# ath92/splat-renderer

Hardware: AMD Instinct MI355X
Metric: Msplats/sec (higher is better)
Workload: dtype f32

## Files before the change

include/splat.h:

```cpp
#ifndef SPLAT_H
#define SPLAT_H

#include <stddef.h>
#include <stdint.h>

#ifdef __cplusplus
extern "C" {
#endif

#define SPLAT_ABI_VERSION 3

#define SPLAT_OK 0
#define SPLAT_ERR_INVALID (-1)
#define SPLAT_ERR_HIP (-2)
#define SPLAT_ERR_OOM (-3)
#define SPLAT_ERR_CAPACITY (-4)
#define SPLAT_ERR_STATE (-5)
#define SPLAT_ERR_NO_DEVICE (-6)
#define SPLAT_ERR_COMM (-7)
#define SPLAT_ERR_RETRY (-8)

typedef struct splat_ctx splat_ctx;
typedef struct splat_sorter splat_sorter;
typedef struct splat_binner splat_binner;
typedef struct splat_comm splat_comm;

#define SPLAT_PROPS_BYTES 32
#define SPLAT_PROJECTED_BYTES 32
#define SPLAT_SORT_BLOCK 3840

enum {
    SPLAT_STAGE_PROJECT = 0,
    SPLAT_STAGE_SORT = 1,
    SPLAT_STAGE_BIN = 2,
    SPLAT_STAGE_COMPOSITE = 3,
    SPLAT_STAGE_EXCHANGE = 4,
    SPLAT_STAGE_BIN_SCATTER = 5,
    SPLAT_STAGE_BIN_PASS2 = 6,
    SPLAT_STAGE_BIN_TILE_SORT = 7,
    SPLAT_STAGE_COUNT = 8
};

int splat_ctx_create(int device_ordinal, splat_ctx **out);
int splat_ctx_create_on_stream(int device_ordinal, void *hip_stream, splat_ctx **out);
void splat_ctx_destroy(splat_ctx *ctx);
const char *splat_last_error(splat_ctx *ctx);
int splat_sync(splat_ctx *ctx);
int splat_abi_version(void);
int splat_set_timing(splat_ctx *ctx, int enabled);
#define SPLAT_TIMING_COUNT_ENTRIES 0x80000000u
int splat_set_timing_stages(splat_ctx *ctx, uint32_t stage_mask);
int splat_set_timing_sampling(splat_ctx *ctx, uint32_t every);
int splat_stage_time_ms(splat_ctx *ctx, int stage, float *ms);
// ... 24 lines not shown
void splat_sort_destroy(splat_sorter *s);
uint32_t splat_sort_capacity(const splat_sorter *s);
void *splat_sort_keys(splat_sorter *s);
void *splat_sort_payload(splat_sorter *s);
int splat_sort_run(splat_sorter *s, uint32_t n, uint32_t bit_begin, uint32_t bit_end);
void *splat_sort_sorted_payload(splat_sorter *s);
void *splat_sort_sorted_keys(splat_sorter *s);
int splat_probe_lds_atomic_order(splat_ctx *ctx, uint64_t *mismatches);
int splat_sort_set_mode(splat_sorter *s, int mode);
int splat_rank_status(splat_ctx *ctx, int *policy, int *atomics_ordered, uint32_t *order_faults);
#ifdef SPLAT_TEST_HOOKS
int splat_debug_inject_order_fault(splat_ctx *ctx, uint32_t tile, uint32_t position);
int splat_debug_set_tile_order(splat_ctx *ctx, const void *order_dptr);
int splat_debug_set_tile_sort_order(splat_ctx *ctx, const void *order_dptr);
int splat_debug_rerun_tile_sort(splat_ctx *ctx, splat_binner *binner);
int splat_debug_tile_sort_launches(splat_ctx *ctx, uint32_t *launches);
int splat_debug_lds_rate(splat_ctx *ctx, int kind, uint32_t workgroups_per_cu, uint32_t iters, float *ms);
#endif
int splat_composite_forget_history(splat_ctx *ctx);
int splat_composite_options(splat_ctx *ctx, int kernel, int ahead, int predict);

int splat_scan_u32(splat_ctx *ctx, const void *in, void *out, uint32_t n, void *total_dptr);

int splat_bin_create(splat_ctx *ctx, uint32_t tile_size, splat_binner **out);
void splat_bin_destroy(splat_binner *b);
int splat_bin_run(splat_binner *b, const void *projected, uint32_t n_splats, const void *sorted,
                  uint32_t n_sorted, uint32_t width, uint32_t height, uint32_t tile_row0,
                  uint32_t tile_row1);
uint32_t splat_bin_tile_size(const splat_binner *b);
int splat_bin_counts(splat_binner *b, void **dptr);
int splat_bin_offsets(splat_binner *b, void **dptr);
int splat_bin_indices(splat_binner *b, void **dptr);
int splat_bin_total(splat_binner *b, uint64_t *total_pairs);
#define SPLAT_FRAME_ORDER_DEFAULT (-1)
#define SPLAT_FRAME_SORT_FIRST 0
#define SPLAT_FRAME_TILE_FIRST 1
int splat_bin_set_frame_order(splat_binner *b, int order);
int splat_bin_dims(splat_binner *b, uint32_t *ntx, uint32_t *nty);

int splat_validate_tile_order(splat_ctx *ctx, const void *projected, const void *tile_offsets,
                              uint32_t num_tiles, const void *tile_indices, uint64_t total_pairs,
                              uint64_t *violations_host);

#define SPLAT_COMPOSITE_FRONT_TO_BACK 0
#define SPLAT_COMPOSITE_REFERENCE_LITERAL 1
#define SPLAT_RECORDS_PROJECTED 0
#define SPLAT_RECORDS_COMPACT 1
#define SPLAT_RECORDS_DISC48 2
#define SPLAT_RECORDS_LIT32 3
#define SPLAT_FOOTPRINT_ISOTROPIC 0
#define SPLAT_FOOTPRINT_DISC 1
#define SPLAT_FOOTPRINT_ELLIPSOID 2
typedef struct splat_composite_cfg {
    uint32_t mode;
    uint32_t early_out;
    uint32_t tile_size;
    uint32_t tile_row0;
    uint32_t tile_row1;
    uint32_t record_format;
    uint32_t prelit;
    uint32_t footprint;
} splat_composite_cfg;
int splat_lit_colors(splat_ctx *ctx, const void *color_opacity, uint32_t color_stride_vec4,
                     const void *normals, uint32_t normal_stride_vec4, uint32_t n, void *lit);
int splat_composite(splat_ctx *ctx, const splat_composite_cfg *cfg, const void *color_opacity,
                    uint32_t color_stride_vec4, const void *normals, uint32_t normal_stride_vec4,
// ... 191 lines not shown
```

splat_renderer_amd/_lib.py:

```python
import ctypes as C
import os

_HERE = os.path.dirname(os.path.abspath(__file__))
LIB_PATH = os.environ.get("SPLAT_LIB_PATH") or os.path.join(_HERE, "libsplat_hip.so")

OK = 0
ERR_NAMES = {-1: "INVALID", -2: "HIP", -3: "OOM", -4: "CAPACITY", -5: "STATE", -6: "NO_DEVICE", -7: "COMM", -8: "RETRY"}
ERR_CAPACITY, ERR_RETRY = -4, -8
RENDER_AGAIN = (ERR_CAPACITY, ERR_RETRY)

STAGE_PROJECT, STAGE_SORT, STAGE_BIN, STAGE_COMPOSITE, STAGE_EXCHANGE, STAGE_BIN_SCATTER, STAGE_BIN_PASS2, STAGE_BIN_TILE_SORT = range(8)
STAGE_NAMES = ("project", "sort", "bin", "composite", "exchange", "bin_scatter", "bin_second_pass", "bin_tile_sort")
TIMING_COUNT_ENTRIES = 0x80000000
MODE_FRONT_TO_BACK, MODE_REFERENCE_LITERAL = 0, 1
RECORDS_PROJECTED, RECORDS_COMPACT, RECORDS_DISC48, RECORDS_LIT32 = 0, 1, 2, 3
FOOTPRINT_ISOTROPIC, FOOTPRINT_DISC, FOOTPRINT_ELLIPSOID = 0, 1, 2
U32_MAX = 0xFFFFFFFF


class SplatError(RuntimeError):
    def __init__(self, code, msg):
        super().__init__(f"libsplat_hip error {ERR_NAMES.get(code, code)}: {msg}")
        self.code = code


SDF_SPHERE, SDF_BOX, SDF_TORUS, SDF_CAPSULE, SDF_UNION, SDF_INTERSECTION, SDF_SUBTRACTION, SDF_SMOOTH_UNION = 0, 1, 2, 3, 16, 17, 18, 19
SDF_MAX_INSTR = 32


class SdfInstr(C.Structure):
    _fields_ = [("op", C.c_uint32), ("a", C.c_float * 7)]


class Aov(C.Structure):
    _fields_ = [("depth_f32", C.c_void_p), ("alpha_f32", C.c_void_p), ("id_u32", C.c_void_p)]


class CompositeCfg(C.Structure):
    _fields_ = [("mode", C.c_uint32), ("early_out", C.c_uint32), ("tile_size", C.c_uint32),
                ("tile_row0", C.c_uint32), ("tile_row1", C.c_uint32), ("record_format", C.c_uint32),
                ("prelit", C.c_uint32), ("footprint", C.c_uint32)]

# ... 62 lines not shown
    "splat_densify_plan_workspace_bytes": (C.c_uint64, [_u32]),
    "splat_densify_plan": (_i, [_vp, _vp, _vp, _vp, _vp, _vp, _u32, C.POINTER(DensifyCfg), _vp, C.c_uint64, _vp, C.POINTER(_u32),
                                C.POINTER(_u32)]),
    "splat_densify_geometry": (_i, [_vp, _vp, _u32, _vp, _vp, _vp, C.POINTER(DensifyCfg), _vp, _vp]),
    "splat_densify_rows": (_i, [_vp, _vp, _u32, _vp, _vp, _u32, _u32]),
    "splat_mcmc_sample_workspace_bytes": (C.c_uint64, [_u32]),
    "splat_mcmc_sample": (_i, [_vp, _vp, _u32, _u32, _u32, _f64, C.c_uint64, _vp, C.c_uint64, _vp, _vp, _vp, C.POINTER(_u32)]),
    "splat_mcmc_apply": (_i, [_vp, _vp, _vp, _vp, _u32, _u32, _u32, _f64, C.POINTER(McmcPlanes)]),
    "splat_mcmc_noise": (_i, [_vp, _vp, _vp, _vp, _vp, _u32, _f64, _u32, C.c_uint64]),
    "splat_extract_keys":(_i, [_vp, _vp, _u32, _u32, _vp, _vp]),
    "splat_sort_create": (_i, [_vp, _u32, _pvp]),
    "splat_sort_destroy": (None, [_vp]),
    "splat_sort_capacity": (_u32, [_vp]),
    "splat_sort_keys": (_vp, [_vp]),
    "splat_sort_payload": (_vp, [_vp]),
    "splat_sort_run": (_i, [_vp, _u32, _u32, _u32]),
    "splat_sort_sorted_payload": (_vp, [_vp]),
    "splat_sort_sorted_keys": (_vp, [_vp]),
    "splat_probe_lds_atomic_order": (_i, [_vp, C.POINTER(C.c_uint64)]),
    "splat_sort_set_mode": (_i, [_vp, _i]),
    "splat_rank_status": (_i, [_vp, C.POINTER(_i), C.POINTER(_i), C.POINTER(_u32)]),
    "splat_composite_forget_history": (_i, [_vp]),
    "splat_composite_options": (_i, [_vp, _i, _i, _i]),
    "splat_scan_u32": (_i, [_vp, _vp, _vp, _u32, _vp]),
    "splat_bin_create": (_i, [_vp, _u32, _pvp]),
    "splat_bin_destroy": (None, [_vp]),
    "splat_bin_run": (_i, [_vp, _vp, _u32, _vp, _u32, _u32, _u32, _u32, _u32]),
    "splat_bin_tile_size": (_u32, [_vp]),
    "splat_bin_counts": (_i, [_vp, _pvp]),
    "splat_bin_offsets": (_i, [_vp, _pvp]),
    "splat_bin_indices": (_i, [_vp, _pvp]),
    "splat_bin_total": (_i, [_vp, C.POINTER(C.c_uint64)]),
    "splat_bin_set_frame_order": (_i, [_vp, _i]),
    "splat_bin_dims": (_i, [_vp, C.POINTER(_u32), C.POINTER(_u32)]),
    "splat_validate_tile_order": (_i, [_vp, _vp, _vp, _u32, _vp, C.c_uint64, C.POINTER(C.c_uint64)]),
    "splat_lit_colors": (_i, [_vp, _vp, _u32, _vp, _u32, _u32, _vp]),
    "splat_composite": (_i, [_vp, C.POINTER(CompositeCfg), _vp, _u32, _vp, _u32, _vp, _vp, _vp, _vp, _u32, _u32,
                             _vp, _vp, _vp]),
    "splat_render_frame": (_i, [_vp, _vp, _vp, C.POINTER(CompositeCfg), C.POINTER(C.c_float), _vp, _vp, _u32, _u32,
                                _u32, _vp, _vp, _vp]),
    "splat_render_frame_planes": (_i, [_vp, _vp, _vp, C.POINTER(CompositeCfg), C.POINTER(C.c_float), _vp, _vp, _vp, _u32,
                                       _u32, _u32, _vp, _vp, _vp]),
    "splat_composite_aov": (_i, [_vp, C.POINTER(CompositeCfg), _vp, _u32, _vp, _u32, _vp, _vp, _vp, _vp, _u32, _u32,
                                 _vp, _vp, _vp, C.POINTER(Aov)]),
    "splat_render_frame_aov": (_i, [_vp, _vp, _vp, C.POINTER(CompositeCfg), C.POINTER(C.c_float), _vp, _vp, _u32, _u32,
                                    _u32, _vp, _vp, _vp, C.POINTER(Aov)]),
    "splat_render_frame_planes_aov": (_i, [_vp, _vp, _vp, C.POINTER(CompositeCfg), C.POINTER(C.c_float), _vp, _vp, _vp,
                                           _u32, _u32, _u32, _vp, _vp, _vp, C.POINTER(Aov)]),
    "splat_project_slice": (_i, [_vp, C.POINTER(C.c_float), _vp, _u32, _u32, _u32, _vp]),
    "splat_project_slice_compact": (_i, [_vp, C.POINTER(C.c_float), _vp, _u32, _u32, _u32, _vp]),
    "splat_project_slice_disc": (_i, [_vp, C.POINTER(C.c_float), _vp, _u32, _vp, _u32, _u32, _u32, _vp]),
    "splat_expand_compact": (_i, [_vp, _vp, _u32, _u32, _vp]),
    "splat_band_frame": (_i, [_vp, _vp, _vp, C.POINTER(CompositeCfg), _vp, _vp, _vp, _u32, _u32, _u32, _vp, _vp, _vp]),
    "splat_band_settle": (_i, [_vp, _vp, _vp, C.POINTER(_u32), C.POINTER(C.c_uint64)]),
    "splat_band_kept": (_i, [_vp, _vp, C.POINTER(_u32)]),
    "splat_band_keys": (_i, [_vp, _vp, _vp, _u32, _u32, _u32, _u32, _u32, _u32, C.POINTER(_u32)]),
    "splat_sdf_gradients": (_i, [_vp, _vp, _u32, _vp, _u32, _vp]),
    "splat_sdf_update_positions": (_i, [_vp, _vp, _vp, _u32, _vp]),
    "splat_sdf_scale_factors": (_i, [_vp, _vp, _u32, _vp, _u32, _vp]),
    "splat_sdf_curvature": (_i, [_vp, _vp, _vp, _u32, _vp]),
    "splat_sdf_seed_positions": (_i, [_vp, C.POINTER(C.c_float), C.POINTER(C.c_float), _u32, C.c_uint64, _vp]),
    "splat_sdf_generate": (_i, [_vp, _vp, _u32, C.POINTER(C.c_float), C.POINTER(C.c_float), C.c_uint64, _vp, _u32, _u32, _vp, _vp, _vp, _vp]),
    "splat_point_frame": (_i, [_vp, _vp, C.POINTER(C.c_float), _vp, _u32, _vp, _u32, _vp, _u32, _u32, _u32, _u32, _vp, _vp, _vp, _vp]),
    "splat_comm_unique_id": (_i, [_vp]),
    "splat_comm_init": (_i, [_vp, _i, _i, _vp, _pvp]),
    "splat_comm_destroy": (None, [_vp]),
# ... 60 lines not shown
```

splat_renderer_amd/csrc/bin.hip:

```cpp
#include "common.h"
#include <cstring>
#include "tile_range.h"

#include <chrono>
#include <cstdio>
#include <cstdlib>
#include <sched.h>

constexpr uint32_t BIN_THREADS = 256;
constexpr uint32_t BIN_PER_THREAD = 4;
constexpr uint32_t BIN_BLOCK = BIN_THREADS * BIN_PER_THREAD;
constexpr uint32_t BIN_STAGE_PAIRS = 4096;

__device__ __forceinline__ uint32_t range_hits(uint2 r) {
    const uint32_t tx0 = r.x & 0xffffu, tx1 = r.x >> 16, ty0 = r.y & 0xffffu, ty1 = r.y >> 16;
    return (tx0 > tx1 || ty0 > ty1) ? 0u : (tx1 - tx0 + 1) * (ty1 - ty0 + 1);
}

__device__ __forceinline__ uint32_t block_sum(uint32_t v, uint32_t *wsum) {
#pragma unroll
    for (int d = 32; d >= 1; d >>= 1) v += __shfl_xor(v, d);
    if ((threadIdx.x & 63) == 0) wsum[threadIdx.x >> 6] = v;
    __syncthreads();
    return wsum[0] + wsum[1] + wsum[2] + wsum[3];
// ... 155 lines not shown
        hi = nhi;
    }
    const uint32_t pos = lo + lane;
    const bool less = pos < hi && sorted_tiles[pos] < t;
    const uint32_t first = lo + (uint32_t)__popcll(__ballot(less));
    if (lane == 0) offsets[t] = first;
}

__global__ __launch_bounds__(256) void k_tile_counts(const uint32_t *__restrict__ offsets, uint32_t tiles,
                                                     uint32_t *__restrict__ counts) {
    const uint32_t t = blockIdx.x * 256u + threadIdx.x;
    if (t < tiles) counts[t] = offsets[t + 1] - offsets[t];
}

__global__ __launch_bounds__(256) void k_validate_tile_order(const float4 *__restrict__ projected,
                                                             const uint32_t *__restrict__ offsets, uint32_t tiles,
                                                             const uint32_t *__restrict__ indices, uint32_t pairs,
                                                             unsigned long long *__restrict__ violations) {
    const uint32_t i = blockIdx.x * 256u + threadIdx.x;
    if (i + 1 >= pairs) return;
    uint32_t lo = 0, hi = tiles;
    while (hi - lo > 1) {
        const uint32_t mid = (lo + hi) >> 1;
        if (offsets[mid] <= i) lo = mid; else hi = mid;
    }
    if (i + 1 >= offsets[lo + 1]) return;
    const uint32_t a = indices[i], b = indices[i + 1];
    const uint32_t ka = __float_as_uint(reinterpret_cast<const float *>(projected)[(size_t)a * 8 + 4]);
    const uint32_t kb = __float_as_uint(reinterpret_cast<const float *>(projected)[(size_t)b * 8 + 4]);
    const uint32_t sa = ka ^ (((ka >> 31) == 1u) ? 0xffffffffu : 0x80000000u), sb = kb ^ (((kb >> 31) == 1u) ? 0xffffffffu : 0x80000000u);
    if (sa > sb || (sa == sb && a >= b)) atomicAdd(violations, 1ull);
}

static void binner_free(splat_binner *b) {
    if (b->counts) (void)hipFree(b->counts);
    if (b->offsets) (void)hipFree(b->offsets);
    if (b->blocksums) (void)hipFree(b->blocksums);
    if (b->ranges) (void)hipFree(b->ranges);
    if (b->tf_hist) (void)hipFree(b->tf_hist);
    b->tf_hist = nullptr;
    b->counts = b->offsets = b->blocksums = nullptr;
    b->ranges = nullptr;
    b->tiles_cap = b->splats_cap = 0;
}

static void sorter_free_members(splat_sorter *s) {
    if (s->keys) (void)hipFree(s->keys);
    if (s->keys_b) (void)hipFree(s->keys_b);
    if (s->hist) (void)hipFree(s->hist);
    if (s->d_count) (void)hipFree(s->d_count);
    s->keys = s->keys_b = s->payload = s->payload_b = s->hist = s->d_count = nullptr;
    s->capacity = 0;
}

int binner_reserve_range32(splat_binner *b, uint32_t n_splats) {
    splat_ctx *ctx = b->ctx;
    if (n_splats <= b->range32_cap) return SPLAT_OK;
    HIP_TRY(ctx, hipStreamSynchronize(ctx->stream));
    if (b->range32) (void)hipFree(b->range32);
    b->range32 = nullptr;
    b->range32_cap = 0;
    if (hipMalloc((void **)&b->range32, (size_t)n_splats * 4 + 16) != hipSuccess) return ctx_fail(ctx, SPLAT_ERR_OOM, "binner hipMalloc");
    b->range32_cap = n_splats;
    return SPLAT_OK;
}

// ... 34 lines not shown
    return SPLAT_OK;
}

int binner_reserve(splat_binner *b, uint32_t tiles, uint32_t n_sorted) {
    splat_ctx *ctx = b->ctx;
    if (tiles <= b->tiles_cap && n_sorted <= b->splats_cap) return SPLAT_OK;
    HIP_TRY(ctx, hipStreamSynchronize(ctx->stream));
    uint32_t tc = tiles > b->tiles_cap ? tiles : b->tiles_cap;
    uint32_t sc = n_sorted > b->splats_cap ? n_sorted : b->splats_cap;
    binner_free(b);
    if (hipMalloc((void **)&b->counts, (size_t)tc * 4 + 16) != hipSuccess ||
        hipMalloc((void **)&b->offsets, (size_t)tc * 4 + 16) != hipSuccess ||
        hipMalloc((void **)&b->blocksums, ((size_t)div_up(sc, BIN_BLOCK) + TF_SMALL_FRAME_SPLATS / TF_BLOCK_SMALL) * 4 + 16) != hipSuccess ||
        hipMalloc((void **)&b->ranges, (size_t)sc * 8 + 16) != hipSuccess ||
        hipMalloc((void **)&b->tf_hist, ((size_t)256 * (div_up(sc, BIN_BLOCK) + TF_SMALL_FRAME_SPLATS / TF_BLOCK_SMALL) + 256) * 4) != hipSuccess) {
        binner_free(b);
        return ctx_fail(ctx, SPLAT_ERR_OOM, "binner hipMalloc");
    }
    b->tiles_cap = tc;
    b->splats_cap = sc;
    return SPLAT_OK;
}

int binner_run(splat_binner *b, const void *projected, uint32_t n_splats, const void *sorted, uint32_t n_sorted, uint32_t width,
               uint32_t height, uint32_t tile_row0, uint32_t tile_row1, const uint32_t *range32, const uint32_t *n_sorted_dev,
               const uint32_t *depth_keys, const uint2 *range_wide) {
    splat_ctx *ctx = b->ctx;
    const bool tile_first = depth_keys != nullptr;
    const bool hist_ready = b->tf_hist_ready;
    const uint32_t *tf_cidx = b->tf_cidx, *tf_kept = b->tf_kept;
    b->tf_hist_ready = false;
    b->tf_cidx = nullptr;
    b->tf_kept = nullptr;
    ARG_CHECK(ctx, width >= 1 && height >= 1);
    ARG_CHECK(ctx, n_sorted == 0 || (projected && (sorted || tile_first)));
    ARG_CHECK(ctx, !tile_first || (range32 && n_sorted == n_splats && !n_sorted_dev));
    ARG_CHECK(ctx, !range_wide || (!range32 && !tile_first));
    const uint32_t ntx = div_up(width, b->tile), nty = div_up(height, b->tile);
    ARG_CHECK(ctx, ntx <= 65535 && nty <= 65535 && (uint64_t)ntx * nty <= (1u << 24));
    const uint32_t tiles = ntx * nty;
    if (tile_row1 > nty) tile_row1 = nty;
    if (tile_row0 > tile_row1) tile_row0 = tile_row1;
    const uint32_t blocks = div_up(n_sorted, BIN_BLOCK);

    int rc = binner_reserve(b, tiles, n_sorted);
    if (rc != SPLAT_OK) return rc;
    b->ntx = ntx;
    b->nty = nty;
    b->ran = false;
    const BinParams bp = {width, height, b->tile, ntx, nty, tile_row0, tile_row1};

    rc = binner_settle(b);
    if (rc != SPLAT_OK) return rc;

    const uint32_t tf_bits = tile_id_bits(tiles), tf_lo_bits = tile_id_low_bits(tiles);
    ARG_CHECK(ctx, !tile_first || hist_ready);

    stage_begin(ctx, SPLAT_STAGE_BIN);
    uint32_t total32 = 0;
    bool async = false;
    if (n_sorted > 0) {
        if (tile_first) {
            rc = radix_rowscan_launch(ctx, b->tf_hist, div_up(n_splats, b->tf_block), 1u << tf_lo_bits);
            if (rc != SPLAT_OK) return rc;
        } else if (range_wide)
            hipLaunchKernelGGL(k_bin_count_wide, dim3(blocks), dim3(BIN_THREADS), 0, ctx->stream, range_wide, n_splats,
// ... 8 lines not shown
        const uint64_t want_async = (uint64_t)b->last_total + b->last_total / 8 + 4096;
        async = b->allow_async && b->have_last && b->last_total > 0 && want_async <= b->pairs.capacity;
        if (!(tile_first && async)) {
            rc = scan_exclusive_u32(ctx, b->blocksums, b->blocksums, tile_first ? div_up(n_splats, b->tf_block) : blocks, b->d_total);
            if (rc != SPLAT_OK) return rc;
        }
        if (async) {
            b->pair_limit = (uint32_t)want_async;
            total32 = b->pair_limit;
        } else {
            HIP_TRY(ctx, hipMemcpyAsync(b->pinned, b->d_total, 4, hipMemcpyDeviceToHost, ctx->stream));
            HIP_TRY(ctx, hipStreamSynchronize(ctx->stream));
            total32 = *(volatile uint32_t *)b->pinned;
            b->last_total = total32;
            b->have_last = true;
            if (total32 > b->pairs.capacity) {
                uint64_t want = (uint64_t)total32 + total32 / 2 + 8192;
                if (want > 0x3ffff000ull) want = 0x3ffff000ull;
                if (total32 > want) return ctx_fail(ctx, SPLAT_ERR_CAPACITY, "binSplats: more than 2^30 tile-splat pairs");
                rc = sorter_reserve(&b->pairs, (uint32_t)want);
                if (rc != SPLAT_OK) return rc;
            }
            b->pair_limit = total32;
        }
    }
    b->total = async ? b->last_total : total32;
    if (total32 > 0 && tile_first) {
        rc = binner_reserve_wide(b);
        if (rc != SPLAT_OK) return rc;
        const uint32_t tf_hi_bits = tf_bits - tf_lo_bits;
        stage_begin(ctx, SPLAT_STAGE_BIN_SCATTER);
        rc = tf_scatter_launch(ctx, range32, depth_keys, n_splats, ntx, (1u << tf_lo_bits) - 1u, b->tf_hist, b->d_total, b->pair_limit,
                               b->d_total + 1, b->tf_hi, b->wide_a, b->tf_block, tf_lo_bits, tf_hi_bits > 0, &b->tf_runs, b->offsets, tiles,
                               nullptr, 0u, tf_cidx, tf_kept);
        stage_end(ctx, SPLAT_STAGE_BIN_SCATTER);
        if (rc != SPLAT_OK) return rc;
        const bool primary = tf_hi_bits == 0;
        stage_begin(ctx, SPLAT_STAGE_BIN_PASS2);
        rc = tf_second_pass_launch(ctx, b->tf_hi, b->wide_a, b->wide_b, &b->tf_runs, total32, tiles, tf_lo_bits, tf_hi_bits, b->tf2_hist,
                                   b->offsets, b->d_total);
        stage_end(ctx, SPLAT_STAGE_BIN_PASS2);
        if (rc != SPLAT_OK) return rc;
        const uint32_t band_tiles = tile_row1 > tile_row0 ? (tile_row1 - tile_row0) * ntx : 1u;
        const uint64_t band_key = ((uint64_t)tile_row0 << 48) ^ ((uint64_t)tile_row1 << 32) ^ tiles;
        stage_begin(ctx, SPLAT_STAGE_BIN_TILE_SORT);
        rc = tile_sort_launch(ctx, b->offsets, tiles, primary ? b->wide_a : b->wide_b, primary ? b->wide_b : b->wide_a, b->pairs.payload,
                              b->counts, b->d_total + 1, band_tiles >= 6144u ? (uint32_t)(b->total / band_tiles) : 0u, band_tiles,
                              (async && b->last_band_key == band_key) ? b->last_long_tiles : 0xffffffffu, &b->last_short_class);
        stage_end(ctx, SPLAT_STAGE_BIN_TILE_SORT);
        if (rc != SPLAT_OK) return rc;
        b->pairs.result_in_primary = true;
        b->pending_tile_first = true;
        b->last_band_key = band_key;
        b->report_for_composite = b->pinned_dev;
        b->report_seq = ++b->seq;
        b->pending = true;
    } else if (total32 > 0) {
        hipLaunchKernelGGL(k_bin_expand, dim3(blocks), dim3(BIN_THREADS), 0, ctx->stream, (const uint32_t *)sorted, n_sorted,
                           b->ranges, b->blocksums, ntx, b->pair_limit, b->d_total + 1, b->pairs.keys, b->pairs.payload);
        LAUNCH_CHECK(ctx, "k_bin_expand");
        const uint32_t bits = tile_id_bits(tiles);
        const uint32_t *p_dev = async ? b->d_total : nullptr;
        const uint32_t lo_bits = tile_id_low_bits(tiles);
        rc = radix_sort_pairs(ctx, b->pairs.keys, b->pairs.payload, b->pairs.keys_b, b->pairs.payload_b, b->pairs.hist, total32, 0,
                              bits, &b->pairs.result_in_primary, 0, p_dev, false, lo_bits);
        if (rc != SPLAT_OK) return rc;
        const uint32_t *sorted_tiles = b->pairs.result_in_primary ? b->pairs.keys : b->pairs.keys_b;
        hipLaunchKernelGGL(k_tile_offsets, dim3(div_up(tiles + 1, 4)), dim3(256), 0, ctx->stream, sorted_tiles, total32, p_dev,
                           tiles, b->offsets, b->d_total, async ? b->pinned_dev : nullptr, async ? ++b->seq : 0u);
        LAUNCH_CHECK(ctx, "k_tile_offsets");
        hipLaunchKernelGGL(k_tile_counts, dim3(div_up(tiles, 256)), dim3(256), 0, ctx->stream, b->offsets, tiles, b->counts);
        LAUNCH_CHECK(ctx, "k_tile_counts");
        if (async) b->pending = true;
    } else {
        HIP_TRY(ctx, hipMemsetAsync(b->counts, 0, (size_t)tiles * 4, ctx->stream));
        HIP_TRY(ctx, hipMemsetAsync(b->offsets, 0, (size_t)(tiles + 1) * 4, ctx->stream));
        if (b->pairs.capacity == 0) {
            rc = sorter_reserve(&b->pairs, 1);
            if (rc != SPLAT_OK) return rc;
        }
    }
    stage_end(ctx, SPLAT_STAGE_BIN);
    b->ran = true;
    return SPLAT_OK;
}

int binner_settle(splat_binner *b) {
    if (!b->pending) return SPLAT_OK;
    splat_ctx *ctx = b->ctx;
    b->pending = false;
    volatile uint32_t *rep = (volatile uint32_t *)b->pinned;
    auto next_query = std::chrono::steady_clock::now() + std::chrono::milliseconds(5);
    for (uint32_t spins = 0; rep[2] != b->seq; ++spins) {
        if ((spins & 63u) != 63u) continue;
        if (std::chrono::steady_clock::now() < next_query) {
            sched_yield();
            continue;
        }
        next_query = std::chrono::steady_clock::now() + std::chrono::milliseconds(1);
        const hipError_t q = hipStreamQuery(ctx->stream);
        if (q == hipSuccess) {
            if (rep[2] != b->seq) return ctx_fail(ctx, SPLAT_ERR_STATE, "binner: the pair-total report of the previous frame never arrived");
            break;
        }
        if (q != hipErrorNotReady) {
            b->have_last = false;
            return ctx_fail(ctx, SPLAT_ERR_HIP, "binner: waiting for the previous frame's pair total", q);
        }
    }
    __atomic_thread_fence(__ATOMIC_ACQUIRE);
    const uint32_t total = ((volatile uint32_t *)b->pinned)[0], flags = ((volatile uint32_t *)b->pinned)[1];
    b->last_long_tiles = b->pending_tile_first ? ((volatile uint32_t *)b->pinned)[3] : 0xffffffffu;
    b->pending_tile_first = false;
    b->last_total = total;
    b->have_last = true;
    b->total = total;
    if (flags & FRAME_FLAG_ORDER) {
        b->ran = false;
        ctx->order_faults++;
        if (ctx->rank_policy != RANK_BALLOT)
            fprintf(stderr, "[splat] a frame's tile lists failed the per-tile order check (tile lists are re-rendered): this context ranks with "
                            "ballots from now on (splat_rank_status: policy ballot, orderFaults %u)\n", ctx->order_faults);
        ctx->rank_policy = RANK_BALLOT;
        return ctx_fail(ctx, SPLAT_ERR_RETRY,
                        "the previous frame's tile lists failed the order check (ranking with returning LDS atomics was not in lane "
                        "order): the context now ranks with ballots; render that frame again");
    }
    if ((flags & FRAME_FLAG_OVERFLOW) || total > b->pair_limit) {
        uint64_t want = (uint64_t)total + total / 2 + 8192;
        if (want > 0x3ffff000ull) want = 0x3ffff000ull;
        b->ran = false;
        int rc = sorter_reserve(&b->pairs, (uint32_t)want);
        if (rc != SPLAT_OK) return rc;
        return ctx_fail(ctx, SPLAT_ERR_CAPACITY,
                        "the previous frame produced more tile-splat pairs than its sync-free limit (sized from the frame "
                        "before it): its tile lists are incomplete; capacity has been raised, render that frame again");
    }
    return SPLAT_OK;
}

extern "C" {

#ifdef SPLAT_TEST_HOOKS
int splat_debug_rerun_tile_sort(splat_ctx *ctx, splat_binner *b) {
    if (!ctx || !b) return ctx_fail(ctx, SPLAT_ERR_INVALID, "ctx/binner is NULL");
    ARG_CHECK(ctx, b->ran && b->wide_a && b->wide_b && b->ntx && b->nty);
    const uint32_t tiles = b->ntx * b->nty;
    const bool primary = tile_id_bits(tiles) - tile_id_low_bits(tiles) == 0;
    return tile_sort_launch(ctx, b->offsets, tiles, primary ? b->wide_a : b->wide_b, primary ? b->wide_b : b->wide_a, b->pairs.payload_b,
                            nullptr, b->d_total + 4, tiles >= 6144u ? (uint32_t)(b->total / tiles) : 0u);
}
#endif

int splat_bin_create(splat_ctx *ctx, uint32_t tile_size, splat_binner **out) {
    if (!ctx) return ctx_fail(nullptr, SPLAT_ERR_INVALID, "ctx is NULL");
    ARG_CHECK(ctx, out != nullptr);
    *out = nullptr;
    ARG_CHECK(ctx, tile_size >= 1 && tile_size <= 4096);
    splat_binner *b = new splat_binner();
    b->ctx = ctx;
    b->tile = tile_size;
    b->pairs.ctx = ctx;
    if (hipMalloc((void **)&b->d_total, 32) != hipSuccess || hipHostMalloc((void **)&b->pinned, 16, hipHostMallocMapped | hipHostMallocCoherent) != hipSuccess ||
        hipHostGetDevicePointer((void **)&b->pinned_dev, b->pinned, 0) != hipSuccess ||
        hipEventCreateWithFlags(&b->readback_done, hipEventDisableTiming) != hipSuccess) {
        if (b->d_total) (void)hipFree(b->d_total);
        if (b->pinned) (void)hipHostFree(b->pinned);
        delete b;
        return ctx_fail(ctx, SPLAT_ERR_OOM, "binner allocation");
    }
    memset(b->pinned, 0, 16);
    if (const char *e = getenv("SPLAT_BIN_SYNC")) b->allow_async = !(e[0] == '1');
    *out = b;
    return SPLAT_OK;
}

void splat_bin_destroy(splat_binner *b) {
    if (!b) return;
    (void)hipStreamSynchronize(b->ctx->stream);
    binner_free(b);
    sorter_free_members(&b->pairs);
    if (b->d_total) (void)hipFree(b->d_total);
    if (b->range32) (void)hipFree(b->range32);
    binner_free_wide(b);
    if (b->expanded) (void)hipFree(b->expanded);
    if (b->discs) (void)hipFree(b->discs);
    if (b->points) (void)hipFree(b->points);
    if (b->band_idx) (void)hipFree(b->band_idx);
    if (b->pinned) (void)hipHostFree(b->pinned);
    if (b->readback_done) (void)hipEventDestroy(b->readback_done);
    delete b;
}

int splat_bin_run(splat_binner *b, const void *projected, uint32_t n_splats, const void *sorted, uint32_t n_sorted,
                  uint32_t width, uint32_t height, uint32_t tile_row0, uint32_t tile_row1) {
    if (!b) return ctx_fail(nullptr, SPLAT_ERR_INVALID, "binner is NULL");
    return binner_run(b, projected, n_splats, sorted, n_sorted, width, height, tile_row0, tile_row1, nullptr);
}

uint32_t splat_bin_tile_size(const splat_binner *b) { return b ? b->tile : 0; }

int splat_bin_set_frame_order(splat_binner *b, int order) {
    if (!b) return ctx_fail(nullptr, SPLAT_ERR_INVALID, "binner is NULL");
    ARG_CHECK(b->ctx, order >= SPLAT_FRAME_ORDER_DEFAULT && order <= SPLAT_FRAME_TILE_FIRST);
    b->frame_order = order;
    return SPLAT_OK;
}

int splat_bin_counts(splat_binner *b, void **dptr) {
    if (!b || !dptr) return ctx_fail(nullptr, SPLAT_ERR_INVALID, "binner/dptr is NULL");
    if (int rc = binner_settle(b)) return rc;
    if (!b->ran) return ctx_fail(b->ctx, SPLAT_ERR_STATE, "Tile counts buffer not initialized");
    *dptr = b->counts;
    return SPLAT_OK;
}

int splat_bin_offsets(splat_binner *b, void **dptr) {
    if (!b || !dptr) return ctx_fail(nullptr, SPLAT_ERR_INVALID, "binner/dptr is NULL");
    if (int rc = binner_settle(b)) return rc;
    if (!b->ran) return ctx_fail(b->ctx, SPLAT_ERR_STATE, "Tile offsets buffer not initialized");
    *dptr = b->offsets;
    return SPLAT_OK;
}

int splat_bin_indices(splat_binner *b, void **dptr) {
    if (!b || !dptr) return ctx_fail(nullptr, SPLAT_ERR_INVALID, "binner/dptr is NULL");
    if (int rc = binner_settle(b)) return rc;
    if (!b->ran) return ctx_fail(b->ctx, SPLAT_ERR_STATE, "Tile indices buffer not initialized");
    *dptr = b->pairs.result_in_primary ? b->pairs.payload : b->pairs.payload_b;
    return SPLAT_OK;
}

int splat_bin_total(splat_binner *b, uint64_t *total_pairs) {
    if (!b || !total_pairs) return ctx_fail(nullptr, SPLAT_ERR_INVALID, "binner/total is NULL");
    if (int rc = binner_settle(b)) return rc;
    if (!b->ran) return ctx_fail(b->ctx, SPLAT_ERR_STATE, "binSplats has not run");
    *total_pairs = b->total;
    return SPLAT_OK;
}

int splat_validate_tile_order(splat_ctx *ctx, const void *projected, const void *tile_offsets, uint32_t num_tiles,
                              const void *tile_indices, uint64_t total_pairs, uint64_t *violations_host) {
    if (!ctx) return ctx_fail(nullptr, SPLAT_ERR_INVALID, "ctx is NULL");
    ARG_CHECK(ctx, violations_host && (total_pairs == 0 || (projected && tile_offsets && tile_indices)) && num_tiles >= 1);
    ARG_CHECK(ctx, total_pairs < (1ull << 32));
    *violations_host = 0;
    if (total_pairs < 2) return SPLAT_OK;
    int rc = ctx_ensure_scan_ws(ctx, 256);
    if (rc != SPLAT_OK) return rc;
    unsigned long long *d = (unsigned long long *)ctx->scan_ws;
    HIP_TRY(ctx, hipMemsetAsync(d, 0, 8, ctx->stream));
    hipLaunchKernelGGL(k_validate_tile_order, dim3(div_up((uint32_t)total_pairs, 256)), dim3(256), 0, ctx->stream,
                       (const float4 *)projected, (const uint32_t *)tile_offsets, num_tiles, (const uint32_t *)tile_indices,
                       (uint32_t)total_pairs, d);
    LAUNCH_CHECK(ctx, "k_validate_tile_order");
    unsigned long long v = 0;
    HIP_TRY(ctx, hipMemcpyAsync(&v, d, 8, hipMemcpyDeviceToHost, ctx->stream));
    HIP_TRY(ctx, hipStreamSynchronize(ctx->stream));
    *violations_host = v;
    return SPLAT_OK;
// ... 12 lines not shown
```

splat_renderer_amd/csrc/common.h:

```cpp
#pragma once

#include <hip/hip_runtime.h>
#include <stdint.h>
#include <string>

#include "../../include/splat.h"

constexpr int kWave = 64;

#include <vector>
struct StageTimer {
    std::vector<hipEvent_t> beg, end;
    size_t used = 0;
    uint32_t tick = 0;
};
struct PxHistory {
    uint64_t key = 0;
    uint32_t *mem = nullptr;
    uint32_t cap = 0, parity = 0, streak = 0;
    uint64_t last_use = 0;
};
constexpr int PX_HISTORIES = 4;

struct splat_ctx {
    int device = 0;
    hipStream_t stream = nullptr;
    bool own_stream = false;
    std::string err;
    bool timing = false;
    int lds_atomic_ordered = -1;
    int rank_policy = 0;
    uint32_t order_faults = 0;
#ifdef SPLAT_TEST_HOOKS
    const uint32_t *debug_tile_order = nullptr;
    const uint32_t *debug_sort_order = nullptr;
    uint32_t inject_order_fault = 0;
    uint32_t inject_order_position = 0;
    uint32_t tile_sort_launches = 0;
#endif
    int opt_composite_kernel = -1, opt_px_ahead = 0, opt_px_predict = -1;
    PxHistory px_hist[PX_HISTORIES];
    uint64_t px_clock = 0;
    uint32_t timing_mask = 0xffffffffu;
    uint32_t timing_every = 1;
    StageTimer timers[SPLAT_STAGE_COUNT];
    void *scan_ws = nullptr;
    size_t scan_ws_bytes = 0;
    unsigned long long *d_consumed = nullptr;
    uint32_t consumed_tiles = 0;
    uint2 *d_window_counts = nullptr;
    uint32_t window_counts_cap = 0;
    void *pinned = nullptr;
    size_t pinned_bytes = 0;
// ... 14 lines not shown
        hipError_t e__ = (expr);                                             \
        if (e__ != hipSuccess) return ctx_fail((ctx), SPLAT_ERR_HIP, #expr, e__); \
    } while (0)

#define LAUNCH_CHECK(ctx, name)                                                       \
    do {                                                                              \
        hipError_t e__ = hipGetLastError();                                           \
        if (e__ != hipSuccess) return ctx_fail((ctx), SPLAT_ERR_HIP, "launch " name, e__); \
    } while (0)

#define ARG_CHECK(ctx, cond)                                               \
    do {                                                                   \
        if (!(cond)) return ctx_fail((ctx), SPLAT_ERR_INVALID, "argument check failed: " #cond); \
    } while (0)

static inline uint32_t div_up(uint32_t a, uint32_t b) { return (a + b - 1) / b; }
static inline uint64_t div_up64(uint64_t a, uint64_t b) { return (a + b - 1) / b; }

int scan_exclusive_u32(splat_ctx *ctx, const uint32_t *in, uint32_t *out, uint32_t n, uint32_t *total);
constexpr uint32_t RADIX_PART = 4096;
int radix_sort_pairs(splat_ctx *ctx, uint32_t *k0, uint32_t *p0, uint32_t *k1, uint32_t *p1,
                     uint32_t *hist, uint32_t n, uint32_t bit_begin, uint32_t bit_end,
                     bool *result_in_primary, int mode = -1, const uint32_t *n_dev = nullptr,
                     bool iota_payload = false, uint32_t first_bits = 8);

int radix_probe_lds_atomic_order(splat_ctx *ctx, uint64_t *mismatches_host);
int ctx_resolve_rank_mode(splat_ctx *ctx);
constexpr int RANK_CHECKED = 0, RANK_ATOMIC = 1, RANK_BALLOT = 2;
static inline bool rank_atomic_ok(const splat_ctx *ctx, bool checked) {
    if (ctx->lds_atomic_ordered != 1 || ctx->rank_policy == RANK_BALLOT) return false;
    return ctx->rank_policy == RANK_ATOMIC || checked;
}
constexpr uint32_t FRAME_FLAG_OVERFLOW = 1u, FRAME_FLAG_ORDER = 2u;

struct splat_sorter {
    splat_ctx *ctx = nullptr;
    uint32_t capacity = 0;
    uint32_t *keys = nullptr, *keys_b = nullptr, *payload = nullptr, *payload_b = nullptr;
    uint32_t *hist = nullptr;
    uint32_t *d_count = nullptr;
    bool count_pending = false, have_last_count = false;
    uint32_t last_count = 0, count_bound = 0;
    uint32_t *pinned_count = nullptr;
    hipEvent_t count_event = nullptr;
    uint32_t kept_blocks = 0;
    bool result_in_primary = true;
    bool ran = false;
    int mode = -1;
};

int sorter_reserve(splat_sorter *s, uint32_t capacity);

struct TfRuns {
    uint32_t *start, *total;
    uint8_t *part_digit;
    uint32_t *parts;
};
constexpr uint32_t TF_RUN_ALIGN = 4096;
constexpr uint32_t TF_RUN_SLACK = 256 * TF_RUN_ALIGN;
static inline uint32_t tf2_parts_bound(uint32_t pairs, uint32_t lo_bits) { return div_up(pairs, TF_RUN_ALIGN) + (1u << lo_bits); }

struct splat_binner {
    splat_ctx *ctx = nullptr;
    uint32_t tile = 16;
    uint32_t ntx = 0, nty = 0;
    uint32_t tiles_cap = 0, splats_cap = 0, range32_cap = 0;
// ... 9 lines not shown
    uint32_t *tf2_hist = nullptr;
    uint32_t *tf_runs_mem = nullptr;
    TfRuns tf_runs = {};
    uint32_t *tf_hist = nullptr;
    int frame_order = -1;
    void *expanded = nullptr;
    uint32_t expanded_cap = 0;
    void *discs = nullptr;
    uint32_t discs_cap = 0;
    void *points = nullptr;
    uint32_t points_cap = 0;
    bool tf_hist_ready = false;
    uint32_t tf_block = 1024;
    const uint32_t *tf_cidx = nullptr, *tf_kept = nullptr;
    uint32_t *band_idx = nullptr;
    uint32_t band_idx_cap = 0;
    uint64_t total = 0;
    bool ran = false;
    bool allow_async = true;
    bool pending = false;
    bool have_last = false;
    uint32_t last_total = 0;
    uint32_t last_long_tiles = 0xffffffffu;
    uint64_t last_band_key = ~0ull;
    uint32_t last_short_class = 0;
    bool pending_tile_first = false;
    uint32_t pair_limit = 0;
    uint32_t *pinned = nullptr;
    uint32_t *pinned_dev = nullptr;
    uint32_t seq = 0;
    uint32_t *report_for_composite = nullptr;
    uint32_t report_seq = 0;
    hipEvent_t readback_done = nullptr;
};

struct BinParams {
    uint32_t width, height, tile, ntx, nty, row0, row1;
    uint32_t skip_outside;
};

constexpr uint32_t TF_BLOCK_LARGE = 1024, TF_BLOCK_SMALL = 256, TF_SMALL_FRAME_SPLATS = 1u << 20;
struct TfHistOut {
    uint32_t *hist, *blocksums, *overflow_flag;
    uint32_t mask, num_parts;
    uint32_t block = TF_BLOCK_LARGE;
    uint32_t xcd_per = 0;
    uint32_t *cidx = nullptr, *kept_groups = nullptr;
};
__device__ __forceinline__ uint32_t xcd_block_of(uint32_t i, uint32_t xcd_per) {
    return xcd_per ? (i & 7u) * xcd_per + (i >> 3) : i;
}
static inline uint32_t tile_id_bits(uint32_t tiles) {
    uint32_t bits = 1;
    while ((1u << bits) < tiles) ++bits;
    return bits;
}
static inline uint32_t tile_id_low_bits(uint32_t tiles) {
    const uint32_t bits = tile_id_bits(tiles);
    return bits <= 8 ? bits : bits / 2 < 8 ? bits / 2 : 8;
}

__device__ __forceinline__ void tile_report(const uint32_t *d_total, uint32_t *report, uint32_t seq) {
    report[0] = d_total[0];
    report[1] = d_total[1];
    report[3] = d_total[3];
    __threadfence_system();
    __hip_atomic_store(&report[2], seq, __ATOMIC_RELEASE, __HIP_MEMORY_SCOPE_SYSTEM);
}

int binner_reserve_range32(splat_binner *b, uint32_t n_splats);
int binner_run(splat_binner *b, const void *projected, uint32_t n_splats, const void *sorted, uint32_t n_sorted, uint32_t width,
               uint32_t height, uint32_t tile_row0, uint32_t tile_row1, const uint32_t *range32,
               const uint32_t *n_sorted_dev = nullptr, const uint32_t *depth_keys = nullptr,
               const uint2 *range_wide = nullptr);
int binner_reserve(splat_binner *b, uint32_t tiles, uint32_t n_sorted);
int tf_scatter_launch(splat_ctx *ctx, const uint32_t *range32, const uint32_t *depth_keys, uint32_t n, uint32_t ntx, uint32_t mask,
                      const uint32_t *hist, uint32_t *d_total, uint32_t pair_limit, uint32_t *overflow, uint8_t *out_hi,
                      uint2 *out_val, uint32_t block_splats, uint32_t lo_bits, bool second_pass, const TfRuns *runs,
                      uint32_t *offsets_if_final, uint32_t tiles, uint32_t *report, uint32_t seq, const uint32_t *cidx = nullptr,
                      const uint32_t *kept = nullptr);
int tf_second_pass_launch(splat_ctx *ctx, const uint8_t *hi, const uint2 *val_in, uint2 *val_out, const TfRuns *runs, uint32_t pairs_bound,
                          uint32_t tiles, uint32_t lo_bits, uint32_t hi_bits, uint32_t *hist, uint32_t *offsets, const uint32_t *d_total);
int radix_rowscan_launch(splat_ctx *ctx, uint32_t *hist, uint32_t parts, uint32_t rows);
int tile_sort_launch(splat_ctx *ctx, const uint32_t *offsets, uint32_t tiles, uint2 *vals, uint2 *scratch, uint32_t *out_idx,
                     uint32_t *counts, uint32_t *frame_flags, uint32_t mean_list, uint32_t band_tiles = 0,
                     uint32_t long_tiles_hint = 0xffffffffu, uint32_t *short_class_io = nullptr);
int binner_settle(splat_binner *b);
struct CompositeArgs {
    const void *color_opacity = nullptr, *normals = nullptr;
    uint32_t color_stride_vec4 = 1, normal_stride_vec4 = 1;
    const void *projected = nullptr, *tile_indices = nullptr, *tile_counts = nullptr, *tile_offsets = nullptr;
    uint32_t width = 0, height = 0;
    void *out_rgba8 = nullptr, *out_rgba32f = nullptr;
    void *consumed = nullptr;
    const uint32_t *frame_total = nullptr;
    uint32_t *report = nullptr;
    uint32_t report_seq = 0;
    const splat_aov *aov = nullptr;
    const float *ext_z = nullptr;
    uint32_t ext_zstride = 0;
};
int composite_launch(splat_ctx *ctx, const splat_composite_cfg *cfg, const CompositeArgs &a);
int aov_check(splat_ctx *ctx, const splat_composite_cfg *cfg, const splat_aov *aov, bool has_depth);
int project_launch(splat_ctx *ctx, const float *uniforms, const void *pos_radius, uint32_t pr_stride_vec4, uint32_t n,
                   uint32_t index_base, void *projected, void *keys, void *payload, uint32_t n_padded, uint32_t *range32,
                   const BinParams *bp, const TfHistOut *hist_out = nullptr, const void *normals = nullptr,
                   uint32_t normal_stride_vec4 = 1, void *discs = nullptr,
                   const struct LitIO *lit = nullptr,
                   uint2 *range_wide = nullptr,
                   const struct EllIO *ell = nullptr);
int binner_reserve_range_wide(splat_binner *b, uint32_t n_splats);
```

splat_renderer_amd/csrc/composite.h:

```cpp
#pragma once
#include "common.h"
#include "disc.h"
#include "shade.h"
#include "variant.h"

typedef float v2f __attribute__((ext_vector_type(2)));

constexpr int CT = 16;
constexpr int CBATCH = 256;

struct CompositeParams {
    const float4 *color;  uint32_t color_stride;
    const float4 *normals; uint32_t normal_stride;
    const float4 *projected;
    uint32_t compact;
    uint32_t lit32;
    uint32_t disc;
    uint32_t disc_stride;
    uint32_t disc_lit;
    uint32_t prelit;
    const uint32_t *indices, *counts, *offsets;
    uint32_t width, height, ntx, tile_row0;
    uint32_t *out_rgba8;
    float4 *out_rgba32f;
    unsigned long long *consumed;
    const uint32_t *frame_total;
    uint32_t *report;
    uint32_t report_seq;
    const uint32_t *tile_order;
    uint32_t *tile_cost;
    const uint32_t *order_src;
    uint32_t *order_dst;
    const uint32_t *cost_prev;
#ifdef PX_PROFILE
    uint32_t debug_cap;
#endif
    float *aov_depth;
    float *aov_alpha;
    uint32_t *aov_id;
    const float *aov_z;
    uint32_t aov_zstride;
};

struct AovPixel {
    float zw = 0.0f, ws = 0.0f, wmax = 0.0f;
    uint32_t id = 0xffffffffu;
    __device__ __forceinline__ void add(float w, float2 zi) {
        zw += zi.x * w;
        ws += w;
        const bool top = w > wmax;
        wmax = top ? w : wmax;
        id = top ? __float_as_uint(zi.y) : id;
    }
    __device__ __forceinline__ void store(const CompositeParams &p, size_t o, float T_end) const {
        if (p.aov_alpha) p.aov_alpha[o] = 1.0f - T_end;
        if (p.aov_depth) p.aov_depth[o] = ws > 0.0f ? zw / ws : __builtin_inff();
        if (p.aov_id) p.aov_id[o] = id;
    }
};

__device__ __forceinline__ float2 aov_entry(const CompositeParams &p, uint32_t idx) {
    if (idx == 0xffffffffu) return make_float2(0.0f, __uint_as_float(0xffffffffu));
    const float z = p.aov_z ? p.aov_z[(size_t)idx * p.aov_zstride] : 0.0f;
    return make_float2(z, __uint_as_float(idx));
}

__device__ __forceinline__ uint32_t unorm8(float v) {
    v = fminf(fmaxf(v, 0.0f), 1.0f);
    return (uint32_t)(v * 255.0f + 0.5f);
}

__device__ __forceinline__ uint2 quadrant_mask(uint32_t xb, uint32_t yb) {
    const uint32_t lo = (((yb & 15u) * 0x00204081u) & 0x01010101u) * xb;
    const uint32_t hi = (((yb >> 4) * 0x00204081u) & 0x01010101u) * xb;
// ... 64 lines not shown
```

splat_renderer_amd/csrc/composite.hip:

```cpp
#include "composite.h"


#include <cstdlib>

__global__ __launch_bounds__(256) void k_lit_colors(const float4 *__restrict__ color, uint32_t color_stride,
                                                    const float4 *__restrict__ normals, uint32_t normal_stride, uint32_t n,
                                                    float4 *__restrict__ lit) {
    const uint32_t i = blockIdx.x * 256u + threadIdx.x;
    if (i < n) lit[i] = lit_color(color[(size_t)i * color_stride], normals[(size_t)i * normal_stride]);
}

template <int MODE, bool EARLY_OUT, bool DISC, bool LIT32, bool AOV = false, bool ELL = false>
__global__ __launch_bounds__(256) void k_composite(CompositeParams p) {
    constexpr int PAR = DISC ? 3 : 2;
    __shared__ float4 s_par[CBATCH][PAR];
    __shared__ uint2 s_mask[4][CBATCH];
    __shared__ uint32_t s_wave_done[4];
    __shared__ uint32_t s_wave_consumed[4];
    __shared__ float2 s_aov[AOV ? CBATCH : 1];
    static_assert(!AOV || MODE == SPLAT_COMPOSITE_FRONT_TO_BACK, "the auxiliary outputs are nearest-on-top only");
    AovPixel aov;

    const uint32_t tid = threadIdx.x, lane = tid & 63, w = tid >> 6;
    if (p.report && blockIdx.x == 0 && blockIdx.y == 0 && tid == 0) tile_report(p.frame_total, p.report, p.report_seq);
// ... 349 lines not shown
}

#ifndef PX_WAVES
#define PX_WAVES 5
#endif
#define PX_PRIORITY(N)                                         \
    do {                                                       \
        if ((N) == 3u) __builtin_amdgcn_s_setprio(1);          \
        else if ((N) == 6u) __builtin_amdgcn_s_setprio(2);     \
        else if ((N) == 10u) __builtin_amdgcn_s_setprio(3);    \
    } while (0)
__device__ __forceinline__ v2f fma_clamp01(v2f a, v2f b, v2f c) {
    v2f r;
    asm("v_pk_fma_f32 %0, %1, %2, %3 clamp" : "=v"(r) : "v"(a), "v"(b), "v"(c));
    return r;
}

__device__ __forceinline__ bool px_any_live(const v2f *T) {
    const uint32_t m = max(max(__float_as_uint(T[0].x), __float_as_uint(T[0].y)), max(__float_as_uint(T[1].x), __float_as_uint(T[1].y)));
    return m > __float_as_uint(T_STOP);
}

__device__ __forceinline__ void px_top(v2f w, uint32_t id, v2f &wmax, v2u &idmax) {
    const bool t0 = w.x > wmax.x, t1 = w.y > wmax.y;
    wmax = (v2f){t0 ? w.x : wmax.x, t1 ? w.y : wmax.y};
    idmax = (v2u){t0 ? id : idmax.x, t1 ? id : idmax.y};
}
__device__ __forceinline__ void px_aov_store(const CompositeParams &p, size_t o, float T_end, float zw, float ws, uint32_t id) {
    if (p.aov_alpha) p.aov_alpha[o] = 1.0f - T_end;
    if (p.aov_depth) p.aov_depth[o] = ws > 0.0f ? zw / ws : __builtin_inff();
    if (p.aov_id) p.aov_id[o] = id;
}

template <bool EARLY_OUT, bool LIT32, bool COUNT, int AH, bool DISC, bool AOV = false, bool ELL = false>
__global__ __launch_bounds__(128, AOV ? 4 : PX_WAVES) void k_composite_px(CompositeParams p, uint32_t band_tiles) {
    constexpr uint32_t NB = AH + 1;
    typedef typename PxBufOf<DISC>::type Buf;
    constexpr uint32_t BUF_BYTES = NB * sizeof(Buf) > PX_ORDER_SCRATCH ? NB * sizeof(Buf) : PX_ORDER_SCRATCH;
    __shared__ __attribute__((aligned(16))) char s_raw[BUF_BYTES];
    Buf *const s_buf = reinterpret_cast<Buf *>(s_raw);
    __shared__ uint32_t s_done[2];
    __shared__ float2 s_aov[AOV ? NB : 1][PXC + 1];
    const uint32_t tid = threadIdx.x, lane = tid & 63;
    const uint32_t role = (uint32_t)__builtin_amdgcn_readfirstlane((int)(tid >> 6));
    if (blockIdx.x == 0) {
        if (p.report && tid == 0) tile_report(p.frame_total, p.report, p.report_seq);
        if (p.order_dst) px_make_order(p.order_src, band_tiles, p.order_dst, reinterpret_cast<uint32_t *>(s_buf));
        return;
    }
    const uint32_t t_local = p.tile_order ? p.tile_order[blockIdx.x - 1u] : blockIdx.x - 1u;
    const uint32_t tx = t_local % p.ntx, ty = t_local / p.ntx + p.tile_row0;
    const uint32_t tile_idx = ty * p.ntx + tx;
#ifdef PX_PROFILE
    const uint32_t count = min(p.counts[tile_idx], p.debug_cap), off = p.offsets[tile_idx];
#else
    const uint32_t count = p.counts[tile_idx], off = p.offsets[tile_idx];
#endif
    const uint32_t nchunks = (count + PXC - 1) / PXC;
    const float tile_x0 = (float)(tx * CT), tile_y0 = (float)(ty * CT);
    uint32_t lim = nchunks;
    if (p.cost_prev) lim = min(max(p.cost_prev[t_local], 1u), nchunks);
    lim = (uint32_t)__builtin_amdgcn_readfirstlane((int)lim);

    if (role == 1) {
        if (count == 0) return;
        const uint32_t e = lane & 31, h = lane >> 5;
        const float tile_c = (h ? tile_y0 : tile_x0) + 0.5f, tile_0 = h ? tile_y0 : tile_x0;
        if constexpr (DISC) {
            if (lane < 3 * NB) s_buf[lane / 3].par[0][lane % 3] = make_float4(0.0f, 0.0f, 0.0f, 0.0f);
        } else if (lane <= PX_TROWS) {
#pragma unroll
            for (uint32_t b = 0; b < NB; ++b) {
                if (lane < PX_TROWS) s_buf[b].t[lane][0] = make_float2(0.0f, 0.0f);
                else s_buf[b].col[0] = make_float4(0.0f, 0.0f, 0.0f, 0.0f);
            }
        }
        if constexpr (AOV) {
            if (lane < NB) s_aov[lane][0] = make_float2(0.0f, __uint_as_float(0xffffffffu));
        }
// ... 107 lines not shown
#endif
            if (EARLY_OUT && __builtin_amdgcn_readfirstlane((int)s_done[k & 1])) break;
            if (k >= nchunks) break;
            if (k >= lim) {
                lim = nchunks;
                fetch_lim = count - 1u;
                idx_c = p.indices[off + min((k + 2u) * PXC + e, fetch_lim)];
                PX_FETCH(p.indices[off + min((k + 1u) * PXC + e, fetch_lim)], rb);
                if (COUNT) staged = max(staged, min((k + 2u) * PXC, count));
                built = k;
                continue;
            }
            ++k;
        }
#ifdef PX_PROFILE
        if (p.consumed && lane == 0)
            p.consumed[(size_t)tile_idx * 2] = (((__builtin_amdgcn_s_memtime() - pb0) >> 4) & 0xffffull) | (((pb_wait >> 4) & 0xffffull) << 16) |
                                               ((pb_chunks & 0xffffull) << 48);
        return;
#endif
        if (COUNT && p.consumed && lane == 0) p.consumed[(size_t)tile_idx * 2] += (unsigned long long)staged;
        return;
    }

    const uint32_t bx = lane & 7, by = lane >> 3;
    const uint32_t px0 = tx * CT + 2 * bx, py0 = ty * CT + 2 * by;
    const bool okx0 = px0 < p.width, okx1 = px0 + 1 < p.width, oky0 = py0 < p.height, oky1 = py0 + 1 < p.height;
    v2f cr[2] = {{0.0f, 0.0f}, {0.0f, 0.0f}}, cg[2] = {{0.0f, 0.0f}, {0.0f, 0.0f}}, cb[2] = {{0.0f, 0.0f}, {0.0f, 0.0f}};
    v2f T[2] = {{(okx0 && oky0) ? 1.0f : 0.0f, (okx1 && oky0) ? 1.0f : 0.0f}, {(okx0 && oky1) ? 1.0f : 0.0f, (okx1 && oky1) ? 1.0f : 0.0f}};
    v2f zw[2] = {{0.0f, 0.0f}, {0.0f, 0.0f}}, ws[2] = {{0.0f, 0.0f}, {0.0f, 0.0f}}, wm[2] = {{0.0f, 0.0f}, {0.0f, 0.0f}};
    v2u idm[2] = {{0xffffffffu, 0xffffffffu}, {0xffffffffu, 0xffffffffu}};
    uint32_t stop_pos = 0;
    uint32_t walked = 0;
    constexpr uint32_t NONE = 0xffffffffu;
    const uint32_t lane_x = DISC ? 48u : (bx * PX_ROW + 1u) * 8u;
    const uint32_t d_xy = ((8u + by - bx) * PX_ROW) * 8u;
    const uint32_t d_col = DISC ? 0u : (uint32_t)offsetof(PxBuf, col) + 16u - lane_x;
    const v2f pxc = {(float)px0 + 0.5f, (float)px0 + 1.5f}, pyc = {(float)py0 + 0.5f, (float)py0 + 1.5f};
    const char *const lds = reinterpret_cast<const char *>(s_buf);
    v2f k_huge = {0x1p40f, 0x1p40f}, k_stop = {-T_STOP * 0x1p40f, -T_STOP * 0x1p40f};
    asm volatile("" : "+v"(k_huge), "+v"(k_stop));
    v2f k_in_a = {-0x1p23f, -0x1p23f}, k_in_b = {0x1p23f + 1.0f, 0x1p23f + 1.0f};
    static_assert(0x1p23f + 1.0f == 8388609.0f, "2^23 + 1 is a binary32 number");
    if (DISC) asm volatile("" : "+v"(k_in_a), "+v"(k_in_b));
#ifdef PX_PROFILE
    const unsigned long long pc0 = __builtin_amdgcn_s_memtime();
    unsigned long long pc_wait = 0, pc_trips = 0, pc_ntrips = 0;
#endif
    if (count) {
        if (lane < 2) s_done[lane] = 0;
        bool finished = false;
        bool carried_ok = false;
        uint32_t carried = 0;
        for (uint32_t k = 0;; ++k) {
#ifdef PX_PROFILE
            { const unsigned long long w0_ = __builtin_amdgcn_s_memtime(); __syncthreads(); pc_wait += __builtin_amdgcn_s_memtime() - w0_; }
#else
            __syncthreads();
#endif
            if (EARLY_OUT && finished) break;
            if (k >= nchunks) break;
            if (k >= lim) {
                lim = nchunks;
                __syncthreads();
            }
            const uint32_t o0 = (k % NB) * (uint32_t)sizeof(Buf), o1 = ((k + 1u) % NB) * (uint32_t)sizeof(Buf);
// ... 141 lines not shown
            for (;;) {
                if (ra_ == 0) break;
#ifdef PX_PROFILE
                pc_ntrips++;
#endif
                PX_POP(jb, rb_, ab, sb);
                PX_LOAD(jb, ab, eb);
                __builtin_amdgcn_sched_barrier(0);
                PX_BLEND(ja, ra_, sa, ea, true);
                if (EARLY_OUT && all_stopped) break;
                if (rb_ == 0) break;
#ifdef PX_PROFILE
                pc_ntrips++;
#endif
                PX_POP(ja, ra_, aa, sa);
                PX_LOAD(ja, aa, ea);
                __builtin_amdgcn_sched_barrier(0);
                PX_BLEND(jb, rb_, sb, eb, COUNT);
                if (EARLY_OUT && all_stopped) break;
            }
#undef PX_POP
#undef PX_LOAD
#undef PX_BLEND
#undef PX_DISC_ROW
#ifdef PX_PROFILE
            if (__ballot(T[0].x > 1e30f) == 0) pc_trips += __builtin_amdgcn_s_memtime() - pt0;
#endif
            carried = nxt;
            if (AH >= 2) walked += __ballot(nxt != nxt0) != 0 ? 1u : 0u;
            if (COUNT && EARLY_OUT && jlast != NONE) stop_pos = cb0 + jlast + 1;
            if (EARLY_OUT) {
                const bool live = px_any_live(T);
                finished = __ballot(live) == 0;
                if (finished && lane == 0) s_done[(k + 1u) & 1u] = 1;
            }
        }
    }

    if (p.tile_cost && lane == 0) p.tile_cost[t_local] = walked;
#ifdef PX_PROFILE
    if (p.consumed && lane == 0)
        p.consumed[(size_t)tile_idx * 2 + 1] = (((__builtin_amdgcn_s_memtime() - pc0) >> 4) & 0xffffull) | (((pc_wait >> 4) & 0xffffull) << 16) |
                                               (((pc_trips >> 4) & 0xffffull) << 32) | ((pc_ntrips & 0xffffull) << 48);
#else
    if (COUNT && p.consumed && count) {
        uint32_t used = stop_pos;
#pragma unroll
        for (int d = 32; d >= 1; d >>= 1) used = max(used, (uint32_t)__shfl_xor((int)used, d));
        const bool px_live = px_any_live(T);
        if (!EARLY_OUT || __ballot(px_live) != 0) used = count;
        if (lane == 0) p.consumed[(size_t)tile_idx * 2 + 1] += (unsigned long long)used;
    }
#endif

#pragma unroll
    for (int r = 0; r < 2; ++r) {
        const uint32_t py = py0 + r;
        if (py >= p.height || !okx0) continue;
        if (EARLY_OUT && !DISC) {
            T[r].x = (T[r].x >= 0.0f) ? T[r].x : __builtin_nanf("");
            T[r].y = (T[r].y >= 0.0f) ? T[r].y : __builtin_nanf("");
        }
        const float r0 = cr[r].x + 0.05f * T[r].x, g0 = cg[r].x + 0.05f * T[r].x, b0 = cb[r].x + 0.1f * T[r].x;
        const float r1 = cr[r].y + 0.05f * T[r].y, g1 = cg[r].y + 0.05f * T[r].y, b1 = cb[r].y + 0.1f * T[r].y;
        const size_t o = (size_t)py * p.width + px0;
        const uint32_t q0 = unorm8(r0) | (unorm8(g0) << 8) | (unorm8(b0) << 16) | (255u << 24);
        const uint32_t q1 = unorm8(r1) | (unorm8(g1) << 8) | (unorm8(b1) << 16) | (255u << 24);
        if (p.out_rgba8) {
            if (okx1 && (o & 1) == 0) *reinterpret_cast<uint2 *>(p.out_rgba8 + o) = make_uint2(q0, q1);
            else {
                p.out_rgba8[o] = q0;
                if (okx1) p.out_rgba8[o + 1] = q1;
            }
        }
        if (p.out_rgba32f) {
            p.out_rgba32f[o] = make_float4(r0, g0, b0, 1.0f);
            if (okx1) p.out_rgba32f[o + 1] = make_float4(r1, g1, b1, 1.0f);
        }
        if constexpr (AOV) {
            px_aov_store(p, o, T[r].x, zw[r].x, ws[r].x, idm[r].x);
            if (okx1) px_aov_store(p, o + 1, T[r].y, zw[r].y, ws[r].y, idm[r].y);
        }
    }
}

static bool g_px_order_on = true;
static bool g_px_predict_on = true;
static int g_px_ahead = 0;

bool composite_uses_px(const splat_ctx *ctx, uint32_t ntx, uint32_t nty) {
    constexpr uint32_t PX_MIN_TILES = 2048;
    static int s_px = -2;
    if (s_px == -2) {
        const char *e = getenv("SPLAT_COMPOSITE");
        s_px = !e ? -1 : (e[0] == 'p' || e[0] == 'P') ? 1 : (e[0] == 'q' || e[0] == 'Q') ? 0 : -1;
    }
    const int kernel = ctx->opt_composite_kernel >= 0 ? ctx->opt_composite_kernel : s_px;
    return kernel == 1 || (kernel == -1 && ntx * nty >= PX_MIN_TILES);
}

static int px_order_prepare(splat_ctx *ctx, uint32_t band_tiles, uint64_t key, CompositeParams &p) {
    const bool predict_on = ctx->opt_px_predict >= 0 ? ctx->opt_px_predict != 0 : g_px_predict_on;
    if (!g_px_order_on && !predict_on) return SPLAT_OK;
    PxHistory *h = nullptr, *lru = &ctx->px_hist[0];
    for (auto &e : ctx->px_hist) {
        if (e.key == key) h = &e;
        if (e.last_use < lru->last_use) lru = &e;
    }
    if (!h) {
        h = lru;
        h->key = key;
        h->streak = 0;
    }
    h->last_use = ++ctx->px_clock;
    if (band_tiles > h->cap) {
        HIP_TRY(ctx, hipStreamSynchronize(ctx->stream));
        if (h->mem) (void)hipFree(h->mem);
        h->mem = nullptr;
        h->cap = 0;
        h->streak = 0;
        const uint32_t cap = (band_tiles + 128u * 16u + 1023u) & ~1023u;
        if (hipMalloc((void **)&h->mem, (size_t)cap * 16) != hipSuccess) {
            h->key = 0;
            return ctx_fail(ctx, SPLAT_ERR_OOM, "composite tile order hipMalloc");
        }
        (void)hipMemsetAsync(h->mem, 0, (size_t)cap * 16, ctx->stream);
        h->cap = cap;
    }
    uint32_t *cost[2] = {h->mem, h->mem + h->cap}, *order[2] = {h->mem + 2 * (size_t)h->cap, h->mem + 3 * (size_t)h->cap};
    const uint32_t q = h->parity & 1u;
    p.tile_cost = cost[q];
    if (g_px_order_on && h->streak >= 2) p.tile_order = order[q];
    if (h->streak >= 1) {
        if (predict_on) p.cost_prev = cost[q ^ 1u];
        if (g_px_order_on) {
            p.order_src = cost[q ^ 1u];
            p.order_dst = order[q ^ 1u];
        }
    }
    h->parity ^= 1u;
    if (h->streak < 2) h->streak++;
#ifdef PX_PROFILE
    {
        static int freeze = -1;
        static uint32_t *frozen = nullptr;
        if (freeze < 0) freeze = getenv("SPLAT_PX_FREEZE") ? 1 : 0;
        if (freeze) {
// ... 144 lines not shown
    const uint32_t ntx = div_up(width, T), nty = div_up(height, T);
    uint32_t r0 = cfg->tile_row0, r1 = cfg->tile_row1 > nty ? nty : cfg->tile_row1;
    if (r0 >= r1) return SPLAT_OK;
    CompositeParams p;
    p.color = (const float4 *)a.color_opacity;
    p.color_stride = a.color_stride_vec4;
    p.normals = (const float4 *)a.normals;
    p.normal_stride = a.normal_stride_vec4;
    p.projected = (const float4 *)a.projected;
    p.compact = cfg->record_format == SPLAT_RECORDS_COMPACT;
    p.lit32 = lit32;
    p.prelit = cfg->prelit != 0;
    p.disc = is_disc;
    p.disc_stride = (cfg->record_format == SPLAT_RECORDS_DISC48 || (p.disc && lit32)) ? 3u : 2u;
    p.disc_lit = p.disc && lit32;
    p.indices = (const uint32_t *)a.tile_indices;
    p.counts = (const uint32_t *)a.tile_counts;
    p.offsets = (const uint32_t *)a.tile_offsets;
    p.width = width;
    p.height = height;
    p.ntx = ntx;
    p.tile_row0 = r0;
    p.out_rgba8 = (uint32_t *)a.out_rgba8;
    p.out_rgba32f = (float4 *)a.out_rgba32f;
    p.consumed = (unsigned long long *)a.consumed;
    p.frame_total = a.frame_total;
    p.report = a.report;
    p.report_seq = a.report_seq;
    p.tile_order = nullptr;
    p.tile_cost = nullptr;
    p.order_src = nullptr;
    p.order_dst = nullptr;
    p.cost_prev = nullptr;
#ifdef PX_PROFILE
    p.debug_cap = getenv("SPLAT_PX_CAP") ? (uint32_t)strtoul(getenv("SPLAT_PX_CAP"), nullptr, 10) : 0xffffffffu;
#endif
    p.aov_depth = aov ? (float *)aov->depth_f32 : nullptr;
    p.aov_alpha = aov ? (float *)aov->alpha_f32 : nullptr;
    p.aov_id = aov ? (uint32_t *)aov->id_u32 : nullptr;
    p.aov_z = (aov && aov->depth_f32) ? zsrc + zoff : (const float *)a.tile_counts;
    p.aov_zstride = (aov && aov->depth_f32) ? zstride : 0u;
    if (T != CT) return composite_tile_launch(ctx, cfg, p, nty, r0, r1, &report.launched);
    static bool s_env = false;
    if (!s_env) {
        s_env = true;
        const char *o = getenv("SPLAT_TILE_ORDER");
        g_px_order_on = !(o && o[0] == '0');
        const char *pr = getenv("SPLAT_PX_PREDICT");
        g_px_predict_on = !(pr && pr[0] == '0');
        const char *ah = getenv("SPLAT_PX_AHEAD");
        g_px_ahead = !ah ? 0 : ah[0] == '1' ? 1 : 2;
    }
    const bool eo = cfg->early_out != 0, want_aov = aov != nullptr, ell = cfg->footprint == SPLAT_FOOTPRINT_ELLIPSOID;
    if (cfg->mode == SPLAT_COMPOSITE_FRONT_TO_BACK && composite_uses_px(ctx, ntx, nty)) {
        const int ahead = ctx->opt_px_ahead > 0 ? ctx->opt_px_ahead : g_px_ahead > 0 ? g_px_ahead : ((eo && !p.disc) ? 1 : 2);
        const uint32_t band_tiles = ntx * (r1 - r0);
        const uint64_t key = (((uint64_t)ntx << 40) ^ ((uint64_t)r0 << 20) ^ (uint64_t)r1 ^ ((uint64_t)width << 50) ^
                              ((uint64_t)(uintptr_t)a.tile_counts * 0x9E3779B97F4A7C15ull)) | 1u;
        const int orc = px_order_prepare(ctx, band_tiles, key, p);
        if (orc != SPLAT_OK) return orc;
#ifdef SPLAT_TEST_HOOKS
        if (ctx->debug_tile_order) p.tile_order = ctx->debug_tile_order;
#endif
        const bool ok = variant_dispatch(
            [&](auto eo_, auto lit, auto cnt, auto ah, auto disc, auto aov_, auto ell_) {
                if constexpr (!(disc.value && lit.value)) {
                    launch_kernel(ctx, SPLAT_STAGE_COMPOSITE, k_composite_px<eo_.value, lit.value, cnt.value, ah.value, disc.value, aov_.value, ell_.value>,
                                  dim3(band_tiles + 1u), dim3(128), p, band_tiles);
                    return true;
                } else return false;
            },
            eo, lit32 && !p.disc, p.consumed != nullptr, OneOf<1, 2>{ahead == 2 ? 2 : 1}, p.disc != 0, want_aov, ell);
        if (!ok) return ctx_fail(ctx, SPLAT_ERR_INVALID, "k_composite_px: no kernel for this footprint and record format");
        report.launched = hipPeekAtLastError() == hipSuccess;
        LAUNCH_CHECK(ctx, "k_composite_px");
        return SPLAT_OK;
    }
    const bool ok = variant_dispatch(
        [&](auto mode, auto eo_, auto disc, auto lit, auto aov_, auto ell_) {
            if constexpr (composite_variant_exists(mode.value, disc.value, lit.value, aov_.value, ell_.value)) {
                launch_kernel(ctx, SPLAT_STAGE_COMPOSITE, k_composite<mode.value, eo_.value, disc.value, lit.value, aov_.value, ell_.value>,
                              dim3(ntx, r1 - r0), dim3(256), p);
                return true;
            } else return false;
        },
        OneOf<SPLAT_COMPOSITE_FRONT_TO_BACK, SPLAT_COMPOSITE_REFERENCE_LITERAL>{(int)cfg->mode}, eo, p.disc != 0, lit32 && !p.disc, want_aov, ell);
    if (!ok) return ctx_fail(ctx, SPLAT_ERR_INVALID, "k_composite: no kernel for this footprint, record format, blend and outputs");
    report.launched = hipPeekAtLastError() == hipSuccess;
    LAUNCH_CHECK(ctx, "k_composite");
    return SPLAT_OK;
}
```

splat_renderer_amd/csrc/frame.hip:

```cpp
#include "common.h"
#include "tile_range.h"
#include "disc.h"
#include "ellipsoid.h"
#include "shade.h"

#include <cstdlib>

__device__ __forceinline__ uint32_t depth_key_of(float depth) {
    uint32_t bits = __float_as_uint(depth);
    uint32_t mask = ((bits >> 31) == 1u) ? 0xffffffffu : 0x80000000u;
    return bits ^ mask;
}

__global__ __launch_bounds__(256) void k_band_flag(const float4 *__restrict__ projected, uint32_t n, uint32_t width,
                                                   uint32_t height, uint32_t tile, uint32_t ntx, uint32_t nty, uint32_t row0,
                                                   uint32_t row1, uint32_t *__restrict__ flags) {
    uint32_t i = blockIdx.x * 256u + threadIdx.x;
    if (i >= n) return;
    uint32_t a, b, c, d;
    flags[i] = tile_range(projected[(size_t)i * 2], width, height, tile, ntx, nty, row0, row1, a, b, c, d) ? 1u : 0u;
}

__global__ __launch_bounds__(256) void k_band_scatter(const float4 *__restrict__ projected, uint32_t n,
                                                      const uint32_t *__restrict__ slot, const uint32_t *__restrict__ total,
// ... 657 lines not shown
        rc = binner_reserve_range_wide(binner, n);
        if (rc != SPLAT_OK) return rc;
        range_wide = reinterpret_cast<uint2 *>(binner->range32);
    }
    ARG_CHECK(ctx, (((uintptr_t)props | (uintptr_t)projected) & 15) == 0);
    const bool tile_first = fast && frame_order(binner) == SPLAT_FRAME_TILE_FIRST;
    TfHistOut ho = {};
    const bool band_compact = tile_first && bp.skip_outside && band_compacting(row0, row1, nty);
    if (tile_first) {
        rc = binner_reserve(binner, ntx * nty, n);
        if (rc != SPLAT_OK) return rc;
        const uint32_t block = band_compact ? BTC_GROUP : (n <= TF_SMALL_FRAME_SPLATS && !bp.skip_outside) ? TF_BLOCK_SMALL : TF_BLOCK_LARGE;
        ho = {binner->tf_hist, binner->blocksums, binner->d_total + 1, (1u << tile_id_low_bits(ntx * nty)) - 1u, div_up(n, block), block};
        binner->tf_block = block;
        if (band_compact) {
            rc = binner_reserve_band_idx(ctx, binner, n);
            if (rc != SPLAT_OK) return rc;
            ho.cidx = binner->band_idx;
            ho.kept_groups = sorter->hist;
        }
    }
    if (disc && n > binner->discs_cap) {
        HIP_TRY(ctx, hipStreamSynchronize(ctx->stream));
        if (binner->discs) (void)hipFree(binner->discs);
        binner->discs = nullptr;
        binner->discs_cap = 0;
        if (hipMalloc(&binner->discs, (size_t)n * 48 + 256) != hipSuccess) return ctx_fail(ctx, SPLAT_ERR_OOM, "disc records hipMalloc");
        binner->discs_cap = n;
    }
    if (ctx->timing) {
        rc = ctx_ensure_consumed(ctx, ntx * nty);
        if (rc != SPLAT_OK) return rc;
    }
    const LitIO lio = {(const float4 *)color, (const float4 *)normals, color_stride, 1u, cfg->prelit,
                       lit ? (float4 *)projected : disc_lit ? (float4 *)binner->discs : nullptr};
    rc = project_launch(ctx, uniforms, props, pos_stride, n, 0, lit ? nullptr : projected, splat_sort_keys(sorter), nullptr, n, range32, &bp,
                        tile_first ? &ho : nullptr, normals, 1, disc ? binner->discs : nullptr, &lio, range_wide, ell);
    if (rc != SPLAT_OK) return rc;
    binner->tf_hist_ready = tile_first;
    binner->tf_cidx = band_compact ? binner->band_idx : nullptr;
    binner->tf_kept = band_compact ? sorter->hist : nullptr;
    const void *bin_records = projected ? projected : (const void *)binner->discs;
    if (tile_first) {
        sorter->ran = false;
        rc = binner_run(binner, bin_records, n, nullptr, n, width, height, row0, row1, range32, nullptr, sorter->keys);
        if (rc != SPLAT_OK) return rc;
    } else {
        stage_begin(ctx, SPLAT_STAGE_SORT);
        rc = radix_sort_pairs(ctx, sorter->keys, sorter->payload, sorter->keys_b, sorter->payload_b, sorter->hist, n, 0, 32,
                              &sorter->result_in_primary, 0, nullptr, true);
        stage_end(ctx, SPLAT_STAGE_SORT);
        if (rc != SPLAT_OK) return rc;
        sorter->ran = true;
        rc = binner_run(binner, bin_records, n, splat_sort_sorted_payload(sorter), n, width, height, row0, row1, range32, nullptr, nullptr,
                        range_wide);
        if (rc != SPLAT_OK) return rc;
    }
    void *counts = binner->counts, *offsets = binner->offsets;
    void *indices = binner->pairs.result_in_primary ? binner->pairs.payload : binner->pairs.payload_b;
    const void *records = disc ? (n ? (const void *)binner->discs : (projected ? projected : (const void *)counts)) : projected;
    uint32_t *report = binner->report_for_composite;
    binner->report_for_composite = nullptr;
    CompositeArgs a;
    a.color_opacity = color, a.color_stride_vec4 = color_stride;
    a.normals = normals;
    a.projected = records;
    a.tile_indices = indices, a.tile_counts = counts, a.tile_offsets = offsets;
    a.width = width, a.height = height;
    a.out_rgba8 = out_rgba8, a.out_rgba32f = out_rgba32f;
    a.consumed = (ctx->timing && (ctx->timing_mask & SPLAT_TIMING_COUNT_ENTRIES)) ? (void *)ctx->d_consumed : nullptr;
    a.frame_total = binner->d_total, a.report = report, a.report_seq = binner->report_seq;
    a.aov = aov;
    a.ext_z = (disc && !disc_lit && projected) ? (const float *)projected + 4 : nullptr, a.ext_zstride = 8u;
    return composite_launch(ctx, cfg, a);
}

extern "C" {

int splat_render_frame(splat_ctx *ctx, splat_sorter *sorter, splat_binner *binner, const splat_composite_cfg *cfg,
                       const float *uniforms, const void *props, const void *normals, uint32_t n, uint32_t width,
                       uint32_t height, void *projected, void *out_rgba8, void *out_rgba32f) {
    return splat_render_frame_aov(ctx, sorter, binner, cfg, uniforms, props, normals, n, width, height, projected, out_rgba8, out_rgba32f,
                                  nullptr);
}

int splat_render_frame_aov(splat_ctx *ctx, splat_sorter *sorter, splat_binner *binner, const splat_composite_cfg *cfg,
                           const float *uniforms, const void *props, const void *normals, uint32_t n, uint32_t width,
                           uint32_t height, void *projected, void *out_rgba8, void *out_rgba32f, const splat_aov *aov) {
    return render_frame_impl(ctx, sorter, binner, cfg, uniforms, props, 2, props ? (const char *)props + 16 : nullptr, 2, normals, n,
                             width, height, projected, out_rgba8, out_rgba32f, aov);
}

int splat_render_frame_planes(splat_ctx *ctx, splat_sorter *sorter, splat_binner *binner, const splat_composite_cfg *cfg,
                              const float *uniforms, const void *pos_radius, const void *color_opacity, const void *normals,
                              uint32_t n, uint32_t width, uint32_t height, void *projected, void *out_rgba8, void *out_rgba32f) {
    return splat_render_frame_planes_aov(ctx, sorter, binner, cfg, uniforms, pos_radius, color_opacity, normals, n, width, height, projected,
                                         out_rgba8, out_rgba32f, nullptr);
}

int splat_render_frame_planes_aov(splat_ctx *ctx, splat_sorter *sorter, splat_binner *binner, const splat_composite_cfg *cfg,
                                  const float *uniforms, const void *pos_radius, const void *color_opacity, const void *normals,
                                  uint32_t n, uint32_t width, uint32_t height, void *projected, void *out_rgba8, void *out_rgba32f,
                                  const splat_aov *aov) {
    return render_frame_impl(ctx, sorter, binner, cfg, uniforms, pos_radius, 1, color_opacity, 1, normals, n, width, height, projected,
                             out_rgba8, out_rgba32f, aov);
// ... 17 lines not shown
```

splat_renderer_amd/csrc/project.hip:

```cpp
#include "common.h"
#include "variant.h"
#include "tile_range.h"
#include "disc.h"
#include "ellipsoid.h"
#include "shade.h"

struct FrameUniforms {
    float m[16];
    float eye[3];
    float time;
    float w, h;
};

__device__ __forceinline__ void to_screen(const FrameUniforms &u, float x, float y, float z, float &sx, float &sy) {
    float cx = ((u.m[0] * x + u.m[4] * y) + u.m[8] * z) + u.m[12];
    float cy = ((u.m[1] * x + u.m[5] * y) + u.m[9] * z) + u.m[13];
    float cw = ((u.m[3] * x + u.m[7] * y) + u.m[11] * z) + u.m[15];
    float nx = cx / cw, ny = cy / cw;
    sx = ((nx + 1.0f) * 0.5f) * u.w;
    sy = ((1.0f - ny) * 0.5f) * u.h;
}

__device__ __forceinline__ uint32_t depth_key(float depth) {
    uint32_t bits = __float_as_uint(depth);
// ... 47 lines not shown
    const float icw = __builtin_amdgcn_rcpf(cw), iden = __builtin_amdgcn_rcpf(den);
    const float ndx = cx * icw, ndy = cy * icw;
    const float bx = (0.5f * u.w) * (ax + fabsf(ndx) * aw) * iden, by = (0.5f * u.h) * (ay + fabsf(ndy) * aw) * iden;
    const float reach = __builtin_amdgcn_sqrtf(bx * bx + by * by) * (1.5f * 1.001f) + 1.0f;
    const float scy = ((1.0f - ndy) * 0.5f) * u.h;
    const float ts = (float)bp.tile;
    return (scy + reach < (float)bp.row0 * ts - 2.0f) || (scy - reach > (float)bp.row1 * ts + 2.0f);
}

struct SplatIn {
    float4 pr, col, nrm, scl, rot;
};
template <bool DISC, bool LIT, bool ELL = false>
__device__ __forceinline__ SplatIn load_splat(const float4 *__restrict__ pos_radius, uint32_t stride_vec4, uint32_t i, const DiscIO &dio,
                                              const LitIO &lio) {
    SplatIn s;
    s.pr = pos_radius[(size_t)i * stride_vec4];
    s.col = s.nrm = s.scl = s.rot = make_float4(0.0f, 0.0f, 0.0f, 0.0f);
    if (ELL) {
        s.scl = dio.ell.scales[(size_t)i * dio.ell.scale_stride];
        s.rot = dio.ell.rotations[(size_t)i * dio.ell.rot_stride];
    } else if (DISC) s.nrm = dio.normals[(size_t)i * dio.normal_stride];
    if (LIT) {
        s.col = lio.color[(size_t)i * lio.color_stride];
        if (!lio.prelit) s.nrm = lio.normals[(size_t)i * lio.normal_stride];
    }
    return s;
}

template <bool WITH_KEYS, bool WITH_RANGE, bool DISC, bool LIT = false, bool WIDE = false, bool ELL = false>
__device__ __forceinline__ uint32_t project_one(const FrameUniforms &u, const SplatIn &in, uint32_t i, uint32_t index_base,
                                                float4 *__restrict__ projected, uint32_t *__restrict__ keys,
                                                uint32_t *__restrict__ payload, uint32_t *__restrict__ range32, const BinParams &bp,
                                                const DiscIO &dio, const LitIO &lio = LitIO{}, uint32_t kslot = 0xffffffffu) {
    const uint32_t ks = kslot == 0xffffffffu ? i : kslot;
    float4 a, b;
    float depth;
    if (DISC) {
        const float4 pr = in.pr;
        const DiscRecord d = ELL ? ellipsoid_record(u.m, u.w, u.h, pr, in.scl, in.rot) : disc_record(u.m, u.w, u.h, pr, in.nrm);
        dio.discs[(size_t)i * dio.disc_stride] = d.a;
        dio.discs[(size_t)i * dio.disc_stride + 1] = d.b;
        const float dx = pr.x - u.eye[0], dy = pr.y - u.eye[1], dz = pr.z - u.eye[2];
        depth = sqrtf((dx * dx + dy * dy) + dz * dz);
        if (LIT) {
            const float4 lc = (ELL || lio.prelit) ? in.col : lit_color(in.col, in.nrm);
            dio.discs[(size_t)i * dio.disc_stride + 2] = make_float4(lc.x, lc.y, lc.z, depth);
        }
        disc_bounds(d, a);
        b = make_float4(depth, 0.5f * fmaxf(a.z - a.x, a.w - a.y), __uint_as_float(index_base + i), 0.0f);
    } else {
        const float4 c = project_centre(u, in.pr);
        const float scx = c.x, scy = c.y, max_r = c.z;
        depth = c.w;
        float padded = max_r * 1.5f;
        a = make_float4(scx - padded, scy - padded, scx + padded, scy + padded);
        b = make_float4(depth, max_r, __uint_as_float(index_base + i), 0.0f);
        if (LIT) {
            lio.records[(size_t)i * 2] = c;
            lio.records[(size_t)i * 2 + 1] = lio.prelit ? in.col : lit_color(in.col, in.nrm);
        }
    }
    if ((!DISC && !LIT) || projected) {
        projected[(size_t)i * 2] = a;
        projected[(size_t)i * 2 + 1] = b;
    }
    if (WITH_KEYS) {
        keys[ks] = depth_key(depth);
        if (payload) payload[ks] = index_base + i;
    }
    uint32_t packed = 1u;
    if (WITH_RANGE) {
        uint32_t tx0, tx1, ty0, ty1;
        const bool ok = tile_range(a, bp.width, bp.height, bp.tile, bp.ntx, bp.nty, bp.row0, bp.row1, tx0, tx1, ty0, ty1);
        if (WIDE) {
            reinterpret_cast<uint2 *>(range32)[ks] = pack_range_wide(ok, tx0, tx1, ty0, ty1);
        } else {
            packed = pack_range32(ok, tx0, tx1, ty0, ty1);
            range32[ks] = packed;
        }
    }
    return packed;
}

__global__ __launch_bounds__(256) void k_project_compact(FrameUniforms u, const float4 *__restrict__ pos_radius, uint32_t stride_vec4,
                                                         uint32_t n, float4 *__restrict__ records16) {
    const uint32_t i = blockIdx.x * 256u + threadIdx.x;
    if (i < n) records16[i] = project_centre(u, pos_radius[(size_t)i * stride_vec4]);
}

__global__ __launch_bounds__(256) void k_project_disc48(FrameUniforms u, const float4 *__restrict__ pos_radius, uint32_t stride_vec4,
                                                        const float4 *__restrict__ normals, uint32_t normal_stride, uint32_t n,
                                                        float4 *__restrict__ records48) {
    const uint32_t i = blockIdx.x * 256u + threadIdx.x;
    if (i >= n) return;
    const float4 pr = pos_radius[(size_t)i * stride_vec4];
    const DiscRecord d = disc_record(u.m, u.w, u.h, pr, normals[(size_t)i * normal_stride]);
    const float dx = pr.x - u.eye[0], dy = pr.y - u.eye[1], dz = pr.z - u.eye[2];
    records48[(size_t)i * 3] = d.a;
    records48[(size_t)i * 3 + 1] = d.b;
    records48[(size_t)i * 3 + 2] = make_float4(sqrtf((dx * dx + dy * dy) + dz * dz), 0.0f, 0.0f, 0.0f);
// ... 12 lines not shown
template <bool WITH_KEYS, bool WITH_RANGE, bool DISC, bool LIT = false, bool ELL = false>
__global__ __launch_bounds__(256) void k_project(FrameUniforms u, const float4 *__restrict__ pos_radius,
                                                 uint32_t stride_vec4, uint32_t n, uint32_t n_padded, uint32_t index_base,
                                                 float4 *__restrict__ projected, uint32_t *__restrict__ keys,
                                                 uint32_t *__restrict__ payload, uint32_t *__restrict__ range32, BinParams bp,
                                                 DiscIO dio, LitIO lio) {
    uint32_t i = blockIdx.x * 256u + threadIdx.x;
    if (i >= n) {
        if (WITH_KEYS && i < n_padded) {
            keys[i] = 0xffffffffu;
            if (payload) payload[i] = 0xffffffffu;
        }
        return;
    }
    const SplatIn in = load_splat<DISC, LIT, ELL>(pos_radius, stride_vec4, i, dio, lio);
    project_one<WITH_KEYS, WITH_RANGE, DISC, LIT, false, ELL>(u, in, i, index_base, projected, keys, payload, range32, bp, dio, lio);
}

template <bool DISC, bool LIT, bool ELL = false>
__global__ __launch_bounds__(256) void k_project_wide(FrameUniforms u, const float4 *__restrict__ pos_radius, uint32_t stride_vec4,
                                                      uint32_t n, uint32_t n_padded, float4 *__restrict__ projected,
                                                      uint32_t *__restrict__ keys, uint2 *__restrict__ range_wide, BinParams bp,
                                                      DiscIO dio, LitIO lio) {
    const uint32_t i = blockIdx.x * 256u + threadIdx.x;
    if (i >= n) {
        if (i < n_padded) keys[i] = 0xffffffffu;
        return;
    }
    const SplatIn in = load_splat<DISC, LIT, ELL>(pos_radius, stride_vec4, i, dio, lio);
    project_one<true, true, DISC, LIT, true, ELL>(u, in, i, 0, projected, keys, nullptr, reinterpret_cast<uint32_t *>(range_wide), bp, dio,
                                                  lio);
}

template <bool DISC, bool LIT, uint32_t PER, uint32_t AHEAD = 1, bool ELL = false>
__global__ __launch_bounds__(256) void k_project_hist(FrameUniforms u, const float4 *__restrict__ pos_radius, uint32_t stride_vec4,
                                                      uint32_t n, uint32_t n_padded, float4 *__restrict__ projected,
                                                      uint32_t *__restrict__ keys, uint32_t *__restrict__ range32, BinParams bp,
                                                      TfHistOut ho, DiscIO dio, LitIO lio) {
    __shared__ uint32_t lh[4][256];
    __shared__ uint32_t wsum[4];
    const uint32_t tid = threadIdx.x, w = tid >> 6;
    const uint32_t blk = xcd_block_of(blockIdx.x, ho.xcd_per);
    if (blk * (PER * 256u) >= n_padded) return;
    SplatIn in[PER];
#pragma unroll
    for (uint32_t k = 0; k < AHEAD; ++k) {
        const uint32_t i = blk * (PER * 256u) + k * 256u + tid;
        if (i < n) in[k] = load_splat<DISC, LIT, ELL>(pos_radius, stride_vec4, i, dio, lio);
    }
    if (blk == 0 && tid == 0) *ho.overflow_flag = 0;
    for (uint32_t j = tid; j < 4 * 256; j += 256) (&lh[0][0])[j] = 0;
    __syncthreads();
    uint32_t local = 0;
#pragma unroll
    for (uint32_t k = 0; k < PER; ++k) {
        if (k + AHEAD < PER) {
            const uint32_t i = blk * (PER * 256u) + (k + AHEAD) * 256u + tid;
            if (i < n) in[k + AHEAD] = load_splat<DISC, LIT, ELL>(pos_radius, stride_vec4, i, dio, lio);
        }
        const uint32_t i = blk * (PER * 256u) + k * 256u + tid;
        if (i >= n) {
            if (i < n_padded) keys[i] = 0xffffffffu;
            continue;
        }
        const uint32_t r = project_one<true, true, DISC, LIT, false, ELL>(u, in[k], i, 0, projected, keys, nullptr, range32, bp, dio, lio);
        const uint32_t tx0 = r & 0xffu, tx1 = (r >> 8) & 0xffu, ty0 = (r >> 16) & 0xffu, ty1 = r >> 24;
        if (tx0 > tx1 || ty0 > ty1) continue;
        local += hist_add_rect(lh[w], tx0, tx1, ty0, ty1, bp.ntx, ho.mask);
    }
#pragma unroll
    for (int d = 32; d >= 1; d >>= 1) local += __shfl_xor(local, d);
    if ((tid & 63) == 0) wsum[w] = local;
    __syncthreads();
    if (blk < ho.num_parts) {
        if (tid <= ho.mask) ho.hist[(size_t)tid * ho.num_parts + blk] = lh[0][tid] + lh[1][tid] + lh[2][tid] + lh[3][tid];
        if (tid == 0) ho.blocksums[blk] = wsum[0] + wsum[1] + wsum[2] + wsum[3];
    }
}

template <bool DISC, bool LIT>
__global__ __launch_bounds__(256) void k_project_hist_band(FrameUniforms u, const float4 *__restrict__ pos_radius, uint32_t stride_vec4,
                                                           uint32_t n, uint32_t n_padded, float4 *__restrict__ projected,
                                                           uint32_t *__restrict__ keys, uint32_t *__restrict__ range32, BinParams bp,
                                                           TfHistOut ho, DiscIO dio, LitIO lio) {
    __shared__ uint32_t lh[4][256];
    __shared__ uint32_t wsum[4];
    __shared__ uint32_t s_list[1024];
    __shared__ uint32_t s_count;
    const uint32_t tid = threadIdx.x, w = tid >> 6, lane = tid & 63;
    if (blockIdx.x == 0 && tid == 0) *ho.overflow_flag = 0;
    if (tid == 0) s_count = 0;
    for (uint32_t j = tid; j < 4 * 256; j += 256) (&lh[0][0])[j] = 0;
    __syncthreads();
#pragma unroll
    for (uint32_t k = 0; k < 4; ++k) {
        const uint32_t i = blockIdx.x * 1024u + k * 256u + tid;
        bool keep = false;
        if (i < n) {
            const float4 pr = pos_radius[(size_t)i * stride_vec4];
            float r = fabsf(pr.w);
            if (DISC) {
                const float4 nr = dio.normals[(size_t)i * dio.normal_stride];
                r *= fmaxf(1.0f, 1.001f * __builtin_amdgcn_sqrtf((nr.x * nr.x + nr.y * nr.y) + nr.z * nr.z));
            }
            keep = !cannot_reach_band<DISC>(u, pr, r, bp);
            if (!keep) {
                keys[i] = 0xffffffffu;
                range32[i] = 1u;
            }
// ... 143 lines not shown
    if (i >= n) return;
    float4 p = positions[i], c = curvature[i];
    props[(size_t)i * 2] = make_float4(p.x, p.y, p.z, 0.04f);
    props[(size_t)i * 2 + 1] = make_float4(fabsf(c.x) * 0.8f + 0.2f, fabsf(c.y) * 0.8f + 0.2f, fabsf(c.z) * 0.8f + 0.2f, 1.0f);
}

__global__ __launch_bounds__(256) void k_update_props_planes(const float4 *__restrict__ positions,
                                                             const float4 *__restrict__ curvature, uint32_t n,
                                                             float4 *__restrict__ pos_radius, float4 *__restrict__ color_opacity) {
    uint32_t i = blockIdx.x * 256u + threadIdx.x;
    if (i >= n) return;
    float4 p = positions[i], c = curvature[i];
    pos_radius[i] = make_float4(p.x, p.y, p.z, 0.04f);
    color_opacity[i] = make_float4(fabsf(c.x) * 0.8f + 0.2f, fabsf(c.y) * 0.8f + 0.2f, fabsf(c.z) * 0.8f + 0.2f, 1.0f);
}

__global__ __launch_bounds__(256) void k_props_to_planes(const float4 *__restrict__ props, uint32_t n,
                                                         float4 *__restrict__ pos_radius, float4 *__restrict__ color_opacity) {
    uint32_t i = blockIdx.x * 256u + threadIdx.x;
    if (i >= n) return;
    pos_radius[i] = props[(size_t)i * 2];
    color_opacity[i] = props[(size_t)i * 2 + 1];
}

static void load_uniforms(FrameUniforms &u, const float *uniforms) {
    for (int i = 0; i < 16; ++i) u.m[i] = uniforms[i];
    u.eye[0] = uniforms[16]; u.eye[1] = uniforms[17]; u.eye[2] = uniforms[18];
    u.time = uniforms[19]; u.w = uniforms[20]; u.h = uniforms[21];
}

int project_launch(splat_ctx *ctx, const float *uniforms, const void *pos_radius, uint32_t pr_stride_vec4, uint32_t n,
                   uint32_t index_base, void *projected, void *keys, void *payload, uint32_t n_padded, uint32_t *range32,
                   const BinParams *bp, const TfHistOut *hist_out, const void *normals, uint32_t normal_stride_vec4, void *discs,
                   const LitIO *lit, uint2 *range_wide, const EllIO *ell) {
    FrameUniforms u;
    load_uniforms(u, uniforms);
    const uint32_t work = keys ? n_padded : n;
    if (work == 0) return SPLAT_OK;
    BinParams none = {0, 0, 1, 0, 0, 0, 0};
    const float4 *src = (const float4 *)pos_radius + (size_t)index_base * pr_stride_vec4;
    const bool disc = discs != nullptr;
    const bool el = disc && ell != nullptr;
    if (el && hist_out && bp && bp->skip_outside)
        return ctx_fail(ctx, SPLAT_ERR_INVALID, "project_launch: the ellipsoid footprint has no band projector");
    const bool with_lit = lit && lit->records && !disc, disc_lit = lit && lit->records && disc;
    if ((with_lit || disc_lit) && !(keys && (range32 || range_wide) && !payload && index_base == 0))
        return ctx_fail(ctx, SPLAT_ERR_INVALID, "project_launch: lit records are written by the frame's projector only");
    DiscIO dio = {(disc && !el) ? (const float4 *)normals + (size_t)index_base * normal_stride_vec4 : nullptr, normal_stride_vec4,
                  (float4 *)discs, disc_lit ? 3u : 2u, EllIO{}};
    if (el) {
        dio.ell = *ell;
        dio.ell.scales += (size_t)index_base * ell->scale_stride;
        dio.ell.rotations += (size_t)index_base * ell->rot_stride;
    }
    const LitIO lio = (with_lit || disc_lit) ? *lit : LitIO{};
    stage_begin(ctx, SPLAT_STAGE_PROJECT);
    const dim3 block(256);
    const bool lit_out = with_lit || disc_lit;
    const bool frame_keys = keys && !payload && index_base == 0;
    bool ok = false;
    if (hist_out && frame_keys && range32 && bp->skip_outside) {
        TfHistOut ho = *hist_out;
        if (hist_out->cidx) {
            ho.xcd_per = ho.num_parts >= 64u ? div_up(ho.num_parts, 8u) : 0u;
            const dim3 grid(ho.xcd_per ? 8u * ho.xcd_per : ho.num_parts);
            ok = variant_dispatch(
                [&](auto d, auto l) {
                    launch_kernel(ctx, NO_STAGE, k_project_hist_bandc<d.value, l.value>, grid, dim3(PBC_THREADS), u, src, pr_stride_vec4, n,
                                  (float4 *)projected, (uint32_t *)keys, range32, *bp, ho, dio, lio);
                    return true;
                },
                disc, lit_out);
        } else {
            ok = variant_dispatch(
                [&](auto d, auto l) {
                    launch_kernel(ctx, NO_STAGE, k_project_hist_band<d.value, l.value>, dim3(div_up(work, 1024)), block, u, src, pr_stride_vec4, n,
                                  n_padded, (float4 *)projected, (uint32_t *)keys, range32, *bp, ho, dio, lio);
                    return true;
                },
                disc, lit_out);
        }
    } else if (hist_out && frame_keys && range32) {
        TfHistOut ho = *hist_out;
        const bool small = hist_out->block == TF_BLOCK_SMALL;
        const uint32_t blocks = div_up(work, small ? 256u : 1024u);
        ho.xcd_per = blocks >= 64u ? div_up(blocks, 8u) : 0u;
        const dim3 grid(ho.xcd_per ? 8u * ho.xcd_per : blocks);
        ok = variant_dispatch(
            [&](auto d, auto l, auto per, auto e) {
                if constexpr (d.value || !e.value) {
                    launch_kernel(ctx, NO_STAGE, k_project_hist<d.value, l.value, per.value, 1, e.value>, grid, block, u, src, pr_stride_vec4, n,
                                  n_padded, (float4 *)projected, (uint32_t *)keys, range32, *bp, ho, dio, lio);
                    return true;
                } else return false;
            },
            disc, lit_out, OneOf<1, 4>{small ? 1 : 4}, el);
    } else if (frame_keys && range_wide) {
        ok = variant_dispatch(
            [&](auto d, auto l, auto e) {
                if constexpr (d.value || !e.value) {
                    launch_kernel(ctx, NO_STAGE, k_project_wide<d.value, l.value, e.value>, dim3(div_up(work, 256)), block, u, src, pr_stride_vec4, n,
                                  n_padded, (float4 *)projected, (uint32_t *)keys, range_wide, *bp, dio, lio);
                    return true;
                } else return false;
            },
            disc, lit_out, el);
    } else {
        const bool with_keys = keys != nullptr, with_range = keys && range32;
        ok = variant_dispatch(
            [&](auto k, auto r, auto d, auto l, auto e) {
                if constexpr ((k.value || !r.value) && (r.value || !l.value) && (d.value || !e.value)) {
                    launch_kernel(ctx, NO_STAGE, k_project<k.value, r.value, d.value, l.value, e.value>, dim3(div_up(work, 256)), block, u, src,
                                  pr_stride_vec4, n, with_keys ? n_padded : n, index_base, (float4 *)projected, (uint32_t *)keys,
                                  (uint32_t *)payload, with_range ? range32 : nullptr, with_range ? *bp : none, dio, lio);
                    return true;
                } else return false;
            },
            with_keys, with_range, disc, with_range && lit_out, el);
    }
    if (!ok) return ctx_fail(ctx, SPLAT_ERR_INVALID, "project_launch: no kernel for this footprint and these outputs");
    LAUNCH_CHECK(ctx, "k_project");
    stage_end(ctx, SPLAT_STAGE_PROJECT);
    return SPLAT_OK;
}

extern "C" {

int splat_project(splat_ctx *ctx, const float *uniforms, const void *pos_radius, uint32_t pr_stride_vec4, uint32_t n,
                  void *projected, void *keys, void *payload, uint32_t n_padded) {
// ... 134 lines not shown
```

splat_renderer_amd/csrc/tile_first.hip:

```cpp
#include "common.h"
#include "tile_range.h"

constexpr uint32_t TF_THREADS = 256;
constexpr uint32_t TF_STAGE = 4096;
static_assert(TF_BLOCK_LARGE == 1024 && TF_BLOCK_SMALL == 256, "the stage word packs the block-local slot in 10 bits; blocks are 256 x {4, 1}");

__device__ __forceinline__ uint32_t range32_hits(uint32_t r) {
    const uint32_t tx0 = r & 0xffu, tx1 = (r >> 8) & 0xffu, ty0 = (r >> 16) & 0xffu, ty1 = r >> 24;
    return (tx0 > tx1 || ty0 > ty1) ? 0u : (tx1 - tx0 + 1) * (ty1 - ty0 + 1);
}

constexpr uint32_t TS_THREADS = 256, TS_WAVES = 4;
constexpr uint32_t TS_LONG_ITEMS = 24;
constexpr uint32_t TS_LDS_ELEMS = 5888;
constexpr uint32_t TS_CHUNK_ITEMS = 16;

struct TileSortShared {
    uint32_t wave_hist[TS_WAVES][256];
    uint32_t digit_base[256];
    uint32_t wave_sums[TS_WAVES];
    uint32_t kmin, kmax;
};

template <bool RANK_ATOMIC>
// ... 22 lines not shown
    wave_hist[2][tid] = c0 + c1;
    wave_hist[3][tid] = c0 + c1 + c2;
    return c0 + c1 + c2 + c3;
}

__device__ __forceinline__ uint32_t ts_scan256(uint32_t *wave_sums, uint32_t v, uint32_t tid) {
    const uint32_t lane = tid & 63, w = tid >> 6;
    uint32_t incl = v;
#pragma unroll
    for (int s = 1; s < 64; s <<= 1) {
        const uint32_t t = __shfl_up(incl, s);
        if ((int)lane >= s) incl += t;
    }
    if (lane == 63) wave_sums[w] = incl;
    __syncthreads();
    const uint32_t wprefix = (w > 0 ? wave_sums[0] : 0u) + (w > 1 ? wave_sums[1] : 0u) + (w > 2 ? wave_sums[2] : 0u);
    __syncthreads();
    return wprefix + incl - v;
}

constexpr uint32_t TFS_ITEMS = TF_STAGE / TF_THREADS;

struct TfScatterShared {
    uint32_t wave_hist[TS_WAVES][256];
    uint32_t digit_base[256];
    uint32_t global_base[256];
    uint32_t wave_sums[TS_WAVES];
};

#ifndef TF_SCATTER_WAVES
#define TF_SCATTER_WAVES 5
#endif
constexpr uint32_t TF_GROUP = 4096;
template <bool RANK_ATOMIC, uint32_t TF_PER_THREAD, bool COMPACTED = false>
__global__ __launch_bounds__(TF_THREADS, TF_SCATTER_WAVES) void k_tf_scatter(const uint32_t *__restrict__ range32,
                                                           const uint32_t *__restrict__ depth_keys, uint32_t n, uint32_t ntx,
                                                           uint32_t mask, uint32_t num_parts,
                                                           const uint32_t *__restrict__ scanned_hist,
                                                           const uint32_t *__restrict__ totals, uint32_t *__restrict__ d_total,
                                                           uint32_t pair_limit, uint32_t *__restrict__ overflow,
                                                           uint8_t *__restrict__ out_hi, uint2 *__restrict__ out_val,
                                                           uint32_t lo_bits, uint32_t align_m1, TfRuns runs,
                                                           uint32_t *__restrict__ offsets_out, uint32_t tiles, uint32_t *report,
                                                           uint32_t seq, const uint32_t *__restrict__ cidx,
                                                           const uint32_t *__restrict__ kept, uint32_t xcd_per) {
    static_assert(!COMPACTED || TF_PER_THREAD == 4, "compacted groups are read four splats per thread");
    const uint32_t blk = xcd_block_of(blockIdx.x, xcd_per);
    if (blk >= num_parts) return;
    __shared__ TfScatterShared sh;
    __shared__ uint32_t wsum[4];
    __shared__ uint32_t stage[TF_STAGE];
    __shared__ uint32_t s_key[TF_THREADS * TF_PER_THREAD];
    __shared__ uint32_t s_idx[COMPACTED ? TF_THREADS * TF_PER_THREAD : 1];
    const uint32_t tid = threadIdx.x, lane = tid & 63, w = tid >> 6;
    uint32_t first = blk * (COMPACTED ? TF_GROUP : TF_THREADS * TF_PER_THREAD);
    if (COMPACTED) n = first + min(kept[blk], TF_GROUP);
    static_assert(TF_PER_THREAD == 4 || TF_PER_THREAD == 1, "uint4 or scalar loads");
    uint32_t i0 = first + tid * TF_PER_THREAD;
    uint4 rr = make_uint4(1u, 1u, 1u, 1u), kk = make_uint4(0, 0, 0, 0);
    if (TF_PER_THREAD == 1) {
        if (i0 < n) { rr.x = range32[i0]; kk.x = depth_keys[i0]; }
    } else if (i0 + 3 < n) {
        rr = reinterpret_cast<const uint4 *>(range32)[i0 >> 2];
        kk = reinterpret_cast<const uint4 *>(depth_keys)[i0 >> 2];
    } else {
        if (i0 < n) { rr.x = range32[i0]; kk.x = depth_keys[i0]; }
        if (i0 + 1 < n) { rr.y = range32[i0 + 1]; kk.y = depth_keys[i0 + 1]; }
        if (i0 + 2 < n) { rr.z = range32[i0 + 2]; kk.z = depth_keys[i0 + 2]; }
    }
    const uint32_t digit_total = totals[tid];
    const uint32_t row_prefix = tid <= mask ? scanned_hist[(size_t)tid * num_parts + blk] : 0u;

    const uint32_t digit_room = (digit_total + align_m1) & ~align_m1;
    uint32_t gincl = digit_total, aincl = digit_room;
    unsigned long long g64 = digit_total;
#pragma unroll
    for (int s = 1; s < 64; s <<= 1) {
        const uint32_t t = __shfl_up(gincl, s), a = __shfl_up(aincl, s);
        const unsigned long long t64 = __shfl_up(g64, s);
        if ((int)lane >= s) {
            gincl += t;
            aincl += a;
            g64 += t64;
        }
    }
    __shared__ unsigned long long wsum64[4];
    if (lane == 63) {
        sh.wave_sums[w] = gincl;
        wsum[w] = aincl;
        wsum64[w] = g64;
    }
    __syncthreads();
    const uint32_t aprefix = (w > 0 ? wsum[0] : 0u) + (w > 1 ? wsum[1] : 0u) + (w > 2 ? wsum[2] : 0u);
    const unsigned long long all_pairs64 = wsum64[0] + wsum64[1] + wsum64[2] + wsum64[3];
    const uint32_t all_pairs = all_pairs64 > 0xffffffffull ? 0xffffffffu : (uint32_t)all_pairs64;
    const uint32_t run_start = aprefix + aincl - digit_room;
    if (blk == 0) {
        const bool fits = all_pairs <= pair_limit;
        if (tid == 0) {
            d_total[0] = all_pairs;
            d_total[2] = fits ? all_pairs : 0u;
            d_total[3] = 0u;
            if (!fits) atomicOr(overflow, 1u);
        }
        runs.start[tid] = fits ? run_start : 0u;
        runs.total[tid] = fits ? digit_total : 0u;
        if (align_m1 && fits)
            for (uint32_t j = 0, first_part = run_start / (align_m1 + 1u); j < digit_room / (align_m1 + 1u); ++j)
                runs.part_digit[first_part + j] = (uint8_t)tid;
        if (tid == 255) *runs.parts = (align_m1 && fits) ? (run_start + digit_room) / (align_m1 + 1u) : 0u;
        if (offsets_out) {
            if (tid < tiles) offsets_out[tid] = fits ? run_start : 0u;
            if (tid == 0) {
                offsets_out[tiles] = fits ? all_pairs : 0u;
                if (report) tile_report(d_total, report, seq);
            }
        }
    }
    if (all_pairs > pair_limit) return;
    sh.global_base[tid] = run_start + row_prefix;
    for (;;) {
    __syncthreads();

    uint32_t r[TF_PER_THREAD], h[TF_PER_THREAD];
    if constexpr (TF_PER_THREAD == 4) {
        reinterpret_cast<uint4 *>(s_key)[tid] = kk;
        r[0] = rr.x; r[1] = rr.y; r[2] = rr.z; r[3] = rr.w;
        if constexpr (COMPACTED) {
            uint4 ii = make_uint4(0, 0, 0, 0);
            if (i0 + 3 < n) ii = reinterpret_cast<const uint4 *>(cidx)[i0 >> 2];
            else {
                if (i0 < n) ii.x = cidx[i0];
                if (i0 + 1 < n) ii.y = cidx[i0 + 1];
                if (i0 + 2 < n) ii.z = cidx[i0 + 2];
            }
            reinterpret_cast<uint4 *>(s_idx)[tid] = ii;
        }
    } else {
        s_key[tid] = kk.x;
        r[0] = rr.x;
    }
#pragma unroll
    for (uint32_t k = 0; k < TF_PER_THREAD; ++k) h[k] = range32_hits(r[k]);
    uint32_t off[TF_PER_THREAD];
    uint32_t carry;
    {
        uint32_t mine = 0;
#pragma unroll
        for (uint32_t k = 0; k < TF_PER_THREAD; ++k) mine += h[k];
        uint32_t incl = mine;
#pragma unroll
        for (int d = 1; d < 64; d <<= 1) {
// ... 569 lines not shown
}

int tf_second_pass_launch(splat_ctx *ctx, const uint8_t *hi, const uint2 *val_in, uint2 *val_out, const TfRuns *runs, uint32_t pairs_bound,
                          uint32_t tiles, uint32_t lo_bits, uint32_t hi_bits, uint32_t *hist, uint32_t *offsets, const uint32_t *d_total) {
    const uint32_t num_parts = tf2_parts_bound(pairs_bound, lo_bits);
    uint32_t *totals = hist + (size_t)256 * num_parts;
    if (hi_bits > 0) {
        const uint32_t hmask = (1u << hi_bits) - 1u;
        const uint32_t xcd_per = num_parts >= 64u ? div_up(num_parts, 8u) : 0u;
        const uint32_t part_blocks = xcd_per ? 8u * xcd_per : num_parts;
        hipLaunchKernelGGL(k_tf_upsweep2, dim3(part_blocks), dim3(TF_THREADS), 0, ctx->stream, hi, *runs, hmask, num_parts, hist, xcd_per);
        LAUNCH_CHECK(ctx, "k_tf_upsweep2");
        int rc = radix_rowscan_launch(ctx, hist, num_parts, hmask + 1u);
        if (rc != SPLAT_OK) return rc;
        const TfOffsetsArgs off = {tiles, lo_bits, offsets, d_total};
        const dim3 grid(part_blocks + div_up(tiles + 1, 256));
        const bool ra = rank_atomic_ok(ctx, true);
        const uint32_t pad = hi_bits >= 8u ? 4096u : 0u;
        if (ra)
            hipLaunchKernelGGL((k_tf_downsweep2<true, 4>), grid, dim3(TF_THREADS), pad, ctx->stream, hi, val_in, val_out, *runs, hmask, num_parts, hist,
                               totals, off, part_blocks, xcd_per);
        else
            hipLaunchKernelGGL((k_tf_downsweep2<false, 4>), grid, dim3(TF_THREADS), pad, ctx->stream, hi, val_in, val_out, *runs, hmask, num_parts, hist,
                               totals, off, part_blocks, xcd_per);
        LAUNCH_CHECK(ctx, "k_tf_downsweep2");
    }
    return SPLAT_OK;
}

int tf_scatter_launch(splat_ctx *ctx, const uint32_t *range32, const uint32_t *depth_keys, uint32_t n, uint32_t ntx, uint32_t mask,
                      const uint32_t *hist, uint32_t *d_total, uint32_t pair_limit, uint32_t *overflow, uint8_t *out_hi,
                      uint2 *out_val, uint32_t block_splats, uint32_t lo_bits, bool second_pass, const TfRuns *runs,
                      uint32_t *offsets_if_final, uint32_t tiles, uint32_t *report, uint32_t seq, const uint32_t *cidx,
                      const uint32_t *kept) {
    const uint32_t parts = div_up(n, block_splats);
    const uint32_t xcd_per = parts >= 64u ? div_up(parts, 8u) : 0u;
    const uint32_t grid_blocks = xcd_per ? 8u * xcd_per : parts;
    if (cidx && block_splats != TF_GROUP) return ctx_fail(ctx, SPLAT_ERR_INVALID, "tf_scatter_launch: compacted input comes in groups of 4096 records");
    const uint32_t *totals = hist + (size_t)256 * parts;
    {
        int prc = ctx_resolve_rank_mode(ctx);
        if (prc != SPLAT_OK) return prc;
    }
    const bool ra = rank_atomic_ok(ctx, true);
#define SPLAT_TF_SCATTER_(RA, PER, COMPACTED)                                                                                     \
    hipLaunchKernelGGL((k_tf_scatter<RA, PER, COMPACTED>), dim3(grid_blocks), dim3(TF_THREADS), 0, ctx->stream, range32, depth_keys, n, ntx, mask, parts, \
                       hist, totals, d_total, pair_limit, overflow, out_hi, out_val, lo_bits, second_pass ? TF_RUN_ALIGN - 1u : 0u, *runs,         \
                       second_pass ? nullptr : offsets_if_final, tiles, report, seq, cidx, kept, xcd_per)
#define SPLAT_TF_SCATTER(RA, PER) SPLAT_TF_SCATTER_(RA, PER, false)
    if (cidx) {
        if (ra) SPLAT_TF_SCATTER_(true, 4, true);
        else SPLAT_TF_SCATTER_(false, 4, true);
    } else if (block_splats == TF_BLOCK_SMALL) {
        if (ra) SPLAT_TF_SCATTER(true, 1);
        else SPLAT_TF_SCATTER(false, 1);
    } else {
        if (ra) SPLAT_TF_SCATTER(true, 4);
        else SPLAT_TF_SCATTER(false, 4);
    }
#undef SPLAT_TF_SCATTER
#undef SPLAT_TF_SCATTER_
    LAUNCH_CHECK(ctx, "k_tf_scatter");
    return SPLAT_OK;
}
```

splat_renderer_amd/dist.py:

```python
import ctypes as C

import numpy as np

from . import _lib
from ._lib import CompositeCfg, check

TILE = 16
REC_FLOATS = 4
DISC_REC_FLOATS = 12


def shard_size(n, world):
    return -(-n // world)


def slice_range(n, rank, world):
    per = shard_size(n, world)
    first = min(rank * per, n)
    return first, min(per, n - first)


def band_rows(nty, rank, world):
    return nty * rank // world, nty * (rank + 1) // world

# ... 24 lines not shown
        if normals_ptr is None:
            raise ValueError("the oriented-disc projector needs the normals")
        check(lib.splat_project_slice_disc(ctx, up, props_ptr, 2, normals_ptr, 1, first, count, out_records.data_ptr()), ctx)
    else:
        check(lib.splat_project_slice_compact(ctx, up, props_ptr, 2, first, count, out_records.data_ptr()), ctx)


class HipStages:

    def __init__(self, torch, device_ordinal, n_total_padded, width, height, tile=TILE, mode=_lib.MODE_FRONT_TO_BACK,
                 early_out=True, footprint="isotropic"):
        self.torch = torch
        if footprint not in ("isotropic", "disc"):
            raise ValueError(f"footprint must be 'isotropic' or 'disc', not {footprint!r}")
        self.disc = footprint == "disc"
        self.rec_floats = DISC_REC_FLOATS if self.disc else REC_FLOATS
        self.lib = _lib.load()
        self.ordinal = device_ordinal
        p = C.c_void_p()
        stream = torch.cuda.current_stream().cuda_stream
        check(self.lib.splat_ctx_create_on_stream(device_ordinal, C.c_void_p(stream), C.byref(p)))
        self.ctx = p
        s = C.c_void_p()
        check(self.lib.splat_sort_create(self.ctx, n_total_padded, C.byref(s)), self.ctx)
        self.sorter = s
        b = C.c_void_p()
        check(self.lib.splat_bin_create(self.ctx, tile, C.byref(b)), self.ctx)
        self.binner = b
        self.width, self.height, self.tile = width, height, tile
        self.mode, self.early_out = mode, early_out
        self.pairs = 0
        self.overflows = 0
        self.misranked = 0
        self.consumed = None
        self.lit = None
        self.pos_plane = None
        self.local_projected = None

    def _again(self, rc):
        if rc == _lib.ERR_RETRY:
            self.misranked += 1
        else:
            self.overflows += 1

    def rank_status(self):
        pol, ordered, faults = C.c_int(), C.c_int(), C.c_uint32()
        check(self.lib.splat_rank_status(self.ctx, C.byref(pol), C.byref(ordered), C.byref(faults)), self.ctx)
        return {"policy": ("checked", "atomic", "ballot")[pol.value], "atomicsOrdered": bool(ordered.value == 1),
                "orderFaults": int(faults.value)}

    def set_lit(self, props_ptr, normals_ptr, n):
        if self.lit is None or self.lit.shape[0] != n:
            self.lit = self.torch.empty((n, 4), dtype=self.torch.float32, device=f"cuda:{self.ordinal}")
        check(self.lib.splat_lit_colors(self.ctx, props_ptr + 16, 2, normals_ptr, 1, n, self.lit.data_ptr()), self.ctx)
        if self.pos_plane is None or self.pos_plane.shape[0] != n:
            self.pos_plane = self.torch.empty((n, 4), dtype=self.torch.float32, device=f"cuda:{self.ordinal}")
        scratch = self.torch.empty((n, 4), dtype=self.torch.float32, device=f"cuda:{self.ordinal}")
        check(self.lib.splat_props_to_planes(self.ctx, props_ptr, n, self.pos_plane.data_ptr(), scratch.data_ptr()), self.ctx)
        check(self.lib.splat_sync(self.ctx), self.ctx)

    def set_timing(self, enabled, stage_mask=0xFFFFFFFF):
        check(self.lib.splat_set_timing_stages(self.ctx, stage_mask), self.ctx)
        check(self.lib.splat_set_timing(self.ctx, int(enabled)), self.ctx)

    def stage_avg_ms(self, stage):
        cnt, tot = C.c_uint32(), C.c_double()
        check(self.lib.splat_stage_time_stats(self.ctx, stage, C.byref(cnt), C.byref(tot)), self.ctx)
        return tot.value / max(cnt.value, 1)

    def row_pairs(self):
        ntx, nty = -(-self.width // self.tile), -(-self.height // self.tile)
        counts = C.c_void_p()
        check(self.lib.splat_bin_counts(self.binner, C.byref(counts)), self.ctx)
        host = np.empty(ntx * nty, np.uint32)
# ... 255 lines not shown
```

splat_renderer_amd/host.py:

```python
import ctypes as C

import numpy as np

from . import _lib
from ._lib import CompositeCfg, SplatError, check

U32_MAX = 0xFFFFFFFF


class Buffer:

    def __init__(self, device, ptr, size, owned=True):
        self.device, self.ptr, self.size, self._owned = device, ptr, int(size), owned
        self._host_shadow = None

    def destroy(self):
        if self._owned and self.ptr:
            check(self.device.lib.splat_buf_free(self.device.ctx, self.ptr), self.device.ctx)
        self.ptr = None

    def write(self, array, offset=0):
        a = np.ascontiguousarray(array)
        if offset + a.nbytes > self.size:
            raise ValueError("write past the end of the buffer")
# ... 477 lines not shown
        n_sorted = numSplats if numSorted is None else numSorted
        check(d.lib.splat_bin_run(self._b, projectedBuffer.ptr, numSplats, sortedIndicesBuffer.ptr, n_sorted, screenWidth,
                                  screenHeight, tileRow0, tileRow1), d.ctx)
        self._tiles = -(-screenWidth // self.tileSize) * -(-screenHeight // self.tileSize)
        d.lastBinner = self

    def _get(self, fn, size):
        p = C.c_void_p()
        rc = fn(self._b, C.byref(p))
        if rc != 0:
            raise SplatError(rc, self.device.lib.splat_last_error(self.device.ctx).decode())
        return Buffer(self.device, p.value, size, owned=False)

    def getTileOffsetsBuffer(self):
        return self._get(self.device.lib.splat_bin_offsets, self._tiles * 4)

    def getTileIndicesBuffer(self):
        buf = self._get(self.device.lib.splat_bin_indices, 4)
        buf.size = max(self.getTotalIndices(), 1) * 4
        return buf

    def getTileCountsBuffer(self):
        return self._get(self.device.lib.splat_bin_counts, self._tiles * 4)

    def getTotalIndices(self):
        t = C.c_uint64()
        check(self.device.lib.splat_bin_total(self._b, C.byref(t)), self.device.ctx)
        return int(t.value)

    def setFrameOrder(self, order):
        code = {"default": -1, "sortFirst": 0, "tileFirst": 1}[order] if isinstance(order, str) else int(order)
        check(self.device.lib.splat_bin_set_frame_order(self._b, code), self.device.ctx)

    def getTileSize(self):
        return self.tileSize

    def cleanupTempBuffers(self):
        self.prefixSumScanner.cleanupTempBuffers()

    def destroy(self):
        if self.device.lastBinner is self:
            self.device.lastBinner = None
        if self._b:
            self.device.lib.splat_bin_destroy(self._b)
            self._b = None


class PerTileSorter:

    def __init__(self, device, validate=False):
        self.device, self.validate = device, validate
        self.violations = 0

    def sort(self, commandEncoder, projectedBuffer, tileListsBuffer, tileOffsetsBuffer, splatIndicesBuffer, numTiles,
             maxSplatsPerTile, totalPairs=None):
        if not self.validate:
            return None
        d = self.device
        if totalPairs is None:
            totalPairs = splatIndicesBuffer.size // 4
        v = C.c_uint64()
        check(d.lib.splat_validate_tile_order(d.ctx, projectedBuffer.ptr, tileOffsetsBuffer.ptr, numTiles,
                                              splatIndicesBuffer.ptr, totalPairs, C.byref(v)), d.ctx)
        self.violations = int(v.value)
        return self.violations

# ... 188 lines not shown
        return self.compositor.readPixelsFloat()

    def destroy(self):
        self.projector.destroy()
        self.binner.destroy()
        self.compositor.destroy()


class Renderer:

    def __init__(self, device, context=None, presentationFormat="rgba8unorm", numPoints=0, tileSize=16,
                 mode=_lib.MODE_FRONT_TO_BACK, earlyOut=True, frameOrder=None, footprint="isotropic", writeProjected=True,
                 records="lit"):
        self.footprint = _footprint(footprint)
        if not writeProjected and self.footprint == _lib.FOOTPRINT_ISOTROPIC:
            raise SplatError(-1, "writeProjected=False: the isotropic composite reads the records the projector writes")
        if records not in ("lit", "lit-always", "projected"):
            raise SplatError(-1, f"records must be 'lit', 'lit-always' or 'projected', not {records!r}")
        self.records = records
        self.writeProjected = writeProjected
        self.device, self.numPoints, self.tileSize = device, numPoints, tileSize
        self.projector = SplatProjector(device, numPoints)
        self.sorter = RadixSorter(device, numPoints)
        self.binner = GPUTileBinner(device, tileSize)
        if frameOrder is not None:
            self.binner.setFrameOrder(frameOrder)
        self.mode, self.earlyOut = mode, earlyOut
        self.output = None
        self.outputFloat = None
        self._wh = (0, 0)
        self._last = None
        self.previousFrameOverflowed = False
        self.framesMisranked = 0
        self.aov = _AovBuffers(device)

    def _again(self, rc):
        if rc == _lib.ERR_RETRY:
            self.framesMisranked += 1
        else:
            self.previousFrameOverflowed = True

    def render(self, uniformData, propertyBuffer, normalsBuffer, scaleFactorsBuffer, width, height, tileRows=(0, U32_MAX),
               wantFloat=False, wantAov=False):
        d = self.device
        u = _uniform_floats(uniformData).copy()
        if u.shape[0] < 22:
            u = np.concatenate([u[:20], np.array([width, height], np.float32)])
        if self._wh != (width, height):
            if self.output:
                self.output.destroy()
            if self.outputFloat:
                self.outputFloat.destroy()
                self.outputFloat = None
            self.output = d.createBuffer(width * height * 4)
            self._wh = (width, height)
        if wantFloat and self.outputFloat is None:
            self.outputFloat = d.createBuffer(width * height * 16)
        ell = self.footprint == _lib.FOOTPRINT_ELLIPSOID
        if ell != isinstance(propertyBuffer, GaussianCloud):
            raise SplatError(-1, "Renderer(footprint='ellipsoid') renders a GaussianCloud, and only it renders one")
        if ell and (normalsBuffer is not None or propertyBuffer.n > self.numPoints):
            raise SplatError(-1, "an ellipsoid frame takes no normals, and at most numPoints splats")
        prelit = ell or (isinstance(propertyBuffer, PropertyPlanes) and propertyBuffer.prelit)
        ts = self.tileSize
        lit = self.records == "lit-always" or (self.records == "lit" and -(-width // ts) <= 256 and -(-height // ts) <= 256)
        frame_format = self.frameRecordFormat = _lib.RECORDS_LIT32 if lit else _lib.RECORDS_PROJECTED
        iso_lit = lit and self.footprint == _lib.FOOTPRINT_ISOTROPIC
        self.recordFormat = _lib.RECORDS_LIT32 if iso_lit else _lib.RECORDS_PROJECTED
        self.projector.contents = "lit" if iso_lit else "projected"
        cfg = CompositeCfg(self.mode, int(self.earlyOut), self.tileSize, tileRows[0], tileRows[1], frame_format, int(prelit),
                           self.footprint)
# ... 167 lines not shown
```

splat_renderer_amd/napi/splat_napi.c:

```c
#define NAPI_VERSION 6
#include <node_api.h>
#include <stdint.h>
#include <stdlib.h>
#include <string.h>

#include "../../include/splat.h"

#define MAX_ARGS 18

typedef struct {
    napi_env env;
    size_t argc;
    napi_value argv[MAX_ARGS];
    int failed;
} call_t;

static int get_args(napi_env env, napi_callback_info info, call_t *c, size_t want) {
    c->env = env;
    c->argc = MAX_ARGS;
    c->failed = 0;
    if (napi_get_cb_info(env, info, &c->argc, c->argv, NULL, NULL) != napi_ok || c->argc < want) {
        napi_throw_type_error(env, NULL, "wrong number of arguments");
        return 0;
    }
// ... 57 lines not shown
    napi_value r;
    napi_create_double(env, v, &r);
    return r;
}

static napi_value mk_undefined(napi_env env) {
    napi_value r;
    napi_get_undefined(env, &r);
    return r;
}

static napi_value mk_external(napi_env env, void *p) {
    napi_value r;
    napi_create_external(env, p, NULL, NULL, &r);
    return r;
}

static napi_value check(napi_env env, splat_ctx *ctx, int rc, napi_value ok) {
    if (rc == SPLAT_OK) return ok;
    char msg[600];
    const char *m = splat_last_error(ctx);
    strcpy(msg, "libsplat_hip ");
    char num[16];
    int n = rc, k = 0;
    if (n < 0) { msg[strlen(msg) + 1] = 0; msg[strlen(msg)] = '-'; n = -n; }
    do { num[k++] = (char)('0' + n % 10); n /= 10; } while (n);
    while (k) { size_t l = strlen(msg); msg[l] = num[--k]; msg[l + 1] = 0; }
    strcat(msg, ": ");
    strncat(msg, m ? m : "", sizeof msg - strlen(msg) - 1);
    napi_throw_error(env, NULL, msg);
    return NULL;
}

#define AGAIN(rc) ((rc) == SPLAT_ERR_CAPACITY || (rc) == SPLAT_ERR_RETRY)

#define FN(name) static napi_value name(napi_env env, napi_callback_info info)
#define ARGS(n) call_t c; if (!get_args(env, info, &c, n)) return NULL
#define BAIL if (c.failed) return NULL

FN(abi_version) { (void)info; return mk_number(env, splat_abi_version()); }

FN(ctx_create) {
    ARGS(1);
    int dev = (int)arg_number(&c, 0); BAIL;
    splat_ctx *ctx = NULL;
    int rc = splat_ctx_create(dev, &ctx);
    return check(env, NULL, rc, rc == SPLAT_OK ? mk_external(env, ctx) : NULL);
}
FN(ctx_destroy) { ARGS(1); splat_ctx_destroy((splat_ctx *)arg_external(&c, 0)); return mk_undefined(env); }
FN(sync) { ARGS(1); splat_ctx *x = arg_external(&c, 0); BAIL; return check(env, x, splat_sync(x), mk_undefined(env)); }
FN(rank_status) {
    ARGS(1); splat_ctx *x = arg_external(&c, 0); BAIL;
    int pol = 0, ordered = 0; uint32_t faults = 0;
    int rc = splat_rank_status(x, &pol, &ordered, &faults);
    if (rc != SPLAT_OK) return check(env, x, rc, NULL);
    napi_value arr;
    if (napi_create_array_with_length(env, 3, &arr) != napi_ok) return NULL;
    napi_set_element(env, arr, 0, mk_number(env, pol));
    napi_set_element(env, arr, 1, mk_number(env, ordered));
    napi_set_element(env, arr, 2, mk_number(env, (double)faults));
    return arr;
}
FN(set_timing) { ARGS(2); splat_ctx *x = arg_external(&c, 0); int e = (int)arg_number(&c, 1); BAIL; return check(env, x, splat_set_timing(x, e), mk_undefined(env)); }
FN(stage_time_ms) {
    ARGS(2); splat_ctx *x = arg_external(&c, 0); int st = (int)arg_number(&c, 1); BAIL;
    float ms = 0; int rc = splat_stage_time_ms(x, st, &ms);
    return check(env, x, rc, mk_number(env, ms));
// ... 41 lines not shown
    return check(env, x, splat_project(x, u, pr, st, n, proj, keys, pay, np), mk_undefined(env));
}
FN(project_disc) {
    ARGS(12); splat_ctx *x = arg_external(&c, 0); size_t ub = 0; float *u = arg_hostbuf(&c, 1, &ub);
    void *pr = arg_dptr(&c, 2); uint32_t st = (uint32_t)arg_number(&c, 3); void *nrm = arg_dptr(&c, 4);
    uint32_t ns = (uint32_t)arg_number(&c, 5), n = (uint32_t)arg_number(&c, 6);
    void *proj = arg_dptr(&c, 7), *discs = arg_dptr(&c, 8), *keys = arg_dptr(&c, 9), *pay = arg_dptr(&c, 10); uint32_t np = (uint32_t)arg_number(&c, 11); BAIL;
    if (ub < 22 * sizeof(float)) { napi_throw_range_error(env, NULL, "uniform block needs 22 floats"); return NULL; }
    return check(env, x, splat_project_disc(x, u, pr, st, nrm, ns, n, proj, discs, keys, pay, np), mk_undefined(env));
}
FN(extract_keys) {
    ARGS(6); splat_ctx *x = arg_external(&c, 0); void *proj = arg_dptr(&c, 1); uint32_t n = (uint32_t)arg_number(&c, 2), np = (uint32_t)arg_number(&c, 3);
    void *k = arg_dptr(&c, 4), *p = arg_dptr(&c, 5); BAIL;
    return check(env, x, splat_extract_keys(x, proj, n, np, k, p), mk_undefined(env));
}
FN(sort_create) {
    ARGS(2); splat_ctx *x = arg_external(&c, 0); uint32_t cap = (uint32_t)arg_number(&c, 1); BAIL;
    splat_sorter *s = NULL; int rc = splat_sort_create(x, cap, &s);
    return check(env, x, rc, rc == SPLAT_OK ? mk_external(env, s) : NULL);
}
FN(sort_destroy) { ARGS(1); splat_sort_destroy(arg_external(&c, 0)); return mk_undefined(env); }
FN(sort_capacity) { ARGS(1); return mk_number(env, splat_sort_capacity(arg_external(&c, 0))); }
FN(sort_keys) { ARGS(1); return mk_number(env, (double)(uintptr_t)splat_sort_keys(arg_external(&c, 0))); }
FN(sort_payload) { ARGS(1); return mk_number(env, (double)(uintptr_t)splat_sort_payload(arg_external(&c, 0))); }
FN(sort_sorted_payload) { ARGS(1); return mk_number(env, (double)(uintptr_t)splat_sort_sorted_payload(arg_external(&c, 0))); }
FN(sort_sorted_keys) { ARGS(1); return mk_number(env, (double)(uintptr_t)splat_sort_sorted_keys(arg_external(&c, 0))); }
FN(sort_run) {
    ARGS(5); splat_ctx *x = arg_external(&c, 0); splat_sorter *s = arg_external(&c, 1);
    uint32_t n = (uint32_t)arg_number(&c, 2), b0 = (uint32_t)arg_number(&c, 3), b1 = (uint32_t)arg_number(&c, 4); BAIL;
    return check(env, x, splat_sort_run(s, n, b0, b1), mk_undefined(env));
}
FN(sort_set_mode) { ARGS(3); splat_ctx *x = arg_external(&c, 0); splat_sorter *s = arg_external(&c, 1); int m = (int)arg_number(&c, 2); BAIL; return check(env, x, splat_sort_set_mode(s, m), mk_undefined(env)); }
FN(bin_set_frame_order) { ARGS(3); splat_ctx *x = arg_external(&c, 0); splat_binner *b = arg_external(&c, 1); int o = (int)arg_number(&c, 2); BAIL; return check(env, x, splat_bin_set_frame_order(b, o), mk_undefined(env)); }
FN(scan_u32) {
    ARGS(5); splat_ctx *x = arg_external(&c, 0); void *in = arg_dptr(&c, 1), *out = arg_dptr(&c, 2); uint32_t n = (uint32_t)arg_number(&c, 3);
    void *tot = arg_dptr(&c, 4); BAIL;
    return check(env, x, splat_scan_u32(x, in, out, n, tot), mk_undefined(env));
}
FN(bin_create) {
    ARGS(2); splat_ctx *x = arg_external(&c, 0); uint32_t t = (uint32_t)arg_number(&c, 1); BAIL;
    splat_binner *b = NULL; int rc = splat_bin_create(x, t, &b);
    return check(env, x, rc, rc == SPLAT_OK ? mk_external(env, b) : NULL);
}
FN(bin_destroy) { ARGS(1); splat_bin_destroy(arg_external(&c, 0)); return mk_undefined(env); }
FN(bin_run) {
    ARGS(10); splat_ctx *x = arg_external(&c, 0); splat_binner *b = arg_external(&c, 1); void *proj = arg_dptr(&c, 2);
    uint32_t ns = (uint32_t)arg_number(&c, 3); void *sorted = arg_dptr(&c, 4); uint32_t nso = (uint32_t)arg_number(&c, 5);
    uint32_t w = (uint32_t)arg_number(&c, 6), h = (uint32_t)arg_number(&c, 7), r0 = (uint32_t)arg_number(&c, 8), r1 = (uint32_t)arg_number(&c, 9); BAIL;
    return check(env, x, splat_bin_run(b, proj, ns, sorted, nso, w, h, r0, r1), mk_undefined(env));
}
#define BIN_GETTER(jsname, cfn)                                                                        \
    FN(jsname) {                                                                                       \
        ARGS(2); splat_ctx *x = arg_external(&c, 0); splat_binner *b = arg_external(&c, 1); BAIL;      \
        void *p = NULL; int rc = cfn(b, &p);                                                           \
        return check(env, x, rc, mk_number(env, (double)(uintptr_t)p));                                \
    }
BIN_GETTER(bin_counts, splat_bin_counts)
BIN_GETTER(bin_offsets, splat_bin_offsets)
BIN_GETTER(bin_indices, splat_bin_indices)
FN(bin_total) {
    ARGS(2); splat_ctx *x = arg_external(&c, 0); splat_binner *b = arg_external(&c, 1); BAIL;
    uint64_t t = 0; int rc = splat_bin_total(b, &t);
    return check(env, x, rc, mk_number(env, (double)t));
}
FN(validate_tile_order) {
    ARGS(6); splat_ctx *x = arg_external(&c, 0); void *proj = arg_dptr(&c, 1), *off = arg_dptr(&c, 2); uint32_t nt = (uint32_t)arg_number(&c, 3);
// ... 490 lines not shown
    uint32_t n = (uint32_t)arg_number(&c, 3), w = (uint32_t)arg_number(&c, 4), h = (uint32_t)arg_number(&c, 5), t = (uint32_t)arg_number(&c, 6);
    uint32_t r0 = (uint32_t)arg_number(&c, 7), r1 = (uint32_t)arg_number(&c, 8); BAIL;
    uint32_t kept = 0;
    int rc = splat_band_keys(x, s, proj, n, w, h, t, r0, r1, &kept);
    return check(env, x, rc, rc == SPLAT_OK ? mk_number(env, kept) : NULL);
}
FN(band_kept) {
    ARGS(2); splat_ctx *x = arg_external(&c, 0); splat_sorter *s = arg_external(&c, 1); BAIL;
    uint32_t kept = 0;
    int rc = splat_band_kept(x, s, &kept);
    return check(env, x, rc, rc == SPLAT_OK ? mk_number(env, kept) : NULL);
}
FN(comm_rank) {
    ARGS(1); splat_comm *cm = arg_external(&c, 0); BAIL;
    int r = 0, w = 0;
    int rc = splat_comm_rank(cm, &r, &w);
    return rc == SPLAT_OK ? mk_pair(env, r, w) : check(env, NULL, rc, NULL);
}
FN(comm_count) {
    ARGS(1); splat_comm *cm = arg_external(&c, 0); BAIL;
    int n = 0, r = 0;
    int rc = splat_comm_count(cm, &n, &r);
    return rc == SPLAT_OK ? mk_pair(env, n, r) : check(env, NULL, rc, NULL);
}

static napi_value init(napi_env env, napi_value exports) {
#define EXPORT(name) { #name, NULL, name, NULL, NULL, NULL, napi_enumerable, NULL }
    napi_property_descriptor d[] = {
        EXPORT(abi_version), EXPORT(ctx_create), EXPORT(ctx_destroy), EXPORT(sync), EXPORT(rank_status), EXPORT(set_timing), EXPORT(stage_time_ms),
        EXPORT(buf_alloc), EXPORT(buf_free), EXPORT(buf_zero), EXPORT(buf_upload), EXPORT(buf_download), EXPORT(update_props), EXPORT(update_props_planes), EXPORT(props_to_planes), EXPORT(lit_colors),
        EXPORT(project), EXPORT(project_disc), EXPORT(extract_keys), EXPORT(sort_create), EXPORT(sort_destroy), EXPORT(sort_capacity), EXPORT(sort_keys),
        EXPORT(sort_payload), EXPORT(sort_sorted_payload), EXPORT(sort_sorted_keys), EXPORT(sort_run), EXPORT(sort_set_mode),
        EXPORT(scan_u32), EXPORT(bin_create), EXPORT(bin_destroy), EXPORT(bin_run), EXPORT(bin_counts), EXPORT(bin_offsets),
        EXPORT(bin_indices), EXPORT(bin_total), EXPORT(bin_set_frame_order), EXPORT(validate_tile_order), EXPORT(composite), EXPORT(render_frame), EXPORT(render_frame_planes),
        EXPORT(composite_aov), EXPORT(render_frame_aov), EXPORT(render_frame_planes_aov),
        EXPORT(project_slice_compact), EXPORT(band_frame), EXPORT(band_settle), EXPORT(comm_unique_id), EXPORT(comm_init), EXPORT(comm_destroy),
        EXPORT(ctx_create_on_stream), EXPORT(last_error), EXPORT(set_timing_stages), EXPORT(set_timing_sampling), EXPORT(stage_time_stats), EXPORT(timing_consumed),
        EXPORT(buf_copy), EXPORT(probe_lds_atomic_order),
        EXPORT(composite_forget_history), EXPORT(composite_options), EXPORT(bin_dims), EXPORT(bin_tile_size), EXPORT(project_slice),
        EXPORT(project_slice_disc), EXPORT(expand_compact), EXPORT(band_keys), EXPORT(band_kept), EXPORT(comm_rank), EXPORT(comm_count),
        EXPORT(allgather_records), EXPORT(sdf_gradients), EXPORT(sdf_update_positions), EXPORT(sdf_scale_factors), EXPORT(sdf_curvature), EXPORT(sdf_seed_positions), EXPORT(sdf_generate),
        EXPORT(point_frame), EXPORT(project_ellipsoid), EXPORT(sh_colors), EXPORT(render_frame_ellipsoids),
        EXPORT(composite_backward), EXPORT(project_ellipsoid_backward), EXPORT(sh_colors_backward),
        EXPORT(composite_aov_depth), EXPORT(composite_backward_depth), EXPORT(project_ellipsoid_backward_depth),
        EXPORT(project_ellipsoid_backward_camera), EXPORT(sh_colors_backward_camera),
        EXPORT(image_loss_workspace_bytes), EXPORT(image_loss), EXPORT(image_loss_backward),
        EXPORT(adam_step), EXPORT(density_accumulate), EXPORT(densify_plan_workspace_bytes), EXPORT(densify_plan),
        EXPORT(densify_geometry), EXPORT(densify_rows),
        EXPORT(mcmc_sample_workspace_bytes), EXPORT(mcmc_sample), EXPORT(mcmc_apply), EXPORT(mcmc_noise),
    };
    napi_define_properties(env, exports, sizeof d / sizeof d[0], d);
    return exports;
}

NAPI_MODULE(NODE_GYP_MODULE_NAME, init)
```

Baseline: 15600.

## Bin only pairs in front of previous frame's per-tile depth cuts

Adds a temporal depth-cut mode. Per-tile depth cuts from the previous frame are dilated into neighbourhood max tables, and the scatter kernel drops splats masked as lying behind them, so fewer tile pairs are binned and sorted. If a tile's composite walk goes past its cut, the frame returns CUT_SHORT and is re-rendered with full binning. Full lists can also be rebuilt on demand when callers ask for bin buffers. This adds cut-table kernels, a mask buffer and a possible re-render, and it is enabled through an env var or setter.

```diff
diff --git a/include/splat.h b/include/splat.h
--- a/include/splat.h
+++ b/include/splat.h
@@ -19,6 +19,7 @@
 #define SPLAT_ERR_NO_DEVICE (-6)
 #define SPLAT_ERR_COMM (-7)
 #define SPLAT_ERR_RETRY (-8)
+#define SPLAT_ERR_CUT_SHORT (-9)
 
 typedef struct splat_ctx splat_ctx;
 typedef struct splat_sorter splat_sorter;
@@ -109,6 +110,8 @@
 int splat_bin_offsets(splat_binner *b, void **dptr);
 int splat_bin_indices(splat_binner *b, void **dptr);
 int splat_bin_total(splat_binner *b, uint64_t *total_pairs);
+int splat_bin_set_depth_cut(splat_binner *b, int on);
+int splat_bin_cut_stats(splat_binner *b, uint64_t *pairs_binned, uint64_t *pairs_full, uint32_t *frames_short);
 #define SPLAT_FRAME_ORDER_DEFAULT (-1)
 #define SPLAT_FRAME_SORT_FIRST 0
 #define SPLAT_FRAME_TILE_FIRST 1
diff --git a/splat_renderer_amd/_lib.py b/splat_renderer_amd/_lib.py
--- a/splat_renderer_amd/_lib.py
+++ b/splat_renderer_amd/_lib.py
@@ -5,9 +5,9 @@
 LIB_PATH = os.environ.get("SPLAT_LIB_PATH") or os.path.join(_HERE, "libsplat_hip.so")
 
 OK = 0
-ERR_NAMES = {-1: "INVALID", -2: "HIP", -3: "OOM", -4: "CAPACITY", -5: "STATE", -6: "NO_DEVICE", -7: "COMM", -8: "RETRY"}
-ERR_CAPACITY, ERR_RETRY = -4, -8
-RENDER_AGAIN = (ERR_CAPACITY, ERR_RETRY)
+ERR_NAMES = {-1: "INVALID", -2: "HIP", -3: "OOM", -4: "CAPACITY", -5: "STATE", -6: "NO_DEVICE", -7: "COMM", -8: "RETRY", -9: "CUT_SHORT"}
+ERR_CAPACITY, ERR_RETRY, ERR_CUT_SHORT = -4, -8, -9
+RENDER_AGAIN = (ERR_CAPACITY, ERR_RETRY, ERR_CUT_SHORT)
 
 STAGE_PROJECT, STAGE_SORT, STAGE_BIN, STAGE_COMPOSITE, STAGE_EXCHANGE, STAGE_BIN_SCATTER, STAGE_BIN_PASS2, STAGE_BIN_TILE_SORT = range(8)
 STAGE_NAMES = ("project", "sort", "bin", "composite", "exchange", "bin_scatter", "bin_second_pass", "bin_tile_sort")
@@ -136,6 +136,8 @@
     "splat_bin_indices": (_i, [_vp, _pvp]),
     "splat_bin_total": (_i, [_vp, C.POINTER(C.c_uint64)]),
     "splat_bin_set_frame_order": (_i, [_vp, _i]),
+    "splat_bin_set_depth_cut": (_i, [_vp, _i]),
+    "splat_bin_cut_stats": (_i, [_vp, C.POINTER(C.c_uint64), C.POINTER(C.c_uint64), C.POINTER(_u32)]),
     "splat_bin_dims": (_i, [_vp, C.POINTER(_u32), C.POINTER(_u32)]),
     "splat_validate_tile_order": (_i, [_vp, _vp, _vp, _u32, _vp, C.c_uint64, C.POINTER(C.c_uint64)]),
     "splat_lit_colors": (_i, [_vp, _vp, _u32, _vp, _u32, _u32, _vp]),
diff --git a/splat_renderer_amd/csrc/bin.hip b/splat_renderer_amd/csrc/bin.hip
--- a/splat_renderer_amd/csrc/bin.hip
+++ b/splat_renderer_amd/csrc/bin.hip
@@ -211,6 +211,93 @@
     if (sa > sb || (sa == sb && a >= b)) atomicAdd(violations, 1ull);
 }
 
+__global__ __launch_bounds__(256) void k_cut_tables(const uint32_t *__restrict__ cuts, uint32_t ntx, uint32_t nty, uint32_t *__restrict__ dil,
+                                                    uint32_t *__restrict__ m2, uint32_t *__restrict__ m4, uint32_t *__restrict__ state) {
+    const uint32_t t = blockIdx.x * 256u + threadIdx.x;
+    if (t == 0) state[0] = state[1] = state[2] = 0u;
+    if (t >= ntx * nty) return;
+    const uint32_t tx = t % ntx, ty = t / ntx;
+    const uint32_t x0 = tx ? tx - 1u : 0u, y0 = ty ? ty - 1u : 0u;
+    uint32_t d = 0, a2 = 0, a4 = 0;
+    for (uint32_t y = y0; y <= min(ty + 4u, nty - 1u); ++y)
+        for (uint32_t x = x0; x <= min(tx + 4u, ntx - 1u); ++x) {
+            const uint32_t c = cuts[y * ntx + x];
+            a4 = max(a4, c);
+            if (x <= tx + 2u && y <= ty + 2u) a2 = max(a2, c);
+            if (x <= tx + 1u && y <= ty + 1u) d = max(d, c);
+        }
+    dil[t] = d;
+    m2[t] = a2;
+    m4[t] = a4;
+}
+
+template <uint32_t PER>
+__global__ __launch_bounds__(256) void k_range_hist(const uint32_t *__restrict__ range32, uint32_t n, uint32_t ntx, uint32_t mask,
+                                                    uint32_t num_parts, uint32_t *__restrict__ hist, uint32_t *__restrict__ blocksums,
+                                                    uint32_t *__restrict__ overflow_flag) {
+    __shared__ uint32_t lh[4][256];
+    __shared__ uint32_t wsum[4];
+    const uint32_t tid = threadIdx.x, w = tid >> 6, blk = blockIdx.x;
+    if (blk == 0 && tid == 0) *overflow_flag = 0;
+    for (uint32_t j = tid; j < 4 * 256; j += 256) (&lh[0][0])[j] = 0;
+    __syncthreads();
+    uint32_t local = 0;
+#pragma unroll
+    for (uint32_t k = 0; k < PER; ++k) {
+        const uint32_t i = blk * (PER * 256u) + k * 256u + tid;
+        if (i >= n) continue;
+        const uint32_t r = range32[i];
+        const uint32_t tx0 = r & 0xffu, tx1 = (r >> 8) & 0xffu, ty0 = (r >> 16) & 0xffu, ty1 = r >> 24;
+        if (tx0 > tx1 || ty0 > ty1) continue;
+        local += hist_add_rect(lh[w], tx0, tx1, ty0, ty1, ntx, mask);
+    }
+#pragma unroll
+    for (int d = 32; d >= 1; d >>= 1) local += __shfl_xor(local, d);
+    if ((tid & 63) == 0) wsum[w] = local;
+    __syncthreads();
+    if (blk < num_parts) {
+        if (tid <= mask) hist[(size_t)tid * num_parts + blk] = lh[0][tid] + lh[1][tid] + lh[2][tid] + lh[3][tid];
+        if (tid == 0) blocksums[blk] = wsum[0] + wsum[1] + wsum[2] + wsum[3];
+    }
+}
+
+__global__ void k_bin_report(const uint32_t *d_total, uint32_t *report, uint32_t seq) { tile_report(d_total, report, seq); }
+
+static void binner_free_cut(splat_binner *b) {
+    if (b->cut_tables) (void)hipFree(b->cut_tables);
+    if (b->cut_mask) (void)hipFree(b->cut_mask);
+    if (b->cut_state) (void)hipFree(b->cut_state);
+    b->cut_tables = b->cut_state = nullptr;
+    b->cut_mask = nullptr;
+    b->cut_tiles_cap = b->cut_mask_cap = 0;
+}
+
+int binner_cut_begin(splat_binner *b, const uint32_t *prev_cuts, uint32_t ntx, uint32_t nty, uint32_t n_splats) {
+    splat_ctx *ctx = b->ctx;
+    const uint32_t tiles = ntx * nty;
+    b->cut = CutFrame{};
+    if (tiles > b->cut_tiles_cap || n_splats > b->cut_mask_cap || !b->cut_state) {
+        HIP_TRY(ctx, hipStreamSynchronize(ctx->stream));
+        const uint32_t tc = tiles > b->cut_tiles_cap ? tiles : b->cut_tiles_cap, sc = n_splats > b->cut_mask_cap ? n_splats : b->cut_mask_cap;
+        binner_free_cut(b);
+        if (hipMalloc((void **)&b->cut_tables, (size_t)tc * 12 + 16) != hipSuccess ||
+            hipMalloc((void **)&b->cut_mask, ((size_t)div_up(sc, 64) + 1) * 8) != hipSuccess ||
+            hipMalloc((void **)&b->cut_state, 32) != hipSuccess) {
+            binner_free_cut(b);
+            return ctx_fail(ctx, SPLAT_ERR_OOM, "binner hipMalloc (depth cut)");
+        }
+        b->cut_tiles_cap = tc;
+        b->cut_mask_cap = sc;
+    }
+    uint32_t *dil = b->cut_tables, *m2 = dil + b->cut_tiles_cap, *m4 = m2 + b->cut_tiles_cap;
+    hipLaunchKernelGGL(k_cut_tables, dim3(div_up(tiles, 256)), dim3(256), 0, ctx->stream, prev_cuts, ntx, nty, dil, m2, m4, b->cut_state);
+    LAUNCH_CHECK(ctx, "k_cut_tables");
+    b->cut.dil = dil, b->cut.m2 = m2, b->cut.m4 = m4;
+    b->cut.mask = b->cut_mask;
+    b->cut.state = b->cut_state;
+    return SPLAT_OK;
+}
+
 static void binner_free(splat_binner *b) {
     if (b->counts) (void)hipFree(b->counts);
     if (b->offsets) (void)hipFree(b->offsets);
@@ -311,6 +398,10 @@
     b->tf_hist_ready = false;
     b->tf_cidx = nullptr;
     b->tf_kept = nullptr;
+    const CutFrame cutf = b->cut;
+    b->cut = CutFrame{};
+    b->lists_cut = false;
+    const bool cut_frame = cutf.mask != nullptr && tile_first;
     ARG_CHECK(ctx, width >= 1 && height >= 1);
     ARG_CHECK(ctx, n_sorted == 0 || (projected && (sorted || tile_first)));
     ARG_CHECK(ctx, !tile_first || (range32 && n_sorted == n_splats && !n_sorted_dev));
@@ -385,7 +476,7 @@
         stage_begin(ctx, SPLAT_STAGE_BIN_SCATTER);
         rc = tf_scatter_launch(ctx, range32, depth_keys, n_splats, ntx, (1u << tf_lo_bits) - 1u, b->tf_hist, b->d_total, b->pair_limit,
                                b->d_total + 1, b->tf_hi, b->wide_a, b->tf_block, tf_lo_bits, tf_hi_bits > 0, &b->tf_runs, b->offsets, tiles,
-                               nullptr, 0u, tf_cidx, tf_kept);
+                               nullptr, 0u, tf_cidx, tf_kept, cut_frame ? cutf.mask : nullptr);
         stage_end(ctx, SPLAT_STAGE_BIN_SCATTER);
         if (rc != SPLAT_OK) return rc;
         const bool primary = tf_hi_bits == 0;
@@ -397,8 +488,9 @@
         const uint32_t band_tiles = tile_row1 > tile_row0 ? (tile_row1 - tile_row0) * ntx : 1u;
         const uint64_t band_key = ((uint64_t)tile_row0 << 48) ^ ((uint64_t)tile_row1 << 32) ^ tiles;
         stage_begin(ctx, SPLAT_STAGE_BIN_TILE_SORT);
+        const uint64_t mean_pairs = (cut_frame && b->cut_last_binned) ? b->cut_last_binned : b->total;
         rc = tile_sort_launch(ctx, b->offsets, tiles, primary ? b->wide_a : b->wide_b, primary ? b->wide_b : b->wide_a, b->pairs.payload,
-                              b->counts, b->d_total + 1, band_tiles >= 6144u ? (uint32_t)(b->total / band_tiles) : 0u, band_tiles,
+                              b->counts, b->d_total + 1, band_tiles >= 6144u ? (uint32_t)(mean_pairs / band_tiles) : 0u, band_tiles,
                               (async && b->last_band_key == band_key) ? b->last_long_tiles : 0xffffffffu, &b->last_short_class);
         stage_end(ctx, SPLAT_STAGE_BIN_TILE_SORT);
         if (rc != SPLAT_OK) return rc;
@@ -408,6 +500,8 @@
         b->report_for_composite = b->pinned_dev;
         b->report_seq = ++b->seq;
         b->pending = true;
+        b->pending_cut = cut_frame;
+        b->lists_cut = cut_frame;
     } else if (total32 > 0) {
         hipLaunchKernelGGL(k_bin_expand, dim3(blocks), dim3(BIN_THREADS), 0, ctx->stream, (const uint32_t *)sorted, n_sorted,
                            b->ranges, b->blocksums, ntx, b->pair_limit, b->d_total + 1, b->pairs.keys, b->pairs.payload);
@@ -425,6 +519,12 @@
         hipLaunchKernelGGL(k_tile_counts, dim3(div_up(tiles, 256)), dim3(256), 0, ctx->stream, b->offsets, tiles, b->counts);
         LAUNCH_CHECK(ctx, "k_tile_counts");
         if (async) b->pending = true;
+    } else if (cut_frame) {
+        stage_end(ctx, SPLAT_STAGE_BIN);
+        b->have_last = false;
+        b->cut_skip_next = true;
+        b->cut_frames_short++;
+        return ctx_fail(ctx, SPLAT_ERR_CUT_SHORT, "every pair of this frame lies behind the previous frame's depth cuts: render it again");
     } else {
         HIP_TRY(ctx, hipMemsetAsync(b->counts, 0, (size_t)tiles * 4, ctx->stream));
         HIP_TRY(ctx, hipMemsetAsync(b->offsets, 0, (size_t)(tiles + 1) * 4, ctx->stream));
@@ -434,6 +534,10 @@
         }
     }
     stage_end(ctx, SPLAT_STAGE_BIN);
+    if (tile_first) {
+        b->cut_n = n_splats, b->cut_w = width, b->cut_h = height;
+        b->cut_keys = depth_keys;
+    }
     b->ran = true;
     return SPLAT_OK;
 }
@@ -465,9 +569,16 @@
     const uint32_t total = ((volatile uint32_t *)b->pinned)[0], flags = ((volatile uint32_t *)b->pinned)[1];
     b->last_long_tiles = b->pending_tile_first ? ((volatile uint32_t *)b->pinned)[3] : 0xffffffffu;
     b->pending_tile_first = false;
-    b->last_total = total;
+    const bool was_cut = b->pending_cut;
+    b->pending_cut = false;
+    uint32_t full = total;
+    if (was_cut && ((volatile uint32_t *)b->pinned)[4] > total) full = ((volatile uint32_t *)b->pinned)[4];
+    b->cut_pairs_binned = total;
+    b->cut_pairs_full = full;
+    b->cut_last_binned = was_cut ? (total ? total : 1u) : 0u;
+    b->last_total = full;
     b->have_last = true;
-    b->total = total;
+    b->total = full;
     if (flags & FRAME_FLAG_ORDER) {
         b->ran = false;
         ctx->order_faults++;
@@ -479,8 +590,18 @@
                         "the previous frame's tile lists failed the order check (ranking with returning LDS atomics was not in lane "
                         "order): the context now ranks with ballots; render that frame again");
     }
+    if (was_cut && (flags & FRAME_FLAG_CUT_SHORT)) {
+        b->ran = false;
+        b->lists_cut = false;
+        b->have_last = false;
+        b->cut_skip_next = true;
+        b->cut_frames_short++;
+        return ctx_fail(ctx, SPLAT_ERR_CUT_SHORT,
+                        "the previous frame was binned in front of per-tile depth cuts and a tile's walk went past its cut: render "
+                        "that frame again (it will be binned in full)");
+    }
     if ((flags & FRAME_FLAG_OVERFLOW) || total > b->pair_limit) {
-        uint64_t want = (uint64_t)total + total / 2 + 8192;
+        uint64_t want = (uint64_t)full + full / 2 + 8192;
         if (want > 0x3ffff000ull) want = 0x3ffff000ull;
         b->ran = false;
         int rc = sorter_reserve(&b->pairs, (uint32_t)want);
@@ -492,7 +613,49 @@
     return SPLAT_OK;
 }
 
+static int binner_complete(splat_binner *b) {
+    int rc = binner_settle(b);
+    if (rc != SPLAT_OK || !b->lists_cut || !b->ran) return rc;
+    splat_ctx *ctx = b->ctx;
+    b->lists_cut = false;
+    const uint32_t n = b->cut_n, parts = div_up(n, b->tf_block), lo_mask = (1u << tile_id_low_bits(b->ntx * b->nty)) - 1u;
+    if (b->tf_block == TF_BLOCK_SMALL)
+        hipLaunchKernelGGL(k_range_hist<1>, dim3(parts), dim3(256), 0, ctx->stream, b->range32, n, b->ntx, lo_mask, parts, b->tf_hist, b->blocksums,
+                           b->d_total + 1);
+    else
+        hipLaunchKernelGGL(k_range_hist<4>, dim3(parts), dim3(256), 0, ctx->stream, b->range32, n, b->ntx, lo_mask, parts, b->tf_hist, b->blocksums,
+                           b->d_total + 1);
+    LAUNCH_CHECK(ctx, "k_range_hist");
+    b->tf_hist_ready = true;
+    const bool allow_async = b->allow_async;
+    b->allow_async = false;
+    rc = binner_run(b, b->range32, n, nullptr, n, b->cut_w, b->cut_h, 0, b->nty, b->range32, nullptr, b->cut_keys);
+    b->allow_async = allow_async;
+    if (b->report_for_composite) {
+        hipLaunchKernelGGL(k_bin_report, dim3(1), dim3(1), 0, ctx->stream, b->d_total, b->report_for_composite, b->report_seq);
+        b->report_for_composite = nullptr;
+        (void)hipGetLastError();
+    }
+    if (rc != SPLAT_OK) return rc;
+    return binner_settle(b);
+}
+
 extern "C" {
+
+int splat_bin_set_depth_cut(splat_binner *b, int on) {
+    if (!b) return ctx_fail(nullptr, SPLAT_ERR_INVALID, "binner is NULL");
+    b->cut_on = on != 0;
+    return SPLAT_OK;
+}
+
+int splat_bin_cut_stats(splat_binner *b, uint64_t *pairs_binned, uint64_t *pairs_full, uint32_t *frames_short) {
+    if (!b) return ctx_fail(nullptr, SPLAT_ERR_INVALID, "binner is NULL");
+    if (int rc = binner_settle(b)) return rc;
+    if (pairs_binned) *pairs_binned = b->cut_pairs_binned;
+    if (pairs_full) *pairs_full = b->cut_pairs_full;
+    if (frames_short) *frames_short = b->cut_frames_short;
+    return SPLAT_OK;
+}
 
 #ifdef SPLAT_TEST_HOOKS
 int splat_debug_rerun_tile_sort(splat_ctx *ctx, splat_binner *b) {
@@ -514,7 +677,7 @@
     b->ctx = ctx;
     b->tile = tile_size;
     b->pairs.ctx = ctx;
-    if (hipMalloc((void **)&b->d_total, 32) != hipSuccess || hipHostMalloc((void **)&b->pinned, 16, hipHostMallocMapped | hipHostMallocCoherent) != hipSuccess ||
+    if (hipMalloc((void **)&b->d_total, 32) != hipSuccess || hipHostMalloc((void **)&b->pinned, 32, hipHostMallocMapped | hipHostMallocCoherent) != hipSuccess ||
         hipHostGetDevicePointer((void **)&b->pinned_dev, b->pinned, 0) != hipSuccess ||
         hipEventCreateWithFlags(&b->readback_done, hipEventDisableTiming) != hipSuccess) {
         if (b->d_total) (void)hipFree(b->d_total);
@@ -522,8 +685,9 @@
         delete b;
         return ctx_fail(ctx, SPLAT_ERR_OOM, "binner allocation");
     }
-    memset(b->pinned, 0, 16);
+    memset(b->pinned, 0, 32);
     if (const char *e = getenv("SPLAT_BIN_SYNC")) b->allow_async = !(e[0] == '1');
+    if (const char *e = getenv("SPLAT_DEPTH_CUT")) b->cut_on = !(e[0] == '0');
     *out = b;
     return SPLAT_OK;
 }
@@ -536,6 +700,7 @@
     if (b->d_total) (void)hipFree(b->d_total);
     if (b->range32) (void)hipFree(b->range32);
     binner_free_wide(b);
+    binner_free_cut(b);
     if (b->expanded) (void)hipFree(b->expanded);
     if (b->discs) (void)hipFree(b->discs);
     if (b->points) (void)hipFree(b->points);
@@ -562,7 +727,7 @@
 
 int splat_bin_counts(splat_binner *b, void **dptr) {
     if (!b || !dptr) return ctx_fail(nullptr, SPLAT_ERR_INVALID, "binner/dptr is NULL");
-    if (int rc = binner_settle(b)) return rc;
+    if (int rc = binner_complete(b)) return rc;
     if (!b->ran) return ctx_fail(b->ctx, SPLAT_ERR_STATE, "Tile counts buffer not initialized");
     *dptr = b->counts;
     return SPLAT_OK;
@@ -570,7 +735,7 @@
 
 int splat_bin_offsets(splat_binner *b, void **dptr) {
     if (!b || !dptr) return ctx_fail(nullptr, SPLAT_ERR_INVALID, "binner/dptr is NULL");
-    if (int rc = binner_settle(b)) return rc;
+    if (int rc = binner_complete(b)) return rc;
     if (!b->ran) return ctx_fail(b->ctx, SPLAT_ERR_STATE, "Tile offsets buffer not initialized");
     *dptr = b->offsets;
     return SPLAT_OK;
@@ -578,7 +743,7 @@
 
 int splat_bin_indices(splat_binner *b, void **dptr) {
     if (!b || !dptr) return ctx_fail(nullptr, SPLAT_ERR_INVALID, "binner/dptr is NULL");
-    if (int rc = binner_settle(b)) return rc;
+    if (int rc = binner_complete(b)) return rc;
     if (!b->ran) return ctx_fail(b->ctx, SPLAT_ERR_STATE, "Tile indices buffer not initialized");
     *dptr = b->pairs.result_in_primary ? b->pairs.payload : b->pairs.payload_b;
     return SPLAT_OK;
diff --git a/splat_renderer_amd/csrc/common.h b/splat_renderer_amd/csrc/common.h
--- a/splat_renderer_amd/csrc/common.h
+++ b/splat_renderer_amd/csrc/common.h
@@ -19,6 +19,8 @@
     uint32_t *mem = nullptr;
     uint32_t cap = 0, parity = 0, streak = 0;
     uint64_t last_use = 0;
+    uint32_t *cut_mem = nullptr;
+    uint32_t cut_cap = 0, cut_parity = 0, cut_streak = 0;
 };
 constexpr int PX_HISTORIES = 4;
 
@@ -99,6 +101,22 @@
     return ctx->rank_policy == RANK_ATOMIC || checked;
 }
 constexpr uint32_t FRAME_FLAG_OVERFLOW = 1u, FRAME_FLAG_ORDER = 2u;
+constexpr uint32_t FRAME_FLAG_CUT_SHORT = 4u;
+
+constexpr uint32_t NOCUT = 0xffffffffu;
+constexpr uint32_t CUT_M_DEFAULT = 2;
+struct CutFrame {
+    const uint32_t *dil = nullptr;
+    const uint32_t *m2 = nullptr;
+    const uint32_t *m4 = nullptr;
+    unsigned long long *mask = nullptr;
+    uint32_t *state = nullptr;
+};
+static inline uint64_t px_history_key(uint32_t ntx, uint32_t r0, uint32_t r1, uint32_t width, const void *tile_counts) {
+    return (((uint64_t)ntx << 40) ^ ((uint64_t)r0 << 20) ^ (uint64_t)r1 ^ ((uint64_t)width << 50) ^
+            ((uint64_t)(uintptr_t)tile_counts * 0x9E3779B97F4A7C15ull)) | 1u;
+}
+const uint32_t *px_cut_lookup(const splat_ctx *ctx, uint64_t key, uint32_t band_tiles);
 
 struct splat_sorter {
     splat_ctx *ctx = nullptr;
@@ -174,6 +192,21 @@
     uint32_t *report_for_composite = nullptr;
     uint32_t report_seq = 0;
     hipEvent_t readback_done = nullptr;
+    bool cut_on = true;
+    CutFrame cut;
+    uint32_t *cut_tables = nullptr;
+    uint32_t cut_tiles_cap = 0;
+    unsigned long long *cut_mask = nullptr;
+    uint32_t cut_mask_cap = 0;
+    uint32_t *cut_state = nullptr;
+    bool pending_cut = false;
+    bool cut_skip_next = false;
+    bool lists_cut = false;
+    uint32_t cut_n = 0, cut_w = 0, cut_h = 0;
+    const uint32_t *cut_keys = nullptr;
+    uint64_t cut_pairs_binned = 0, cut_pairs_full = 0;
+    uint32_t cut_last_binned = 0;
+    uint32_t cut_frames_short = 0;
 };
 
 struct BinParams {
@@ -220,13 +253,15 @@
                       const uint32_t *hist, uint32_t *d_total, uint32_t pair_limit, uint32_t *overflow, uint8_t *out_hi,
                       uint2 *out_val, uint32_t block_splats, uint32_t lo_bits, bool second_pass, const TfRuns *runs,
                       uint32_t *offsets_if_final, uint32_t tiles, uint32_t *report, uint32_t seq, const uint32_t *cidx = nullptr,
-                      const uint32_t *kept = nullptr);
+                      const uint32_t *kept = nullptr,
+                      const unsigned long long *cut_mask = nullptr);
 int tf_second_pass_launch(splat_ctx *ctx, const uint8_t *hi, const uint2 *val_in, uint2 *val_out, const TfRuns *runs, uint32_t pairs_bound,
                           uint32_t tiles, uint32_t lo_bits, uint32_t hi_bits, uint32_t *hist, uint32_t *offsets, const uint32_t *d_total);
 int radix_rowscan_launch(splat_ctx *ctx, uint32_t *hist, uint32_t parts, uint32_t rows);
 int tile_sort_launch(splat_ctx *ctx, const uint32_t *offsets, uint32_t tiles, uint2 *vals, uint2 *scratch, uint32_t *out_idx,
                      uint32_t *counts, uint32_t *frame_flags, uint32_t mean_list, uint32_t band_tiles = 0,
                      uint32_t long_tiles_hint = 0xffffffffu, uint32_t *short_class_io = nullptr);
+int binner_cut_begin(splat_binner *b, const uint32_t *prev_cuts, uint32_t ntx, uint32_t nty, uint32_t n_splats);
 int binner_settle(splat_binner *b);
 struct CompositeArgs {
     const void *color_opacity = nullptr, *normals = nullptr;
@@ -241,6 +276,9 @@
     const splat_aov *aov = nullptr;
     const float *ext_z = nullptr;
     uint32_t ext_zstride = 0;
+    bool want_cut = false;
+    CutFrame cut;
+    const uint32_t *cut_prev = nullptr, *cut_keys = nullptr;
 };
 int composite_launch(splat_ctx *ctx, const splat_composite_cfg *cfg, const CompositeArgs &a);
 int aov_check(splat_ctx *ctx, const splat_composite_cfg *cfg, const splat_aov *aov, bool has_depth);
@@ -250,5 +288,6 @@
                    uint32_t normal_stride_vec4 = 1, void *discs = nullptr,
                    const struct LitIO *lit = nullptr,
                    uint2 *range_wide = nullptr,
-                   const struct EllIO *ell = nullptr);
+                   const struct EllIO *ell = nullptr,
+                   const CutFrame *cut = nullptr);
 int binner_reserve_range_wide(splat_binner *b, uint32_t n_splats);
diff --git a/splat_renderer_amd/csrc/composite.h b/splat_renderer_amd/csrc/composite.h
--- a/splat_renderer_amd/csrc/composite.h
+++ b/splat_renderer_amd/csrc/composite.h
@@ -40,6 +40,10 @@
     uint32_t *aov_id;
     const float *aov_z;
     uint32_t aov_zstride;
+    uint32_t *cut_out;
+    const uint32_t *cut_dil, *cut_prev, *cut_keys;
+    uint32_t *cut_state;
+    uint32_t cut_m;
 };
 
 struct AovPixel {
diff --git a/splat_renderer_amd/csrc/composite.hip b/splat_renderer_amd/csrc/composite.hip
--- a/splat_renderer_amd/csrc/composite.hip
+++ b/splat_renderer_amd/csrc/composite.hip
@@ -405,7 +405,7 @@
     if (p.aov_id) p.aov_id[o] = id;
 }
 
-template <bool EARLY_OUT, bool LIT32, bool COUNT, int AH, bool DISC, bool AOV = false, bool ELL = false>
+template <bool EARLY_OUT, bool LIT32, bool COUNT, int AH, bool DISC, bool AOV = false, bool ELL = false, bool CUT = false>
 __global__ __launch_bounds__(128, AOV ? 4 : PX_WAVES) void k_composite_px(CompositeParams p, uint32_t band_tiles) {
     constexpr uint32_t NB = AH + 1;
     typedef typename PxBufOf<DISC>::type Buf;
@@ -417,7 +417,7 @@
     const uint32_t tid = threadIdx.x, lane = tid & 63;
     const uint32_t role = (uint32_t)__builtin_amdgcn_readfirstlane((int)(tid >> 6));
     if (blockIdx.x == 0) {
-        if (p.report && tid == 0) tile_report(p.frame_total, p.report, p.report_seq);
+        if (p.report && tid == 0 && !(CUT && p.cut_dil)) tile_report(p.frame_total, p.report, p.report_seq);
         if (p.order_dst) px_make_order(p.order_src, band_tiles, p.order_dst, reinterpret_cast<uint32_t *>(s_buf));
         return;
     }
@@ -591,6 +591,7 @@
     v2u idm[2] = {{0xffffffffu, 0xffffffffu}, {0xffffffffu, 0xffffffffu}};
     uint32_t stop_pos = 0;
     uint32_t walked = 0;
+    bool all_stopped_at_end = false;
     constexpr uint32_t NONE = 0xffffffffu;
     const uint32_t lane_x = DISC ? 48u : (bx * PX_ROW + 1u) * 8u;
     const uint32_t d_xy = ((8u + by - bx) * PX_ROW) * 8u;
@@ -798,12 +799,45 @@
             if (EARLY_OUT) {
                 const bool live = px_any_live(T);
                 finished = __ballot(live) == 0;
+                if (CUT) all_stopped_at_end = finished;
                 if (finished && lane == 0) s_done[(k + 1u) & 1u] = 1;
             }
         }
     }
 
     if (p.tile_cost && lane == 0) p.tile_cost[t_local] = walked;
+    if constexpr (CUT) {
+        if (lane == 0) {
+            const uint32_t dil = p.cut_dil ? p.cut_dil[tile_idx] : NOCUT;
+            const bool was_cut = dil != NOCUT;
+            bool valid = !was_cut;
+            uint32_t next = NOCUT;
+            if (all_stopped_at_end) {
+                const uint32_t last = min(walked * PXC, count) - 1u;
+                const unsigned long long q = ((unsigned long long)walked + p.cut_m) * PXC;
+                if (was_cut) valid = p.cut_keys[p.indices[off + last]] <= dil;
+                if (valid) {
+                    if (q <= count) next = p.cut_keys[p.indices[off + (uint32_t)q - 1u]];
+                    else if (was_cut) next = p.cut_prev[tile_idx];
+                }
+            }
+            p.cut_out[t_local] = next;
+            if (p.cut_dil && p.report) {
+                if (!valid) atomicOr(&p.cut_state[2], 1u);
+                __threadfence();
+                if (atomicAdd(&p.cut_state[1], 1u) == band_tiles - 1u) {
+                    __threadfence();
+                    const uint32_t fell_short = __hip_atomic_load(&p.cut_state[2], __ATOMIC_RELAXED, __HIP_MEMORY_SCOPE_AGENT);
+                    p.report[0] = p.frame_total[0];
+                    p.report[1] = p.frame_total[1] | (fell_short ? FRAME_FLAG_CUT_SHORT : 0u);
+                    p.report[3] = p.frame_total[3];
+                    p.report[4] = __hip_atomic_load(&p.cut_state[0], __ATOMIC_RELAXED, __HIP_MEMORY_SCOPE_AGENT);
+                    __threadfence_system();
+                    __hip_atomic_store(&p.report[2], p.report_seq, __ATOMIC_RELEASE, __HIP_MEMORY_SCOPE_SYSTEM);
+                }
+            }
+        }
+    }
 #ifdef PX_PROFILE
     if (p.consumed && lane == 0)
         p.consumed[(size_t)tile_idx * 2 + 1] = (((__builtin_amdgcn_s_memtime() - pc0) >> 4) & 0xffffull) | (((pc_wait >> 4) & 0xffffull) << 16) |
@@ -865,9 +899,15 @@
     return kernel == 1 || (kernel == -1 && ntx * nty >= PX_MIN_TILES);
 }
 
-static int px_order_prepare(splat_ctx *ctx, uint32_t band_tiles, uint64_t key, CompositeParams &p) {
+const uint32_t *px_cut_lookup(const splat_ctx *ctx, uint64_t key, uint32_t band_tiles) {
+    for (const auto &e : ctx->px_hist)
+        if (e.key == key && e.cut_streak >= 1 && e.cut_mem && band_tiles <= e.cut_cap) return e.cut_mem + (size_t)((e.cut_parity ^ 1u) & 1u) * e.cut_cap;
+    return nullptr;
+}
+
+static int px_order_prepare(splat_ctx *ctx, uint32_t band_tiles, uint64_t key, CompositeParams &p, bool want_cut) {
     const bool predict_on = ctx->opt_px_predict >= 0 ? ctx->opt_px_predict != 0 : g_px_predict_on;
-    if (!g_px_order_on && !predict_on) return SPLAT_OK;
+    if (!g_px_order_on && !predict_on && !want_cut) return SPLAT_OK;
     PxHistory *h = nullptr, *lru = &ctx->px_hist[0];
     for (auto &e : ctx->px_hist) {
         if (e.key == key) h = &e;
@@ -877,8 +917,25 @@
         h = lru;
         h->key = key;
         h->streak = 0;
+        h->cut_streak = 0;
     }
     h->last_use = ++ctx->px_clock;
+    if (!want_cut) h->cut_streak = 0;
+    else {
+        if (band_tiles > h->cut_cap) {
+            HIP_TRY(ctx, hipStreamSynchronize(ctx->stream));
+            if (h->cut_mem) (void)hipFree(h->cut_mem);
+            h->cut_mem = nullptr;
+            h->cut_cap = h->cut_streak = 0;
+            const uint32_t cap = (band_tiles + 1023u) & ~1023u;
+            if (hipMalloc((void **)&h->cut_mem, (size_t)cap * 8) != hipSuccess) return ctx_fail(ctx, SPLAT_ERR_OOM, "composite tile cuts hipMalloc");
+            h->cut_cap = cap;
+        }
+        p.cut_out = h->cut_mem + (size_t)(h->cut_parity & 1u) * h->cut_cap;
+        h->cut_parity ^= 1u;
+        if (h->cut_streak < 2) h->cut_streak++;
+    }
+    if (!g_px_order_on && !predict_on) return SPLAT_OK;
     if (band_tiles > h->cap) {
         HIP_TRY(ctx, hipStreamSynchronize(ctx->stream));
         if (h->mem) (void)hipFree(h->mem);
@@ -1089,6 +1146,7 @@
     p.order_src = nullptr;
     p.order_dst = nullptr;
     p.cost_prev = nullptr;
+    p.cut_out = nullptr, p.cut_dil = p.cut_prev = p.cut_keys = nullptr, p.cut_state = nullptr, p.cut_m = 0;
 #ifdef PX_PROFILE
     p.debug_cap = getenv("SPLAT_PX_CAP") ? (uint32_t)strtoul(getenv("SPLAT_PX_CAP"), nullptr, 10) : 0xffffffffu;
 #endif
@@ -1097,6 +1155,8 @@
     p.aov_id = aov ? (uint32_t *)aov->id_u32 : nullptr;
     p.aov_z = (aov && aov->depth_f32) ? zsrc + zoff : (const float *)a.tile_counts;
     p.aov_zstride = (aov && aov->depth_f32) ? zstride : 0u;
+    if (a.cut.dil && !(T == CT && cfg->mode == SPLAT_COMPOSITE_FRONT_TO_BACK && composite_uses_px(ctx, ntx, nty)))
+        return ctx_fail(ctx, SPLAT_ERR_STATE, "composite: a frame was cut that its composite cannot check");
     if (T != CT) return composite_tile_launch(ctx, cfg, p, nty, r0, r1, &report.launched);
     static bool s_env = false;
     if (!s_env) {
@@ -1112,22 +1172,33 @@
     if (cfg->mode == SPLAT_COMPOSITE_FRONT_TO_BACK && composite_uses_px(ctx, ntx, nty)) {
         const int ahead = ctx->opt_px_ahead > 0 ? ctx->opt_px_ahead : g_px_ahead > 0 ? g_px_ahead : ((eo && !p.disc) ? 1 : 2);
         const uint32_t band_tiles = ntx * (r1 - r0);
-        const uint64_t key = (((uint64_t)ntx << 40) ^ ((uint64_t)r0 << 20) ^ (uint64_t)r1 ^ ((uint64_t)width << 50) ^
-                              ((uint64_t)(uintptr_t)a.tile_counts * 0x9E3779B97F4A7C15ull)) | 1u;
-        const int orc = px_order_prepare(ctx, band_tiles, key, p);
+        const uint64_t key = px_history_key(ntx, r0, r1, width, a.tile_counts);
+        const bool cut = a.want_cut && a.cut_keys && eo && !p.disc && !want_aov && !p.compact && r0 == 0 && r1 == nty;
+        if (a.cut.dil && !cut) return ctx_fail(ctx, SPLAT_ERR_STATE, "k_composite_px: a frame was cut that its composite cannot check");
+        const int orc = px_order_prepare(ctx, band_tiles, key, p, cut);
         if (orc != SPLAT_OK) return orc;
+        if (cut && a.cut.dil) {
+            p.cut_dil = a.cut.dil, p.cut_prev = a.cut_prev, p.cut_keys = a.cut_keys, p.cut_state = a.cut.state;
+        } else if (cut) p.cut_keys = a.cut_keys;
+        static const uint32_t s_cut_m = [] {
+            const char *e = getenv("SPLAT_DEPTH_CUT_M");
+            const int v = e ? atoi(e) : -1;
+            return (v >= 0 && v <= 64) ? (uint32_t)v : CUT_M_DEFAULT;
+        }();
+        p.cut_m = s_cut_m;
 #ifdef SPLAT_TEST_HOOKS
         if (ctx->debug_tile_order) p.tile_order = ctx->debug_tile_order;
 #endif
         const bool ok = variant_dispatch(
-            [&](auto eo_, auto lit, auto cnt, auto ah, auto disc, auto aov_, auto ell_) {
-                if constexpr (!(disc.value && lit.value)) {
-                    launch_kernel(ctx, SPLAT_STAGE_COMPOSITE, k_composite_px<eo_.value, lit.value, cnt.value, ah.value, disc.value, aov_.value, ell_.value>,
+            [&](auto eo_, auto lit, auto cnt, auto ah, auto disc, auto aov_, auto ell_, auto cut_) {
+                if constexpr (!(disc.value && lit.value) && (!cut_.value || (eo_.value && !disc.value && !aov_.value && !ell_.value))) {
+                    launch_kernel(ctx, SPLAT_STAGE_COMPOSITE,
+                                  k_composite_px<eo_.value, lit.value, cnt.value, ah.value, disc.value, aov_.value, ell_.value, cut_.value>,
                                   dim3(band_tiles + 1u), dim3(128), p, band_tiles);
                     return true;
                 } else return false;
             },
-            eo, lit32 && !p.disc, p.consumed != nullptr, OneOf<1, 2>{ahead == 2 ? 2 : 1}, p.disc != 0, want_aov, ell);
+            eo, lit32 && !p.disc, p.consumed != nullptr, OneOf<1, 2>{ahead == 2 ? 2 : 1}, p.disc != 0, want_aov, ell, cut);
         if (!ok) return ctx_fail(ctx, SPLAT_ERR_INVALID, "k_composite_px: no kernel for this footprint and record format");
         report.launched = hipPeekAtLastError() == hipSuccess;
         LAUNCH_CHECK(ctx, "k_composite_px");
diff --git a/splat_renderer_amd/csrc/frame.hip b/splat_renderer_amd/csrc/frame.hip
--- a/splat_renderer_amd/csrc/frame.hip
+++ b/splat_renderer_amd/csrc/frame.hip
@@ -713,11 +713,36 @@
         rc = ctx_ensure_consumed(ctx, ntx * nty);
         if (rc != SPLAT_OK) return rc;
     }
+    const bool want_cut = tile_first && binner->cut_on && !disc && !aov && !bp.skip_outside && tile == 16 && cfg->early_out &&
+                          cfg->mode == SPLAT_COMPOSITE_FRONT_TO_BACK && composite_uses_px(ctx, ntx, nty);
+    const uint32_t *cut_prev = nullptr;
+    binner->cut = CutFrame{};
+    if (want_cut) {
+        static const bool s_settle_late = [] {
+            const char *e = getenv("SPLAT_DEPTH_CUT_SETTLE");
+            return e && e[0] == 'l';
+        }();
+        if (!s_settle_late) {
+            rc = binner_settle(binner);
+            if (rc != SPLAT_OK) return rc;
+        }
+        const bool same = binner->cut_n == n && binner->cut_w == width && binner->cut_h == height;
+        if (same && !binner->cut_skip_next) cut_prev = px_cut_lookup(ctx, px_history_key(ntx, 0, nty, width, binner->counts), ntx * nty);
+        binner->cut_skip_next = false;
+        if (cut_prev) {
+            rc = binner_cut_begin(binner, cut_prev, ntx, nty, n);
+            if (rc != SPLAT_OK) return rc;
+        }
+    }
+    const CutFrame cutf = binner->cut;
     const LitIO lio = {(const float4 *)color, (const float4 *)normals, color_stride, 1u, cfg->prelit,
                        lit ? (float4 *)projected : disc_lit ? (float4 *)binner->discs : nullptr};
     rc = project_launch(ctx, uniforms, props, pos_stride, n, 0, lit ? nullptr : projected, splat_sort_keys(sorter), nullptr, n, range32, &bp,
-                        tile_first ? &ho : nullptr, normals, 1, disc ? binner->discs : nullptr, &lio, range_wide, ell);
-    if (rc != SPLAT_OK) return rc;
+                        tile_first ? &ho : nullptr, normals, 1, disc ? binner->discs : nullptr, &lio, range_wide, ell, &cutf);
+    if (rc != SPLAT_OK) {
+        binner->cut = CutFrame{};
+        return rc;
+    }
     binner->tf_hist_ready = tile_first;
     binner->tf_cidx = band_compact ? binner->band_idx : nullptr;
     binner->tf_kept = band_compact ? sorter->hist : nullptr;
@@ -752,6 +777,7 @@
     a.consumed = (ctx->timing && (ctx->timing_mask & SPLAT_TIMING_COUNT_ENTRIES)) ? (void *)ctx->d_consumed : nullptr;
     a.frame_total = binner->d_total, a.report = report, a.report_seq = binner->report_seq;
     a.aov = aov;
+    a.want_cut = want_cut, a.cut = cutf, a.cut_prev = cut_prev, a.cut_keys = sorter->keys;
     a.ext_z = (disc && !disc_lit && projected) ? (const float *)projected + 4 : nullptr, a.ext_zstride = 8u;
     return composite_launch(ctx, cfg, a);
 }
diff --git a/splat_renderer_amd/csrc/project.hip b/splat_renderer_amd/csrc/project.hip
--- a/splat_renderer_amd/csrc/project.hip
+++ b/splat_renderer_amd/csrc/project.hip
@@ -103,7 +103,8 @@
 __device__ __forceinline__ uint32_t project_one(const FrameUniforms &u, const SplatIn &in, uint32_t i, uint32_t index_base,
                                                 float4 *__restrict__ projected, uint32_t *__restrict__ keys,
                                                 uint32_t *__restrict__ payload, uint32_t *__restrict__ range32, const BinParams &bp,
-                                                const DiscIO &dio, const LitIO &lio = LitIO{}, uint32_t kslot = 0xffffffffu) {
+                                                const DiscIO &dio, const LitIO &lio = LitIO{}, uint32_t kslot = 0xffffffffu,
+                                                uint32_t *key_out = nullptr) {
     const uint32_t ks = kslot == 0xffffffffu ? i : kslot;
     float4 a, b;
     float depth;
@@ -138,6 +139,7 @@
     }
     if (WITH_KEYS) {
         keys[ks] = depth_key(depth);
+        if (key_out) *key_out = depth_key(depth);
         if (payload) payload[ks] = index_base + i;
     }
     uint32_t packed = 1u;
@@ -216,13 +218,15 @@
                                                   lio);
 }
 
-template <bool DISC, bool LIT, uint32_t PER, uint32_t AHEAD = 1, bool ELL = false>
+template <bool DISC, bool LIT, uint32_t PER, uint32_t AHEAD = 1, bool ELL = false, bool CUT = false>
 __global__ __launch_bounds__(256) void k_project_hist(FrameUniforms u, const float4 *__restrict__ pos_radius, uint32_t stride_vec4,
                                                       uint32_t n, uint32_t n_padded, float4 *__restrict__ projected,
                                                       uint32_t *__restrict__ keys, uint32_t *__restrict__ range32, BinParams bp,
-                                                      TfHistOut ho, DiscIO dio, LitIO lio) {
+                                                      TfHistOut ho, DiscIO dio, LitIO lio, CutFrame cut) {
     __shared__ uint32_t lh[4][256];
     __shared__ uint32_t wsum[4];
+    __shared__ uint32_t wfull[CUT ? 4 : 1];
+    uint32_t full = 0;
     const uint32_t tid = threadIdx.x, w = tid >> 6;
     const uint32_t blk = xcd_block_of(blockIdx.x, ho.xcd_per);
     if (blk * (PER * 256u) >= n_padded) return;
@@ -243,6 +247,31 @@
             if (i < n) in[k + AHEAD] = load_splat<DISC, LIT, ELL>(pos_radius, stride_vec4, i, dio, lio);
         }
         const uint32_t i = blk * (PER * 256u) + k * 256u + tid;
+        if constexpr (CUT) {
+            bool cut_it = false, keep = false;
+            uint32_t tx0 = 0, tx1 = 0, ty0 = 0, ty1 = 0;
+            if (i >= n) {
+                if (i < n_padded) keys[i] = 0xffffffffu;
+            } else {
+                uint32_t key = 0;
+                const uint32_t r = project_one<true, true, DISC, LIT, false, ELL>(u, in[k], i, 0, projected, keys, nullptr, range32, bp, dio, lio,
+                                                                                  0xffffffffu, &key);
+                tx0 = r & 0xffu, tx1 = (r >> 8) & 0xffu, ty0 = (r >> 16) & 0xffu, ty1 = r >> 24;
+                if (tx0 <= tx1 && ty0 <= ty1) {
+                    const uint32_t dx = tx1 - tx0, dy = ty1 - ty0;
+                    uint32_t lim = NOCUT;
+                    if (dx <= 1u && dy <= 1u) lim = cut.m2[ty0 * bp.ntx + tx0];
+                    else if (dx <= 3u && dy <= 3u) lim = cut.m4[ty0 * bp.ntx + tx0];
+                    cut_it = key > lim;
+                    keep = !cut_it;
+                    full += (dx + 1u) * (dy + 1u);
+                }
+            }
+            const unsigned long long m = __ballot(cut_it);
+            if ((tid & 63) == 0 && i < n) cut.mask[i >> 6] = m;
+            if (keep) local += hist_add_rect(lh[w], tx0, tx1, ty0, ty1, bp.ntx, ho.mask);
+            continue;
+        }
         if (i >= n) {
             if (i < n_padded) keys[i] = 0xffffffffu;
             continue;
@@ -252,6 +281,11 @@
         if (tx0 > tx1 || ty0 > ty1) continue;
         local += hist_add_rect(lh[w], tx0, tx1, ty0, ty1, bp.ntx, ho.mask);
     }
+    if constexpr (CUT) {
+#pragma unroll
+        for (int d = 32; d >= 1; d >>= 1) full += __shfl_xor(full, d);
+        if ((tid & 63) == 0) wfull[w] = full;
+    }
 #pragma unroll
     for (int d = 32; d >= 1; d >>= 1) local += __shfl_xor(local, d);
     if ((tid & 63) == 0) wsum[w] = local;
@@ -259,6 +293,9 @@
     if (blk < ho.num_parts) {
         if (tid <= ho.mask) ho.hist[(size_t)tid * ho.num_parts + blk] = lh[0][tid] + lh[1][tid] + lh[2][tid] + lh[3][tid];
         if (tid == 0) ho.blocksums[blk] = wsum[0] + wsum[1] + wsum[2] + wsum[3];
+        if constexpr (CUT) {
+            if (tid == 0) atomicAdd(&cut.state[0], wfull[0] + wfull[1] + wfull[2] + wfull[3]);
+        }
     }
 }
 
@@ -468,7 +505,7 @@
 int project_launch(splat_ctx *ctx, const float *uniforms, const void *pos_radius, uint32_t pr_stride_vec4, uint32_t n,
                    uint32_t index_base, void *projected, void *keys, void *payload, uint32_t n_padded, uint32_t *range32,
                    const BinParams *bp, const TfHistOut *hist_out, const void *normals, uint32_t normal_stride_vec4, void *discs,
-                   const LitIO *lit, uint2 *range_wide, const EllIO *ell) {
+                   const LitIO *lit, uint2 *range_wide, const EllIO *ell, const CutFrame *cut) {
     FrameUniforms u;
     load_uniforms(u, uniforms);
     const uint32_t work = keys ? n_padded : n;
@@ -522,15 +559,18 @@
         const uint32_t blocks = div_up(work, small ? 256u : 1024u);
         ho.xcd_per = blocks >= 64u ? div_up(blocks, 8u) : 0u;
         const dim3 grid(ho.xcd_per ? 8u * ho.xcd_per : blocks);
+        const bool with_cut = cut && cut->mask;
+        if (with_cut && disc) return ctx_fail(ctx, SPLAT_ERR_INVALID, "project_launch: the depth cut is the isotropic footprint's");
         ok = variant_dispatch(
-            [&](auto d, auto l, auto per, auto e) {
-                if constexpr (d.value || !e.value) {
-                    launch_kernel(ctx, NO_STAGE, k_project_hist<d.value, l.value, per.value, 1, e.value>, grid, block, u, src, pr_stride_vec4, n,
-                                  n_padded, (float4 *)projected, (uint32_t *)keys, range32, *bp, ho, dio, lio);
+            [&](auto d, auto l, auto per, auto e, auto c) {
+                if constexpr ((d.value || !e.value) && !(c.value && d.value)) {
+                    launch_kernel(ctx, NO_STAGE, k_project_hist<d.value, l.value, per.value, 1, e.value, c.value>, grid, block, u, src,
+                                  pr_stride_vec4, n, n_padded, (float4 *)projected, (uint32_t *)keys, range32, *bp, ho, dio, lio,
+                                  with_cut ? *cut : CutFrame{});
                     return true;
                 } else return false;
             },
-            disc, lit_out, OneOf<1, 4>{small ? 1 : 4}, el);
+            disc, lit_out, OneOf<1, 4>{small ? 1 : 4}, el, with_cut);
     } else if (frame_keys && range_wide) {
         ok = variant_dispatch(
             [&](auto d, auto l, auto e) {
diff --git a/splat_renderer_amd/csrc/tile_first.hip b/splat_renderer_amd/csrc/tile_first.hip
--- a/splat_renderer_amd/csrc/tile_first.hip
+++ b/splat_renderer_amd/csrc/tile_first.hip
@@ -78,7 +78,7 @@
 #define TF_SCATTER_WAVES 5
 #endif
 constexpr uint32_t TF_GROUP = 4096;
-template <bool RANK_ATOMIC, uint32_t TF_PER_THREAD, bool COMPACTED = false>
+template <bool RANK_ATOMIC, uint32_t TF_PER_THREAD, bool COMPACTED = false, bool CUT = false>
 __global__ __launch_bounds__(TF_THREADS, TF_SCATTER_WAVES) void k_tf_scatter(const uint32_t *__restrict__ range32,
                                                            const uint32_t *__restrict__ depth_keys, uint32_t n, uint32_t ntx,
                                                            uint32_t mask, uint32_t num_parts,
@@ -89,8 +89,10 @@
                                                            uint32_t lo_bits, uint32_t align_m1, TfRuns runs,
                                                            uint32_t *__restrict__ offsets_out, uint32_t tiles, uint32_t *report,
                                                            uint32_t seq, const uint32_t *__restrict__ cidx,
-                                                           const uint32_t *__restrict__ kept, uint32_t xcd_per) {
+                                                           const uint32_t *__restrict__ kept, uint32_t xcd_per,
+                                                           const unsigned long long *__restrict__ cut_mask) {
     static_assert(!COMPACTED || TF_PER_THREAD == 4, "compacted groups are read four splats per thread");
+    static_assert(!(COMPACTED && CUT), "the depth cut is a whole-screen frame's");
     const uint32_t blk = xcd_block_of(blockIdx.x, xcd_per);
     if (blk >= num_parts) return;
     __shared__ TfScatterShared sh;
@@ -114,6 +116,10 @@
         if (i0 + 1 < n) { rr.y = range32[i0 + 1]; kk.y = depth_keys[i0 + 1]; }
         if (i0 + 2 < n) { rr.z = range32[i0 + 2]; kk.z = depth_keys[i0 + 2]; }
     }
+    unsigned long long cut_word = 0;
+    if constexpr (CUT) {
+        if (i0 < n) cut_word = cut_mask[i0 >> 6];
+    }
     const uint32_t digit_total = totals[tid];
     const uint32_t row_prefix = tid <= mask ? scanned_hist[(size_t)tid * num_parts + blk] : 0u;
 
@@ -164,6 +170,13 @@
         }
     }
     if (all_pairs > pair_limit) return;
+    if constexpr (CUT) {
+        const uint32_t bits = (uint32_t)(cut_word >> (i0 & 63u));
+        if (bits & 1u) rr.x = 1u;
+        if (bits & 2u) rr.y = 1u;
+        if (bits & 4u) rr.z = 1u;
+        if (bits & 8u) rr.w = 1u;
+    }
     sh.global_base[tid] = run_start + row_prefix;
     for (;;) {
     __syncthreads();
@@ -799,7 +812,7 @@
                       const uint32_t *hist, uint32_t *d_total, uint32_t pair_limit, uint32_t *overflow, uint8_t *out_hi,
                       uint2 *out_val, uint32_t block_splats, uint32_t lo_bits, bool second_pass, const TfRuns *runs,
                       uint32_t *offsets_if_final, uint32_t tiles, uint32_t *report, uint32_t seq, const uint32_t *cidx,
-                      const uint32_t *kept) {
+                      const uint32_t *kept, const unsigned long long *cut_mask) {
     const uint32_t parts = div_up(n, block_splats);
     const uint32_t xcd_per = parts >= 64u ? div_up(parts, 8u) : 0u;
     const uint32_t grid_blocks = xcd_per ? 8u * xcd_per : parts;
@@ -810,14 +823,23 @@
         if (prc != SPLAT_OK) return prc;
     }
     const bool ra = rank_atomic_ok(ctx, true);
-#define SPLAT_TF_SCATTER_(RA, PER, COMPACTED)                                                                                     \
-    hipLaunchKernelGGL((k_tf_scatter<RA, PER, COMPACTED>), dim3(grid_blocks), dim3(TF_THREADS), 0, ctx->stream, range32, depth_keys, n, ntx, mask, parts, \
+#define SPLAT_TF_SCATTER_(RA, PER, COMPACTED, CUT)                                                                                \
+    hipLaunchKernelGGL((k_tf_scatter<RA, PER, COMPACTED, CUT>), dim3(grid_blocks), dim3(TF_THREADS), 0, ctx->stream, range32, depth_keys, n, ntx, mask, parts, \
                        hist, totals, d_total, pair_limit, overflow, out_hi, out_val, lo_bits, second_pass ? TF_RUN_ALIGN - 1u : 0u, *runs,         \
-                       second_pass ? nullptr : offsets_if_final, tiles, report, seq, cidx, kept, xcd_per)
-#define SPLAT_TF_SCATTER(RA, PER) SPLAT_TF_SCATTER_(RA, PER, false)
-    if (cidx) {
-        if (ra) SPLAT_TF_SCATTER_(true, 4, true);
-        else SPLAT_TF_SCATTER_(false, 4, true);
+                       second_pass ? nullptr : offsets_if_final, tiles, report, seq, cidx, kept, xcd_per, cut_mask)
+#define SPLAT_TF_SCATTER(RA, PER) SPLAT_TF_SCATTER_(RA, PER, false, false)
+    if (cut_mask) {
+        if (cidx) return ctx_fail(ctx, SPLAT_ERR_INVALID, "tf_scatter_launch: a compacted band has no depth cut");
+        if (block_splats == TF_BLOCK_SMALL) {
+            if (ra) SPLAT_TF_SCATTER_(true, 1, false, true);
+            else SPLAT_TF_SCATTER_(false, 1, false, true);
+        } else {
+            if (ra) SPLAT_TF_SCATTER_(true, 4, false, true);
+            else SPLAT_TF_SCATTER_(false, 4, false, true);
+        }
+    } else if (cidx) {
+        if (ra) SPLAT_TF_SCATTER_(true, 4, true, false);
+        else SPLAT_TF_SCATTER_(false, 4, true, false);
     } else if (block_splats == TF_BLOCK_SMALL) {
         if (ra) SPLAT_TF_SCATTER(true, 1);
         else SPLAT_TF_SCATTER(false, 1);
diff --git a/splat_renderer_amd/dist.py b/splat_renderer_amd/dist.py
--- a/splat_renderer_amd/dist.py
+++ b/splat_renderer_amd/dist.py
@@ -80,6 +80,7 @@
         self.pairs = 0
         self.overflows = 0
         self.misranked = 0
+        self.cut_short = 0
         self.consumed = None
         self.lit = None
         self.pos_plane = None
@@ -88,6 +89,8 @@
     def _again(self, rc):
         if rc == _lib.ERR_RETRY:
             self.misranked += 1
+        elif rc == _lib.ERR_CUT_SHORT:
+            self.cut_short += 1
         else:
             self.overflows += 1
 
diff --git a/splat_renderer_amd/host.py b/splat_renderer_amd/host.py
--- a/splat_renderer_amd/host.py
+++ b/splat_renderer_amd/host.py
@@ -533,6 +533,14 @@
         code = {"default": -1, "sortFirst": 0, "tileFirst": 1}[order] if isinstance(order, str) else int(order)
         check(self.device.lib.splat_bin_set_frame_order(self._b, code), self.device.ctx)
 
+    def setDepthCut(self, on):
+        check(self.device.lib.splat_bin_set_depth_cut(self._b, int(bool(on))), self.device.ctx)
+
+    def cutStats(self):
+        binned, full, short = C.c_uint64(), C.c_uint64(), C.c_uint32()
+        check(self.device.lib.splat_bin_cut_stats(self._b, C.byref(binned), C.byref(full), C.byref(short)), self.device.ctx)
+        return {"pairsBinned": int(binned.value), "pairsFull": int(full.value), "framesShort": int(short.value)}
+
     def getTileSize(self):
         return self.tileSize
 
@@ -787,11 +795,14 @@
         self._last = None
         self.previousFrameOverflowed = False
         self.framesMisranked = 0
+        self.framesCutShort = 0
         self.aov = _AovBuffers(device)
 
     def _again(self, rc):
         if rc == _lib.ERR_RETRY:
             self.framesMisranked += 1
+        elif rc == _lib.ERR_CUT_SHORT:
+            self.framesCutShort += 1
         else:
             self.previousFrameOverflowed = True
 
diff --git a/splat_renderer_amd/napi/splat_napi.c b/splat_renderer_amd/napi/splat_napi.c
--- a/splat_renderer_amd/napi/splat_napi.c
+++ b/splat_renderer_amd/napi/splat_napi.c
@@ -113,7 +113,7 @@
     return NULL;
 }
 
-#define AGAIN(rc) ((rc) == SPLAT_ERR_CAPACITY || (rc) == SPLAT_ERR_RETRY)
+#define AGAIN(rc) ((rc) == SPLAT_ERR_CAPACITY || (rc) == SPLAT_ERR_RETRY || (rc) == SPLAT_ERR_CUT_SHORT)
 
 #define FN(name) static napi_value name(napi_env env, napi_callback_info info)
 #define ARGS(n) call_t c; if (!get_args(env, info, &c, n)) return NULL
@@ -221,6 +221,12 @@
 }
 FN(sort_set_mode) { ARGS(3); splat_ctx *x = arg_external(&c, 0); splat_sorter *s = arg_external(&c, 1); int m = (int)arg_number(&c, 2); BAIL; return check(env, x, splat_sort_set_mode(s, m), mk_undefined(env)); }
 FN(bin_set_frame_order) { ARGS(3); splat_ctx *x = arg_external(&c, 0); splat_binner *b = arg_external(&c, 1); int o = (int)arg_number(&c, 2); BAIL; return check(env, x, splat_bin_set_frame_order(b, o), mk_undefined(env)); }
+FN(bin_set_depth_cut) { ARGS(3); splat_ctx *x = arg_external(&c, 0); splat_binner *b = arg_external(&c, 1); int o = (int)arg_number(&c, 2); BAIL; return check(env, x, splat_bin_set_depth_cut(b, o), mk_undefined(env)); }
+FN(bin_cut_stats) {
+    ARGS(2); splat_ctx *x = arg_external(&c, 0); splat_binner *b = arg_external(&c, 1); BAIL;
+    uint64_t binned = 0; int rc = splat_bin_cut_stats(b, &binned, NULL, NULL);
+    return check(env, x, rc, mk_number(env, (double)binned));
+}
 FN(scan_u32) {
     ARGS(5); splat_ctx *x = arg_external(&c, 0); void *in = arg_dptr(&c, 1), *out = arg_dptr(&c, 2); uint32_t n = (uint32_t)arg_number(&c, 3);
     void *tot = arg_dptr(&c, 4); BAIL;
@@ -777,7 +783,7 @@
         EXPORT(project), EXPORT(project_disc), EXPORT(extract_keys), EXPORT(sort_create), EXPORT(sort_destroy), EXPORT(sort_capacity), EXPORT(sort_keys),
         EXPORT(sort_payload), EXPORT(sort_sorted_payload), EXPORT(sort_sorted_keys), EXPORT(sort_run), EXPORT(sort_set_mode),
         EXPORT(scan_u32), EXPORT(bin_create), EXPORT(bin_destroy), EXPORT(bin_run), EXPORT(bin_counts), EXPORT(bin_offsets),
-        EXPORT(bin_indices), EXPORT(bin_total), EXPORT(bin_set_frame_order), EXPORT(validate_tile_order), EXPORT(composite), EXPORT(render_frame), EXPORT(render_frame_planes),
+        EXPORT(bin_indices), EXPORT(bin_total), EXPORT(bin_set_frame_order), EXPORT(bin_set_depth_cut), EXPORT(bin_cut_stats), EXPORT(validate_tile_order), EXPORT(composite), EXPORT(render_frame), EXPORT(render_frame_planes),
         EXPORT(composite_aov), EXPORT(render_frame_aov), EXPORT(render_frame_planes_aov),
         EXPORT(project_slice_compact), EXPORT(band_frame), EXPORT(band_settle), EXPORT(comm_unique_id), EXPORT(comm_init), EXPORT(comm_destroy),
         EXPORT(ctx_create_on_stream), EXPORT(last_error), EXPORT(set_timing_stages), EXPORT(set_timing_sampling), EXPORT(stage_time_stats), EXPORT(timing_consumed),
```

After: 9354. -40.0%, worse.
